# qurAI-amsterdam/SuperResolution_aniso_MRI

Measured on AMD Instinct MI355X. Metric: training slices/sec (ae_combined, 160x160, latent=128), higher is better.
Workload: dtype f32; 1 GPU; ACDC synthetic 12x(3x1x160x160) triplets, ae_combined latent=128 depth=32 scales=2, MSE synthesis loss (BASELINE configs[1]); global_batch_triplets=12, parallelism=dp1, init=reference Initializer, seed 892372, random weights, launch=captured HIP graph replay

## Files before the change

include/aesr_hip.h:

```cpp
#ifndef AESR_HIP_H
#define AESR_HIP_H

#include <stddef.h>
#include <stdint.h>

#ifdef __cplusplus
extern "C" {
#endif

#define AESR_ABI_VERSION 1
#define AESR_ERR_ARG 1
#define AESR_ERR_HIP 2
#define AESR_ERR_UNSUPPORTED 3

int aesr_version(void);
const char* aesr_last_error_string(void);


size_t aesr_conv2d_packed_floats(int Cout, int Cin, int KS, int transpose);
int aesr_conv2d_pack(const float* w, float* packed, int Cout, int Cin, int KS, int transpose, void* stream);
typedef struct aesr_pack_job {
    const float* w;
    float* packed;
    int Cout, Cin, KS, transpose;
} aesr_pack_job;
int aesr_conv2d_pack_many(const aesr_pack_job* jobs_host, int njobs, void* stream);

#define AESR_PREP_PACK 0
#define AESR_PREP_WINO_PACK 1
#define AESR_PREP_STEM_FOLD 2
#define AESR_PREP_COUT1_FLIP 3
typedef struct aesr_prep_job {
    const float* w;
    const float* aux0;
    const float* aux1;
    float* out;
    int kind, Cout, Cin, KS, transpose;
} aesr_prep_job;
int aesr_weight_prep_many(const aesr_prep_job* jobs_host, int njobs, void* stream);

int aesr_conv2d_fwd(const float* in, const float* packed, const float* bias, float* out, int N, int H, int W, int Cin,
                    int Cout, int KS, int pad, int act, float slope, void* stream);

size_t aesr_conv2d_workspace_floats(int N, int H, int W, int Cin, int Cout, int KS, int pad);
size_t aesr_conv2d_dgrad_workspace_floats(int N, int H, int W, int Cin, int Cout, int KS, int pad);
int aesr_conv2d_fwd_ws(const float* in, const float* packed, const float* bias, float* out, float* workspace, int N, int H, int W,
                       int Cin, int Cout, int KS, int pad, int act, float slope, void* stream);
int aesr_conv2d_dgrad_ws(const float* dy, const float* packed_t, const float* x_saved, float* dx, float* workspace, int N, int H,
                         int W, int Cin, int Cout, int KS, int pad, int mask_act, float slope, void* stream);

int aesr_conv2d_dgrad(const float* dy, const float* packed_t, const float* x_saved, float* dx, int N, int H, int W,
                      int Cin, int Cout, int KS, int pad, int mask_act, float slope, void* stream);

size_t aesr_conv2d_wgrad_workspace_floats(int N, int H, int W, int Cin, int Cout, int KS, int pad);
int aesr_conv2d_wgrad(const float* x, const float* dy, float* dw, float* db, float* workspace, int N, int H, int W,
                      int Cin, int Cout, int KS, int pad, void* stream);

int aesr_conv2d_smallcin_fwd(const float* in, const float* w, const float* bias, const float* y_saved, float* out, int N,
                             int H, int W, int Cin, int Cout, int KS, int pad, int act, int mask_act, float slope,
                             int transpose, int bcast, const float* ca_host, const float* cb_host, void* stream);
int aesr_conv2d_smallcin_dgrad(const float* dy, const float* w, float* dx, int N, int H, int W, int Cin, int Cout, int KS,
                               int pad, int bcast, const float* ca_host, void* stream);
size_t aesr_small_wgrad_workspace_floats(int nout);
int aesr_conv2d_smallcin_wgrad(const float* in, const float* dout, float* dw, float* db, float* workspace, int N, int H,
                               int W, int Cin, int Cout, int pad, void* stream);
int aesr_conv2d_cout1_fwd(const float* x, const float* w, const float* bias, float* out, int N, int H, int W, int Cin, int act,
                          float slope, void* stream);
size_t aesr_conv2d_cout1_workspace_floats(int Cin);
int aesr_conv2d_cout1_wgrad(const float* x, const float* dy, float* dw, float* db, float* workspace, int N, int H, int W,
                            int Cin, void* stream);
int aesr_conv2d_cout1_dgrad(const float* dy, const float* w, const float* y_saved, float* dx, float* workspace, int N, int H,
                            int W, int Cin, int mask_act, float slope, void* stream);
int aesr_conv2d_cout1_dgrad_pre(const float* dy, const float* w_flipped, const float* y_saved, float* dx, int N, int H, int W, int Cin,
                                int mask_act, float slope, void* stream);

size_t aesr_stemconv_folded_floats(int C1);
int aesr_stemconv_fold(const float* w_stem, const float* b_stem, const float* w1, float* folded, int Cs, int C1, void* stream);
int aesr_stemconv_fwd(const float* x, const float* folded, const float* b1, float* out, int N, int H, int W, int C1,
                      int stem_pad, int act, float slope, void* stream);
size_t aesr_stemconv_workspace_floats(int C1);
int aesr_stemconv_wgrad(const float* x, const float* g, const float* w_stem, const float* b_stem, const float* w1,
                        float* dw_stem, float* db_stem, float* dw1, float* db1, float* workspace, int N, int H, int W, int Cs,
                        int C1, int stem_pad, void* stream);

int aesr_space_to_depth2(const float* x, float* out, int N, int H, int W, int C, void* stream);
int aesr_depth_to_space2(const float* g, float* dx, int N, int H, int W, int C, void* stream);

#define AESR_RS_POOL 1
#define AESR_RS_NEAREST 2
#define AESR_RS_BILINEAR 3
int aesr_resample2_fwd(const float* x, float* out, int N, int H, int W, int C, int mode, void* stream);
int aesr_resample2_bwd(const float* gout, const float* x_saved, float* dx, int N, int H, int W, int C, int mode, int mask_act,
                       float slope, void* stream);

#define AESR_BN_NONE 0
#define AESR_BN_POOL 1
#define AESR_BN_UP 2
#define AESR_BN_NWG 512

int aesr_bn_stats(const float* y, float* partial, double* sums, int HW, int C, int G, const int* nstart_host,
                  void* stream);
int aesr_bn_finalize(const double* sums, const double* counts_host, const float* gamma, const float* beta,
                     float* running_mean, float* running_var, int64_t* num_batches_tracked, float* mean, float* invstd,
                     float* scale, float* shift, int C, int G, float momentum, float eps, int train, int update_running,
                     void* stream);
int aesr_bn_stats_finalize(const float* y, float* partial, const double* counts_host, const float* gamma, const float* beta,
                           float* running_mean, float* running_var, int64_t* num_batches_tracked, float* mean, float* invstd,
                           float* scale, float* shift, int HW, int C, int G, const int* nstart_host, float momentum, float eps,
                           int update_running, void* stream);
int aesr_bn_apply(const float* y, const float* scale, const float* shift, float* out, int N, int H, int W, int C, int mode,
                  int G, const int* nstart_host, void* stream);
int aesr_bn_fused_supported(int C, int G);
int aesr_bn_finalize_apply(const double* sums, const double* counts_host, const float* gamma, const float* beta, float* running_mean,
                           float* running_var, int64_t* num_batches_tracked, float* mean, float* invstd, float* scale, float* shift,
                           const float* y, float* out, int N, int H, int W, int C, int mode, int G, const int* nstart_host, float momentum,
                           float eps, int update_running, void* stream);
int aesr_bn_bwd_reduce(const float* gout, const float* y, const float* mean, const float* invstd, float* partial,
                       double* sums, int N, int H, int W, int C, int mode, int G, const int* nstart_host, void* stream);
int aesr_bn_bwd_apply(const float* gout, const float* y, const float* mean, const float* invstd, const float* scale,
                      const double* sums, const double* counts_host, float* coef, float* dgamma, float* dbeta,
                      float* dpre, int N, int H, int W, int C, int mode, int act, float slope, int G,
                      const int* nstart_host, void* stream);
int aesr_bn_bwd(const float* gout, const float* y, const float* mean, const float* invstd, const float* scale, float* partial,
                const double* counts_host, float* coef, float* dgamma, float* dbeta, float* dpre, int N, int H, int W, int C,
                int mode, int act, float slope, int G, const int* nstart_host, void* stream);

int aesr_scale_expand_fwd(const float* x, float* out4, size_t n, const float* ca_host, const float* cb_host, void* stream);
int aesr_scale_expand_bwd(const float* d4, float* dx, size_t n, const float* ca_host, void* stream);
int aesr_maxpool2_fwd(const float* x, float* out, int N, int H, int W, int C, void* stream);
int aesr_maxpool2_bwd(const float* gout, const float* x, const float* gadd, float* dx, int N, int H, int W, int C,
                      int relu_mask, void* stream);
#define AESR_LPIPS_NCH 64
int aesr_lpips_tap_fwd(const float* f, const float* lin_w, float* partial, int B, int HW, int C, void* stream);
int aesr_lpips_tap_bwd(const float* f, const float* lin_w, const float* gd, float* gf0, int B, int HW, int C, void* stream);
int aesr_lpips_finalize(const float* const* partials_host, const int* hw_host, int ntaps, float* d, int B, void* stream);

int aesr_lerp_fwd(const float* z, const float* a_from, const float* a_to, float* zmix, int B, size_t per, void* stream);
int aesr_lerp_bwd(const float* dzmix, const float* a_from, const float* a_to, float* dz, int B, size_t per, void* stream);
int aesr_lerp_cat_fwd(const float* z, const float* a_from, const float* a_to, float* zcat, int B, size_t per, void* stream);
int aesr_lerp_multi(const float* z, float* out, int Z, size_t per_slice, const float* alphas_host, int n, int act, float slope,
                    void* stream);
int aesr_lerp_cat_bwd(const float* g, const float* a_from, const float* a_to, float* dz, int B, size_t per, void* stream);
int aesr_interleave_clamp(const float* orig, const float* synth, float* out, int Z, int n, size_t per_slice, float lo, float hi, void* stream);

#define AESR_MSE_NPART 512
int aesr_mse_fwd(const float* a, const float* b, double* partial, float* loss, size_t n, void* stream);
int aesr_mse_bwd(const float* a, const float* b, const float* gloss, float* da, size_t n, void* stream);
#define AESR_MSE3_NPART 256
#define AESR_MSE3_WS (3 * AESR_MSE3_NPART + 1)
int aesr_mse3_fwd(const float* a1, const float* b1, size_t n1, const float* a2, const float* b2, size_t n2, const float* a3,
                  const float* b3, size_t n3, const float* lam, double* workspace, float* out4, void* stream);
int aesr_mse3_bwd(const float* a1, const float* b1, size_t n1, const float* a2, const float* b2, size_t n2, const float* lam,
                  const float* gloss, float* d1, float* d2, void* stream);
int aesr_l1_fwd(const float* a, const float* b, double* partial, float* loss, size_t n, void* stream);
int aesr_l1_bwd(const float* a, const float* b, const float* gloss, float* da, size_t n, void* stream);
int aesr_lap_blur5(const float* in, const float* add, float* out, int P, int H, int W, float gain, int adjoint, void* stream);
int aesr_lap_down2(const float* in, float* out, int P, int H, int W, void* stream);
int aesr_lap_zero_insert2(const float* in, float* out, int P, int h, int w, int H, int W, void* stream);
int aesr_row_mean_fwd(const float* x, float* out, int N, size_t M, void* stream);
int aesr_row_mean_bwd(const float* g, float* dx, int N, size_t M, void* stream);
int aesr_act_bwd(const float* dout, const float* y, float* dpre, size_t n, int act, float slope, void* stream);

void aesr_adam_state_init(float* state_host8, double steps_done, double beta1, double beta2);
int aesr_adam_step(float* p, float* g, float* exp_avg, float* exp_avg_sq, float* state, size_t n, float lr,
                   double beta1, double beta2, float eps, float weight_decay, int zero_grad, void* stream);

typedef struct aesr_triplet_desc {
    long long vol_off;
    int H, W, z_from, z_to, z_between, oy, ox, k;
    float gain, cutoff;
} aesr_triplet_desc;
int aesr_triplet_assemble(const float* volumes, const aesr_triplet_desc* desc_host, int B, int width, float* image,
                          float* between, void* stream);

size_t aesr_ssim_workspace_doubles(int Z, int H, int W);
int aesr_ssim_mse(const float* a, const float* b, double* workspace, double* ssim, double* mse, int Z, int H, int W, int win,
                  double data_range, double k1, double k2, void* stream);

int aesr_long_axis_views(const float* ref, const float* rec, float* ref_view, float* rec_view, unsigned char* black, int Z, int H, int W,
                         int axis, void* stream);

int aesr_bn_fused1_supported(int N, int H, int W, int C, int mode, int G, int backward);
size_t aesr_bn_fused1_workspace_floats(int C, int G);
size_t aesr_bn_fused1_barrier_words(void);
unsigned int aesr_bn_fused1_timeouts(void);
int aesr_bn_fused1_fwd(const float* y, float* out, float* workspace, unsigned int* barrier_state, const double* counts_host, const float* gamma,
                       const float* beta, float* running_mean, float* running_var, int64_t* num_batches_tracked, float* mean, float* invstd,
                       float* scale, float* shift, int N, int H, int W, int C, int mode, int G, const int* nstart_host, float momentum, float eps,
                       int update_running, void* stream);
int aesr_bn_fused1_bwd(const float* gout, const float* y, const float* mean, const float* invstd, const float* scale, float* workspace,
                       unsigned int* barrier_state, const double* counts_host, float* coef, float* dgamma, float* dbeta, float* dpre, int N, int H,
                       int W, int C, int mode, int act, float slope, int G, const int* nstart_host, void* stream);

#define AESR_P2P_HANDLE_BYTES 64
#define AESR_P2P_SLOTS 32
#define AESR_P2P_REC_BYTES (512 * 8 + 128)
int aesr_p2p_alloc(size_t bytes, void** region);
int aesr_p2p_free(void* region);
int aesr_p2p_get_handle(void* region, char* handle64);
int aesr_p2p_open(const char* handle64, void** peer_region);
int aesr_p2p_close(void* peer_region);
size_t aesr_p2p_region_bytes(int world);
int aesr_p2p_tick(unsigned int* gen_dev, void* stream);
int aesr_bn_fused1_fwd_p2p(const float* y, float* out, float* workspace, unsigned int* barrier_state, const double* counts_host, const float* gamma,
                           const float* beta, float* running_mean, float* running_var, int64_t* num_batches_tracked, float* mean, float* invstd,
                           float* scale, float* shift, int N, int H, int W, int C, int mode, int G, const int* nstart_host, float momentum, float eps,
                           int update_running, void* const* peers_host, int world, int rank, int slot, const unsigned int* gen_dev, void* stream);
int aesr_bn_fused1_bwd_p2p(const float* gout, const float* y, const float* mean, const float* invstd, const float* scale, float* workspace,
                           unsigned int* barrier_state, const double* counts_host, float* coef, float* dgamma, float* dbeta, float* dpre, int N, int H,
                           int W, int C, int mode, int act, float slope, int G, const int* nstart_host, void* const* peers_host, int world, int rank,
                           int slot, const unsigned int* gen_dev, void* stream);

size_t aesr_vif_workspace_bytes(int Z, int H, int W);
int aesr_vif_mscale(const float* ref, const float* dist, void* workspace, double* vif, int Z, int H, int W, const double* weights_host,
                    const int* radii_host, double sigma_nsq, void* stream);

int aesr_conv2d_wino_supported(int Cin, int Cout, int KS, int pad, int transpose);
int aesr_conv2d_wino_kernel(int N, int H, int W, int Cin, int Cout, int KS, int pad, int transpose);
unsigned int aesr_conv2d_wino_ring_timeouts(void);
size_t aesr_conv2d_wino_packed_floats(int Cout, int Cin, int transpose);
int aesr_conv2d_wino_pack_many(const aesr_pack_job* jobs_host, int njobs, void* stream);
int aesr_conv2d_wino_fwd(const float* in, const float* upacked, const float* bias, float* out, int N, int H, int W, int Cin,
                         int Cout, int act, float slope, void* stream);
int aesr_conv2d_wino_dgrad(const float* dy, const float* upacked_t, const float* x_saved, float* dx, int N, int H, int W, int Cin,
                           int Cout, int mask_act, float slope, void* stream);
int aesr_conv2d_wino_fwd_bn_supported(int N, int H, int W, int Cin, int Cout);
int aesr_conv2d_wino_fwd_bn(const float* in, const float* upacked, const float* bias, const float* bn_scale, const float* bn_shift, float* out, int N,
                            int H, int W, int Cin, int Cout, int act, float slope, int pool, void* stream);
size_t aesr_conv2d_wino_workspace_floats(int N, int H, int W, int Cin, int Cout, int transpose);
int aesr_conv2d_wino_fwd_ws(const float* in, const float* upacked, const float* bias, float* out, float* workspace, size_t workspace_floats,
                            int N, int H, int W, int Cin, int Cout, int act, float slope, void* stream);
int aesr_conv2d_wino_dgrad_ws(const float* dy, const float* upacked_t, const float* x_saved, float* dx, float* workspace, size_t workspace_floats,
                              int N, int H, int W, int Cin, int Cout, int mask_act, float slope, void* stream);

int aesr_conv2d_wino_fwd_up2(const float* in_half, const float* upacked, const float* bias, float* out, int N, int H, int W, int Cin,
                             int Cout, int act, float slope, void* stream);
int aesr_conv2d_wino_dgrad_sum2(const float* dy, const float* upacked_t, float* dx_half, int N, int H, int W, int Cin, int Cout,
                                void* stream);
int aesr_conv2d_wgrad_up2_supported(int Cin, int Cout);
int aesr_conv2d_wgrad_up2(const float* x_half, const float* dy, float* dw, float* db, float* workspace, int N, int H, int W, int Cin,
                          int Cout, void* stream);

typedef struct aesr_wgrad_reduce_job {
    const float* workspace;
    float* dw;
    float* db;
    int N, H, W, Cin, Cout, KS, pad;
} aesr_wgrad_reduce_job;
int aesr_conv2d_wgrad_partial(const float* x, const float* dy, float* workspace, int N, int H, int W, int Cin, int Cout, int KS,
                              int pad, int x_up2, void* stream);
int aesr_conv2d_wgrad_reduce_many(const aesr_wgrad_reduce_job* jobs_host, int njobs, void* stream);

#define AESR_COMM_ID_BYTES 128
#define AESR_COMM_F32 0
#define AESR_COMM_F64 1
#define AESR_COMM_SUM 0
#define AESR_COMM_MAX 1
int aesr_comm_rccl_version(int* version_out);
int aesr_comm_unique_id(void* id_host128);
int aesr_comm_init(const void* id_host128, int nranks, int rank, void** comm_out);
int aesr_comm_destroy(void* comm);
int aesr_comm_abort(void* comm);
int aesr_comm_allreduce(void* comm, void* buf, size_t count, int dtype, int op, void* stream);
int aesr_comm_allreduce_many(void* comm, void* const* bufs_host, const size_t* counts_host, int nbufs, int dtype, int op,
                             void* stream);
int aesr_comm_broadcast(void* comm, void* buf, size_t count, int dtype, int root, void* stream);

#ifdef __cplusplus
}
#endif
#endif
```

superresolution_aniso_mri_amd/_hip.py:

```python
import ctypes
import os
from ctypes import c_char_p, c_double, c_float, c_int, c_int64, c_size_t, c_void_p

import torch

_HERE = os.path.dirname(os.path.abspath(__file__))
LIB_PATH = os.path.join(_HERE, "libaesr_hip.so")
if os.environ.get("AESR_LIB"):
    import sys as _sys
    LIB_PATH = os.path.abspath(os.environ["AESR_LIB"])
    _sys.stderr.write("[aesr] AESR_LIB: loading the VARIANT library %s (not the shipped libaesr_hip.so)\n" % LIB_PATH)

P = c_void_p
IP = ctypes.POINTER(c_int)
FP = ctypes.POINTER(c_float)
DP = ctypes.POINTER(c_double)

class TripletDesc(ctypes.Structure):
    _fields_ = [("vol_off", ctypes.c_longlong), ("H", c_int), ("W", c_int), ("z_from", c_int), ("z_to", c_int), ("z_between", c_int),
                ("oy", c_int), ("ox", c_int), ("k", c_int), ("gain", c_float), ("cutoff", c_float)]


class WgradReduceJob(ctypes.Structure):
    _fields_ = [("workspace", c_void_p), ("dw", c_void_p), ("db", c_void_p), ("N", c_int), ("H", c_int), ("W", c_int), ("Cin", c_int),
                ("Cout", c_int), ("KS", c_int), ("pad", c_int)]


class PrepJob(ctypes.Structure):
    _fields_ = [("w", c_void_p), ("aux0", c_void_p), ("aux1", c_void_p), ("out", c_void_p), ("kind", c_int), ("Cout", c_int), ("Cin", c_int),
                ("KS", c_int), ("transpose", c_int)]


PREP_PACK, PREP_WINO_PACK, PREP_STEM_FOLD, PREP_COUT1_FLIP = 0, 1, 2, 3


class PackJob(ctypes.Structure):
    _fields_ = [("w", c_void_p), ("packed", c_void_p), ("Cout", c_int), ("Cin", c_int), ("KS", c_int), ("transpose", c_int)]


SIGNATURES = {
    "aesr_version": (c_int, []),
    "aesr_last_error_string": (c_char_p, []),
    "aesr_conv2d_packed_floats": (c_size_t, [c_int, c_int, c_int, c_int]),
    "aesr_conv2d_pack": (c_int, [P, P, c_int, c_int, c_int, c_int, P]),
    "aesr_conv2d_pack_many": (c_int, [ctypes.POINTER(PackJob), c_int, P]),
    "aesr_weight_prep_many": (c_int, [ctypes.POINTER(PrepJob), c_int, P]),
    "aesr_conv2d_cout1_dgrad_pre": (c_int, [P, P, P, P] + [c_int] * 5 + [c_float, P]),
    "aesr_conv2d_fwd": (c_int, [P, P, P, P] + [c_int] * 8 + [c_float, P]),
    "aesr_conv2d_workspace_floats": (c_size_t, [c_int] * 7),
    "aesr_conv2d_dgrad_workspace_floats": (c_size_t, [c_int] * 7),
    "aesr_conv2d_fwd_ws": (c_int, [P, P, P, P, P] + [c_int] * 8 + [c_float, P]),
    "aesr_conv2d_dgrad_ws": (c_int, [P, P, P, P, P] + [c_int] * 8 + [c_float, P]),
    "aesr_conv2d_dgrad": (c_int, [P, P, P, P] + [c_int] * 8 + [c_float, P]),
    "aesr_conv2d_wgrad_workspace_floats": (c_size_t, [c_int] * 7),
    "aesr_conv2d_wgrad": (c_int, [P, P, P, P, P] + [c_int] * 7 + [P]),
    "aesr_conv2d_smallcin_fwd": (c_int, [P, P, P, P, P] + [c_int] * 9 + [c_float, c_int, c_int, FP, FP, P]),
    "aesr_conv2d_smallcin_dgrad": (c_int, [P, P, P] + [c_int] * 8 + [FP, P]),
    "aesr_small_wgrad_workspace_floats": (c_size_t, [c_int]),
    "aesr_conv2d_smallcin_wgrad": (c_int, [P, P, P, P, P] + [c_int] * 6 + [P]),
    "aesr_conv2d_cout1_fwd": (c_int, [P, P, P, P] + [c_int] * 5 + [c_float, P]),
    "aesr_conv2d_cout1_workspace_floats": (c_size_t, [c_int]),
    "aesr_conv2d_cout1_wgrad": (c_int, [P, P, P, P, P] + [c_int] * 4 + [P]),
    "aesr_conv2d_cout1_dgrad": (c_int, [P, P, P, P, P] + [c_int] * 5 + [c_float, P]),
    "aesr_stemconv_folded_floats": (c_size_t, [c_int]),
    "aesr_stemconv_fold": (c_int, [P, P, P, P, c_int, c_int, P]),
    "aesr_stemconv_fwd": (c_int, [P, P, P, P] + [c_int] * 6 + [c_float, P]),
    "aesr_stemconv_workspace_floats": (c_size_t, [c_int]),
    "aesr_stemconv_wgrad": (c_int, [P] * 10 + [c_int] * 6 + [P]),
    "aesr_space_to_depth2": (c_int, [P, P] + [c_int] * 4 + [P]),
    "aesr_depth_to_space2": (c_int, [P, P] + [c_int] * 4 + [P]),
    "aesr_resample2_fwd": (c_int, [P, P] + [c_int] * 5 + [P]),
    "aesr_resample2_bwd": (c_int, [P, P, P] + [c_int] * 6 + [c_float, P]),
    "aesr_bn_stats": (c_int, [P, P, P, c_int, c_int, c_int, IP, P]),
    "aesr_bn_finalize": (c_int, [P, DP] + [P] * 9 + [c_int, c_int, c_float, c_float, c_int, c_int, P]),
    "aesr_bn_stats_finalize": (c_int, [P, P, DP] + [P] * 9 + [c_int, c_int, c_int, IP, c_float, c_float, c_int, P]),
    "aesr_bn_bwd": (c_int, [P] * 6 + [DP] + [P] * 4 + [c_int] * 6 + [c_float, c_int, IP, P]),
    "aesr_bn_fused_supported": (c_int, [c_int, c_int]),
    "aesr_bn_finalize_apply": (c_int, [P] * 13 + [c_int] * 6 + [P, c_float, c_float, c_int, P]),
    "aesr_bn_fused1_supported": (c_int, [c_int] * 7),
    "aesr_bn_fused1_workspace_floats": (c_size_t, [c_int, c_int]),
    "aesr_bn_fused1_barrier_words": (c_size_t, []),
    "aesr_bn_fused1_timeouts": (ctypes.c_uint, []),
    "aesr_bn_fused1_fwd": (c_int, [P, P, P, P, DP] + [P] * 9 + [c_int] * 6 + [IP, c_float, c_float, c_int, P]),
    "aesr_bn_fused1_bwd": (c_int, [P] * 7 + [DP] + [P] * 4 + [c_int] * 6 + [c_float, c_int, IP, P]),
    "aesr_p2p_alloc": (c_int, [c_size_t, ctypes.POINTER(c_void_p)]),
    "aesr_p2p_free": (c_int, [P]),
    "aesr_p2p_get_handle": (c_int, [P, c_char_p]),
    "aesr_p2p_open": (c_int, [c_char_p, ctypes.POINTER(c_void_p)]),
    "aesr_p2p_close": (c_int, [P]),
    "aesr_p2p_region_bytes": (c_size_t, [c_int]),
    "aesr_p2p_tick": (c_int, [P, P]),
    "aesr_bn_fused1_fwd_p2p": (c_int, [P, P, P, P, DP] + [P] * 9 + [c_int] * 6 + [IP, c_float, c_float, c_int, ctypes.POINTER(c_void_p), c_int, c_int, c_int, P, P]),
    "aesr_bn_fused1_bwd_p2p": (c_int, [P] * 7 + [DP] + [P] * 4 + [c_int] * 6 + [c_float, c_int, IP, ctypes.POINTER(c_void_p), c_int, c_int, c_int, P, P]),
    "aesr_bn_apply": (c_int, [P, P, P, P] + [c_int] * 6 + [IP, P]),
    "aesr_bn_bwd_reduce": (c_int, [P] * 6 + [c_int] * 6 + [IP, P]),
    "aesr_bn_bwd_apply": (c_int, [P] * 6 + [DP] + [P] * 4 + [c_int] * 6 + [c_float, c_int, IP, P]),
    "aesr_scale_expand_fwd": (c_int, [P, P, c_size_t, FP, FP, P]),
    "aesr_scale_expand_bwd": (c_int, [P, P, c_size_t, FP, P]),
    "aesr_maxpool2_fwd": (c_int, [P, P] + [c_int] * 4 + [P]),
    "aesr_maxpool2_bwd": (c_int, [P, P, P, P] + [c_int] * 5 + [P]),
    "aesr_lpips_tap_fwd": (c_int, [P, P, P, c_int, c_int, c_int, P]),
    "aesr_lpips_tap_bwd": (c_int, [P, P, P, P, c_int, c_int, c_int, P]),
    "aesr_lpips_finalize": (c_int, [ctypes.POINTER(c_void_p), IP, c_int, P, c_int, P]),
    "aesr_lerp_fwd": (c_int, [P, P, P, P, c_int, c_size_t, P]),
    "aesr_lerp_bwd": (c_int, [P, P, P, P, c_int, c_size_t, P]),
    "aesr_lerp_cat_fwd": (c_int, [P, P, P, P, c_int, c_size_t, P]),
    "aesr_lerp_multi": (c_int, [P, P, c_int, c_size_t, FP, c_int, c_int, c_float, P]),
    "aesr_lerp_cat_bwd": (c_int, [P, P, P, P, c_int, c_size_t, P]),
    "aesr_interleave_clamp": (c_int, [P, P, P, c_int, c_int, c_size_t, c_float, c_float, P]),
    "aesr_mse_fwd": (c_int, [P, P, P, P, c_size_t, P]),
    "aesr_mse_bwd": (c_int, [P, P, P, P, c_size_t, P]),
    "aesr_mse3_fwd": (c_int, [P, P, c_size_t, P, P, c_size_t, P, P, c_size_t, P, P, P, P]),
    "aesr_mse3_bwd": (c_int, [P, P, c_size_t, P, P, c_size_t, P, P, P, P, P]),
    "aesr_row_mean_fwd": (c_int, [P, P, c_int, c_size_t, P]),
    "aesr_row_mean_bwd": (c_int, [P, P, c_int, c_size_t, P]),
    "aesr_l1_fwd": (c_int, [P, P, P, P, c_size_t, P]),
    "aesr_l1_bwd": (c_int, [P, P, P, P, c_size_t, P]),
    "aesr_lap_blur5": (c_int, [P, P, P, c_int, c_int, c_int, c_float, c_int, P]),
    "aesr_lap_down2": (c_int, [P, P, c_int, c_int, c_int, P]),
    "aesr_lap_zero_insert2": (c_int, [P, P, c_int, c_int, c_int, c_int, c_int, P]),
    "aesr_act_bwd": (c_int, [P, P, P, c_size_t, c_int, c_float, P]),
    "aesr_triplet_assemble": (c_int, [P, ctypes.POINTER(TripletDesc), c_int, c_int, P, P, P]),
    "aesr_ssim_workspace_doubles": (c_size_t, [c_int, c_int, c_int]),
    "aesr_ssim_mse": (c_int, [P, P, P, P, P, c_int, c_int, c_int, c_int, c_double, c_double, c_double, P]),
    "aesr_long_axis_views": (c_int, [P, P, P, P, P, c_int, c_int, c_int, c_int, P]),
    "aesr_vif_workspace_bytes": (c_size_t, [c_int, c_int, c_int]),
    "aesr_vif_mscale": (c_int, [P, P, P, P, c_int, c_int, c_int, DP, IP, c_double, P]),
    "aesr_adam_state_init": (None, [FP, c_double, c_double, c_double]),
    "aesr_adam_step": (c_int, [P, P, P, P, P, c_size_t, c_float, c_double, c_double, c_float, c_float, c_int, P]),
    "aesr_conv2d_wino_supported": (c_int, [c_int] * 5),
    "aesr_conv2d_wino_kernel": (c_int, [c_int] * 8),
    "aesr_conv2d_wino_ring_timeouts": (ctypes.c_uint, []),
    "aesr_conv2d_wino_packed_floats": (c_size_t, [c_int, c_int, c_int]),
    "aesr_conv2d_wino_pack_many": (c_int, [ctypes.POINTER(PackJob), c_int, P]),
    "aesr_conv2d_wino_fwd": (c_int, [P, P, P, P] + [c_int] * 6 + [c_float, P]),
    "aesr_conv2d_wino_dgrad": (c_int, [P, P, P, P] + [c_int] * 6 + [c_float, P]),
    "aesr_conv2d_wino_workspace_floats": (c_size_t, [c_int] * 6),
    "aesr_conv2d_wino_fwd_bn_supported": (c_int, [c_int] * 5),
    "aesr_conv2d_wino_fwd_bn": (c_int, [P, P, P, P, P, P] + [c_int] * 6 + [c_float, c_int, P]),
    "aesr_conv2d_wino_fwd_ws": (c_int, [P, P, P, P, P, c_size_t] + [c_int] * 6 + [c_float, P]),
    "aesr_conv2d_wino_dgrad_ws": (c_int, [P, P, P, P, P, c_size_t] + [c_int] * 6 + [c_float, P]),
    "aesr_conv2d_wino_fwd_up2": (c_int, [P, P, P, P] + [c_int] * 6 + [c_float, P]),
    "aesr_conv2d_wino_dgrad_sum2": (c_int, [P, P, P] + [c_int] * 5 + [P]),
    "aesr_conv2d_wgrad_up2_supported": (c_int, [c_int, c_int]),
    "aesr_conv2d_wgrad_up2": (c_int, [P, P, P, P, P] + [c_int] * 5 + [P]),
    "aesr_conv2d_wgrad_partial": (c_int, [P, P, P] + [c_int] * 8 + [P]),
    "aesr_conv2d_wgrad_reduce_many": (c_int, [ctypes.POINTER(WgradReduceJob), c_int, P]),
    "aesr_comm_rccl_version": (c_int, [IP]),
    "aesr_comm_unique_id": (c_int, [c_char_p]),
    "aesr_comm_init": (c_int, [c_char_p, c_int, c_int, ctypes.POINTER(c_void_p)]),
    "aesr_comm_destroy": (c_int, [P]),
    "aesr_comm_abort": (c_int, [P]),
    "aesr_comm_allreduce": (c_int, [P, P, c_size_t, c_int, c_int, P]),
    "aesr_comm_allreduce_many": (c_int, [P, ctypes.POINTER(c_void_p), ctypes.POINTER(c_size_t), c_int, c_int, c_int, P]),
    "aesr_comm_broadcast": (c_int, [P, P, c_size_t, c_int, c_int, P]),
}
SIGNATURES_PREPROC = {
    "aesr_inplane_out_size": (c_int, [c_int, c_double]),
    "aesr_inplane_workspace_bytes": (c_size_t, [c_int, c_int]),
    "aesr_inplane_resample": (c_int, [P, P, P] + [c_int] * 5 + [DP, c_int, DP, c_int, IP, DP, IP, DP, c_int, P]),
}
P2P_HANDLE_BYTES, P2P_SLOTS = 64, 32
COMM_ID_BYTES = 128
COMM_F32, COMM_F64, COMM_SUM, COMM_MAX = 0, 1, 0, 1

ACT_NONE, ACT_LRELU, ACT_RELU, ACT_SIGMOID = 0, 1, 2, 3
BN_NONE, BN_POOL, BN_UP = 0, 1, 2
RS_POOL, RS_NEAREST, RS_BILINEAR = 1, 2, 3
BN_NWG = 512
REDUCE_MAX_JOBS = 16
MSE_NPART = 512
MSE3_WS = 3 * 256 + 1
LPIPS_NCH = 64


def _load():
    if not os.path.exists(LIB_PATH):
        raise RuntimeError(
            "libaesr_hip.so not found at %s -- build it with `python __graft_entry__.py` (or `make -C "
            "superresolution_aniso_mri_amd/csrc`). The HIP extension is mandatory: there is no CPU/eager fallback." % LIB_PATH)
    lib = ctypes.CDLL(LIB_PATH)
    for name, (res, args) in list(SIGNATURES.items()) + list(SIGNATURES_PREPROC.items()):
        fn = getattr(lib, name, None)
        if fn is None:
            raise RuntimeError("libaesr_hip.so does not export %s (stale build?)" % name)
        fn.restype, fn.argtypes = res, args
    return lib


lib = _load()


def last_error():
    return lib.aesr_last_error_string().decode("utf-8", "replace")


def check(rc, what):
    if rc != 0:
        raise RuntimeError("%s failed (code %d): %s" % (what, rc, last_error()))


def check_device_watchdogs(where):
    nb = int(lib.aesr_bn_fused1_timeouts())
    if nb:
        raise RuntimeError("%s: the one-launch BatchNorm kernel's grid barrier gave up %d time(s) in this process -- its workgroups were not all "
                           "resident (the device is shared with another grid-barrier kernel: set AESR_BN_FUSED=0); results since are not "
                           "trustworthy; nothing was written" % (where, nb))
    n = int(lib.aesr_conv2d_wino_ring_timeouts())
    if n:
        raise RuntimeError("%s: the ring convolution kernel's arrival-counter watchdog fired %d time(s) in this process -- activations / "
                           "gradients computed since are not trustworthy (csrc/conv_wino_ring.hip: wait_full); nothing was written" % (where, n))


def ptr(t):
    if t is None:
        return None
    return c_void_p(t.data_ptr())


_raw_stream = getattr(torch._C, "_cuda_getCurrentRawStream", None)
_cur_device = getattr(torch._C, "_cuda_getDevice", None)
# ... 29 lines not shown
```

superresolution_aniso_mri_amd/csrc/aesr_api.hip:

```cpp
#include <stdarg.h>
#include <stdio.h>
#include <stdlib.h>
#include <string.h>

#include <map>
#include <mutex>
#include <tuple>

#include "../../include/aesr_hip.h"
#include "aesr_kernels.h"

static thread_local char g_err[512] = "";
void aesr_set_error(const char* fmt, ...) {
    va_list ap;
    va_start(ap, fmt);
    vsnprintf(g_err, sizeof(g_err), fmt, ap);
    va_end(ap);
}

static void cout_padding(int Cout, int* CoutP, int* NB) {
    if (Cout <= 16) { *CoutP = 16; *NB = 1; }
    else if (Cout <= 32) { *CoutP = 32; *NB = 2; }
    else { *CoutP = round_up(Cout, 64); *NB = 4; }
}
// ... 442 lines not shown
    const int kin = transpose ? Cout : Cin, nout = transpose ? Cin : Cout;
    const WinoPlan p = plan_wino(N, H, W, kin, nout);
    WinoArgs a = {};
    a.N = N; a.H = H; a.W = W; a.Cin = kin; a.Cout = nout;
    a.CinP = p.CinP; a.CoutP = p.CoutP;
    a.plan_cost = p.cost;
    if (aesr_wino_res_ok(a)) return 0;
    return aesr_wino_ring_workspace_floats(a);
}

unsigned int aesr_conv2d_wino_ring_timeouts(void) {
    (void)hipDeviceSynchronize();
    return aesr_wino_ring_timeouts();
}

size_t aesr_conv2d_wino_packed_floats(int Cout, int Cin, int transpose) {
    const int kin = transpose ? Cout : Cin, nout = transpose ? Cin : Cout;
    return (size_t)16 * round_up(kin, 16) * round_up(nout, 32);
}

int aesr_conv2d_wino_pack_many(const aesr_pack_job* jobs_host, int njobs, void* stream) {
    AESR_CHECK_ARG(jobs_host && njobs > 0, "aesr_conv2d_wino_pack_many: no jobs");
    for (int j0 = 0; j0 < njobs; j0 += PACK_MAX_JOBS) {
        PackTable t;
        memset(&t, 0, sizeof(t));
        t.njobs = njobs - j0 < PACK_MAX_JOBS ? njobs - j0 : PACK_MAX_JOBS;
        int nb = 0;
        for (int k = 0; k < t.njobs; ++k) {
            const aesr_pack_job& jb = jobs_host[j0 + k];
            AESR_CHECK_ARG(jb.w && jb.packed && jb.Cout > 0 && jb.Cin > 0 && jb.KS == 3, "aesr_conv2d_wino_pack_many: bad job %d", j0 + k);
            const int kin = jb.transpose ? jb.Cout : jb.Cin, nout = jb.transpose ? jb.Cin : jb.Cout;
            PackJob& o = t.job[k];
            o.w = jb.w; o.p = jb.packed; o.Cout = jb.Cout; o.Cin = jb.Cin; o.KS = 3; o.KinP = round_up(kin, 16); o.NoutP = round_up(nout, 32);
            o.TN = 32; o.transpose = jb.transpose; o.block0 = nb;
            const size_t pairs = (size_t)o.KinP * o.NoutP;
            int blocks = (int)((pairs + 255) / 256);
            if (blocks > 256) blocks = 256;
            nb += blocks;
        }
        t.nblocks = nb;
        if (int e = aesr_launch_wino_pack_many(t, (hipStream_t)stream)) return e;
    }
    return AESR_OK;
}

static int run_wino(const float* in, const float* upk, const float* bias, const float* ysave, float* out, int N, int H, int W,
                    int Cin, int Cout, int act, int mask_act, float slope, hipStream_t st, int in_up2 = 0, int out_sum2 = 0,
                    float* ws = nullptr, size_t ws_floats = 0) {
    AESR_CHECK_DIMS("aesr_conv2d_wino", N, H, W, Cin, Cout);
    const WinoPlan p = plan_wino(N, H, W, Cin, Cout);
    WinoArgs a = {};
    a.in = in; a.upk = upk; a.bias = bias; a.ysave = ysave; a.out = out;
    a.N = N; a.H = H; a.W = W; a.Cin = Cin; a.CinP = p.CinP; a.Cout = Cout; a.CoutP = p.CoutP;
    a.TI = p.TI; a.THt = p.THt; a.TWt = p.TWt; a.regs_y = a.regs_x = a.nitems = 0;
    a.plan_cost = p.cost;
    a.act = act; a.mask_act = mask_act; a.slope = slope; a.dbgbuf = nullptr; a.flags = 0; a.in_up2 = in_up2; a.out_sum2 = out_sum2;
    a.ws = ws_floats ? ws : nullptr; a.ws_floats = ws ? ws_floats : 0;
    a.ksplit = 1;
    return aesr_launch_conv_wino(a, st);
}

int aesr_conv2d_wino_fwd(const float* in, const float* upacked, const float* bias, float* out, int N, int H, int W, int Cin,
                         int Cout, int act, float slope, void* stream) {
    AESR_CHECK_ARG(in && upacked && out && N > 0 && H > 0 && W > 0, "aesr_conv2d_wino_fwd: null pointer or empty shape");
    AESR_CHECK_ARG(aesr_conv2d_wino_supported(Cin, Cout, 3, 1, 0), "aesr_conv2d_wino_fwd: needs Cin %% 16 == 0 and Cout %% 32 == 0 (got %d -> %d)", Cin, Cout);
    return run_wino(in, upacked, bias, nullptr, out, N, H, W, Cin, Cout, act, ACT_NONE, slope, (hipStream_t)stream);
}

int aesr_conv2d_wino_dgrad(const float* dy, const float* upacked_t, const float* x_saved, float* dx, int N, int H, int W, int Cin,
                           int Cout, int mask_act, float slope, void* stream) {
    AESR_CHECK_ARG(dy && upacked_t && dx && N > 0 && H > 0 && W > 0, "aesr_conv2d_wino_dgrad: null pointer or empty shape");
    AESR_CHECK_ARG(aesr_conv2d_wino_supported(Cin, Cout, 3, 1, 1), "aesr_conv2d_wino_dgrad: needs Cout %% 16 == 0 and Cin %% 32 == 0 (got %d -> %d)", Cin, Cout);
    return run_wino(dy, upacked_t, nullptr, x_saved, dx, N, H, W, Cout, Cin, ACT_NONE, mask_act, slope, (hipStream_t)stream);
}

int aesr_conv2d_wino_fwd_ws(const float* in, const float* upacked, const float* bias, float* out, float* workspace, size_t workspace_floats,
                            int N, int H, int W, int Cin, int Cout, int act, float slope, void* stream) {
    AESR_CHECK_ARG(in && upacked && out && N > 0 && H > 0 && W > 0, "aesr_conv2d_wino_fwd_ws: null pointer or empty shape");
    AESR_CHECK_ARG(aesr_conv2d_wino_supported(Cin, Cout, 3, 1, 0), "aesr_conv2d_wino_fwd_ws: needs Cin %% 16 == 0 and Cout %% 32 == 0 (got %d -> %d)", Cin, Cout);
    return run_wino(in, upacked, bias, nullptr, out, N, H, W, Cin, Cout, act, ACT_NONE, slope, (hipStream_t)stream, 0, 0, workspace, workspace_floats);
}

int aesr_conv2d_wino_dgrad_ws(const float* dy, const float* upacked_t, const float* x_saved, float* dx, float* workspace, size_t workspace_floats,
                              int N, int H, int W, int Cin, int Cout, int mask_act, float slope, void* stream) {
    AESR_CHECK_ARG(dy && upacked_t && dx && N > 0 && H > 0 && W > 0, "aesr_conv2d_wino_dgrad_ws: null pointer or empty shape");
    AESR_CHECK_ARG(aesr_conv2d_wino_supported(Cin, Cout, 3, 1, 1), "aesr_conv2d_wino_dgrad_ws: needs Cout %% 16 == 0 and Cin %% 32 == 0 (got %d -> %d)", Cin, Cout);
    return run_wino(dy, upacked_t, nullptr, x_saved, dx, N, H, W, Cout, Cin, ACT_NONE, mask_act, slope, (hipStream_t)stream, 0, 0, workspace, workspace_floats);
}

int aesr_conv2d_wino_fwd_bn_supported(int N, int H, int W, int Cin, int Cout) {
    if (!aesr_conv2d_wino_supported(Cin, Cout, 3, 1, 0) || !conv_dims_ok(N, H, W, Cin, Cout)) return 0;
    const WinoPlan p = plan_wino(N, H, W, Cin, Cout);
    WinoArgs a = {};
    a.N = N; a.H = H; a.W = W; a.Cin = Cin; a.Cout = Cout;
    a.CinP = p.CinP; a.CoutP = p.CoutP;
    a.plan_cost = p.cost;
    if (aesr_wino_res_ok(a)) return 1;
    return aesr_wino_ring_takes(a) ? 1 : 0;
}

int aesr_conv2d_wino_fwd_bn(const float* in, const float* upacked, const float* bias, const float* bn_scale, const float* bn_shift, float* out, int N,
                            int H, int W, int Cin, int Cout, int act, float slope, int pool, void* stream) {
    AESR_CHECK_ARG(in && upacked && bn_scale && bn_shift && out && N > 0 && H > 0 && W > 0, "aesr_conv2d_wino_fwd_bn: null pointer or empty shape");
    AESR_CHECK_ARG(!pool || (H >= 2 && W >= 2), "aesr_conv2d_wino_fwd_bn: pooling needs H, W >= 2");
    AESR_CHECK_ARG(aesr_conv2d_wino_fwd_bn_supported(N, H, W, Cin, Cout), "aesr_conv2d_wino_fwd_bn: %d -> %d at %d x %d x %d is not a resident-filter or ring-kernel layer "
                   "(aesr_conv2d_wino_fwd_bn_supported)", Cin, Cout, N, H, W);
    const WinoPlan p = plan_wino(N, H, W, Cin, Cout);
    WinoArgs a = {};
    a.in = in; a.upk = upacked; a.bias = bias; a.ysave = nullptr; a.out = out;
    a.N = N; a.H = H; a.W = W; a.Cin = Cin; a.CinP = p.CinP; a.Cout = Cout; a.CoutP = p.CoutP;
    a.TI = p.TI; a.THt = p.THt; a.TWt = p.TWt;
    a.plan_cost = p.cost;
    a.act = act; a.mask_act = ACT_NONE; a.slope = slope; a.ksplit = 1;
    a.post_scale = bn_scale; a.post_shift = bn_shift; a.post_pool = pool ? 1 : 0;
    return aesr_launch_conv_wino(a, (hipStream_t)stream);
}

int aesr_conv2d_wino_fwd_up2(const float* in_half, const float* upacked, const float* bias, float* out, int N, int H, int W, int Cin,
                             int Cout, int act, float slope, void* stream) {
    AESR_CHECK_ARG(in_half && upacked && out && N > 0 && H > 0 && W > 0 && !((H | W) & 1), "aesr_conv2d_wino_fwd_up2: null pointer, empty or odd shape");
    AESR_CHECK_ARG(aesr_conv2d_wino_supported(Cin, Cout, 3, 1, 0), "aesr_conv2d_wino_fwd_up2: needs Cin %% 16 == 0 and Cout %% 32 == 0 (got %d -> %d)", Cin, Cout);
    return run_wino(in_half, upacked, bias, nullptr, out, N, H, W, Cin, Cout, act, ACT_NONE, slope, (hipStream_t)stream, 1, 0);
}

int aesr_conv2d_wino_dgrad_sum2(const float* dy, const float* upacked_t, float* dx_half, int N, int H, int W, int Cin, int Cout,
                                void* stream) {
    AESR_CHECK_ARG(dy && upacked_t && dx_half && N > 0 && H > 0 && W > 0 && !((H | W) & 1), "aesr_conv2d_wino_dgrad_sum2: null pointer, empty or odd shape");
    AESR_CHECK_ARG(aesr_conv2d_wino_supported(Cin, Cout, 3, 1, 1), "aesr_conv2d_wino_dgrad_sum2: needs Cout %% 16 == 0 and Cin %% 32 == 0 (got %d -> %d)", Cin, Cout);
    return run_wino(dy, upacked_t, nullptr, nullptr, dx_half, N, H, W, Cout, Cin, ACT_NONE, ACT_NONE, 0.f, (hipStream_t)stream, 0, 1);
}

size_t aesr_conv2d_wgrad_workspace_floats(int N, int H, int W, int Cin, int Cout, int KS, int pad) {
    if (!conv_dims_ok(N, H, W, Cin, Cout) || (KS != 1 && KS != 3) || pad < 0 || pad >= KS) return 0;
    const int Ho = H + 2 * pad - KS + 1, Wo = W + 2 * pad - KS + 1;
    if (Ho <= 0 || Wo <= 0) return 0;
    return plan_wgrad(N, Ho, Wo, Cin, Cout, KS, pad).slab_floats;
}

static int wgrad_impl(const float* x, const float* dy, float* dw, float* db, float* workspace, int N, int H, int W, int Cin,
                      int Cout, int KS, int pad, void* stream, int x_up2);

int aesr_conv2d_wgrad(const float* x, const float* dy, float* dw, float* db, float* workspace, int N, int H, int W, int Cin,
                      int Cout, int KS, int pad, void* stream) {
    return wgrad_impl(x, dy, dw, db, workspace, N, H, W, Cin, Cout, KS, pad, stream, 0);
}

int aesr_conv2d_wgrad_partial(const float* x, const float* dy, float* workspace, int N, int H, int W, int Cin, int Cout, int KS,
                              int pad, int x_up2, void* stream) {
    AESR_CHECK_ARG(!x_up2 || (wgrad_wino_ok(Cin, Cout, KS, pad) && !((H | W) & 1)), "aesr_conv2d_wgrad_partial: the folded upsampling needs "
                   "the Winograd weight-gradient kernel (3x3, padding 1, Cin, Cout multiples of 32) and an even size");
    return wgrad_impl(x, dy, nullptr, nullptr, workspace, N, H, W, Cin, Cout, KS, pad, stream, x_up2);
}

int aesr_conv2d_wgrad_reduce_many(const aesr_wgrad_reduce_job* jobs_host, int njobs, void* stream) {
    AESR_CHECK_ARG(jobs_host && njobs > 0, "aesr_conv2d_wgrad_reduce_many: no jobs");
    for (int j0 = 0; j0 < njobs; j0 += REDUCE_MAX_JOBS) {
        ReduceTable t;
        memset(&t, 0, sizeof(t));
        t.njobs = njobs - j0 < REDUCE_MAX_JOBS ? njobs - j0 : REDUCE_MAX_JOBS;
        int nb = 0;
        for (int k = 0; k < t.njobs; ++k) {
            const aesr_wgrad_reduce_job& jb = jobs_host[j0 + k];
            AESR_CHECK_ARG(jb.workspace && jb.dw && jb.N > 0 && (jb.KS == 1 || jb.KS == 3), "aesr_conv2d_wgrad_reduce_many: bad job %d", j0 + k);
            AESR_CHECK_ARG(conv_dims_ok(jb.N, jb.H, jb.W, jb.Cin, jb.Cout) && jb.pad >= 0 && jb.pad < jb.KS && jb.H + 2 * jb.pad >= jb.KS && jb.W + 2 * jb.pad >= jb.KS,
                           "aesr_conv2d_wgrad_reduce_many: job %d: bad shape", j0 + k);
            const int Ho = jb.H + 2 * jb.pad - jb.KS + 1, Wo = jb.W + 2 * jb.pad - jb.KS + 1;
            const WgradPlan p = plan_wgrad(jb.N, Ho, Wo, jb.Cin, jb.Cout, jb.KS, jb.pad);
            ReduceJob& o = t.job[k];
            o.slab = jb.workspace; o.dw = jb.dw; o.db = jb.db; o.nslab = p.nslab; o.KS2 = jb.KS * jb.KS; o.Cin = jb.Cin; o.CinP = p.CinP;
            o.Cout = jb.Cout; o.CoutP = p.CoutP; o.block0 = nb;
            nb += ceil_div(o.KS2 * jb.Cin * jb.Cout + (jb.db ? jb.Cout : 0), 64);
        }
        t.nblocks = nb;
        if (int e = aesr_launch_wgrad_reduce_many(t, (hipStream_t)stream)) return e;
    }
    return AESR_OK;
}

int aesr_conv2d_wgrad_up2_supported(int Cin, int Cout) { return wgrad_wino_ok(Cin, Cout, 3, 1) ? 1 : 0; }

int aesr_conv2d_wgrad_up2(const float* x_half, const float* dy, float* dw, float* db, float* workspace, int N, int H, int W, int Cin,
                          int Cout, void* stream) {
    AESR_CHECK_ARG(wgrad_wino_ok(Cin, Cout, 3, 1) && !((H | W) & 1), "aesr_conv2d_wgrad_up2: needs the Winograd weight-gradient kernel "
                   "(Cin, Cout multiples of 32; got %d -> %d) and an even size", Cin, Cout);
    return wgrad_impl(x_half, dy, dw, db, workspace, N, H, W, Cin, Cout, 3, 1, stream, 1);
}

static int wgrad_impl(const float* x, const float* dy, float* dw, float* db, float* workspace, int N, int H, int W, int Cin,
                      int Cout, int KS, int pad, void* stream, int x_up2) {
    AESR_CHECK_ARG(x && dy && workspace && N > 0, "aesr_conv2d_wgrad: null pointer or empty shape");
    AESR_CHECK_ARG(Cin % 4 == 0 && Cout % 4 == 0, "aesr_conv2d_wgrad: Cin=%d, Cout=%d must be multiples of 4", Cin, Cout);
    AESR_CHECK_ARG((KS == 1 || KS == 3) && pad >= 0 && pad < KS, "aesr_conv2d_wgrad: unsupported KS=%d pad=%d", KS, pad);
    AESR_CHECK_DIMS("aesr_conv2d_wgrad", N, H, W, Cin, Cout);
    const int Ho = H + 2 * pad - KS + 1, Wo = W + 2 * pad - KS + 1;
    AESR_CHECK_ARG(Ho > 0 && Wo > 0, "aesr_conv2d_wgrad: the %d x %d input is smaller than the %d x %d filter", H, W, KS, KS);
    const WgradPlan p = plan_wgrad(N, Ho, Wo, Cin, Cout, KS, pad);
    WgradArgs a;
    a.x = x; a.dy = dy; a.slab = workspace;
    a.N = N; a.H = H; a.W = W; a.Cin = Cin; a.CinP = p.CinP; a.Cout = Cout; a.CoutP = p.CoutP; a.Ho = Ho; a.Wo = Wo; a.pad = pad;
    a.TH = p.TH; a.TW = p.TW; a.tiles_y = ceil_div(Ho, p.TH); a.tiles_x = ceil_div(Wo, p.TW);
    a.ntiles = N * a.tiles_y * a.tiles_x; a.S = p.S;
    a.PWS = p.PWS; a.TWS = p.TWS; a.PSX = p.PSX; a.PSD = p.PSD; a.dbgbuf = nullptr; a.x_up2 = x_up2;
    if (p.variant == 2) {
        if (int e = aesr_launch_conv_wgrad_wino(a, (hipStream_t)stream)) return e;
    } else if (int e = aesr_launch_conv_wgrad(a, KS, p.variant, (hipStream_t)stream)) {
        return e;
    }
    if (!dw) return AESR_OK;
    return aesr_launch_wgrad_reduce(workspace, dw, db, p.nslab, KS, Cin, p.CinP, Cout, p.CoutP, (hipStream_t)stream);
}

int aesr_conv2d_smallcin_fwd(const float* in, const float* w, const float* bias, const float* y_saved, float* out, int N,
                             int H, int W, int Cin, int Cout, int KS, int pad, int act, int mask_act, float slope,
                             int transpose, int bcast, const float* ca_host, const float* cb_host, void* stream) {
    AESR_CHECK_ARG(in && w && out && N > 0 && Cin >= 1 && Cin <= 4 && Cout > 0, "aesr_conv2d_smallcin_fwd: need 1 <= Cin <= 4");
    AESR_CHECK_ARG(!bcast || (ca_host && cb_host), "aesr_conv2d_smallcin_fwd: bcast needs ca/cb");
    SmallArgs a;
    memset(&a, 0, sizeof(a));
    a.in = in; a.w = w; a.bias = bias; a.ysave = y_saved; a.out = out;
    a.N = N; a.H = H; a.W = W; a.Cin = Cin; a.Cout = Cout; a.KS = KS; a.pad = pad;
    a.Ho = H + 2 * pad - KS + 1; a.Wo = W + 2 * pad - KS + 1;
    a.act = act; a.mask_act = mask_act; a.slope = slope; a.transpose = transpose; a.bcast = bcast;
    for (int i = 0; i < Cin && bcast; ++i) { a.ca[i] = ca_host[i]; a.cb[i] = cb_host[i]; }
    return aesr_launch_smallcin_fwd(a, (hipStream_t)stream);
}

int aesr_conv2d_smallcin_dgrad(const float* dy, const float* w, float* dx, int N, int H, int W, int Cin, int Cout, int KS,
                               int pad, int bcast, const float* ca_host, void* stream) {
    AESR_CHECK_ARG(dy && w && dx && N > 0 && Cin >= 1 && Cin <= 4 && Cout > 0, "aesr_conv2d_smallcin_dgrad: need 1 <= Cin <= 4");
    AESR_CHECK_ARG(!bcast || ca_host, "aesr_conv2d_smallcin_dgrad: bcast needs ca");
    SmallDgradArgs a;
    memset(&a, 0, sizeof(a));
    a.dy = dy; a.w = w; a.dx = dx; a.N = N; a.H = H; a.W = W; a.Cin = Cin; a.Cout = Cout; a.KS = KS; a.pad = pad; a.bcast = bcast;
    a.Ho = H + 2 * pad - KS + 1; a.Wo = W + 2 * pad - KS + 1;
    for (int i = 0; i < Cin && bcast; ++i) a.ca[i] = ca_host[i];
    return aesr_launch_smallcin_dgrad(a, (hipStream_t)stream);
}

#define SMALL_WGRAD_NWG 512
size_t aesr_small_wgrad_workspace_floats(int nout) { return (size_t)SMALL_WGRAD_NWG * nout; }

int aesr_conv2d_smallcin_wgrad(const float* in, const float* dout, float* dw, float* db, float* workspace, int N, int H,
                               int W, int Cin, int Cout, int pad, void* stream) {
    AESR_CHECK_ARG(in && dout && dw && db && workspace && Cin >= 1 && Cin <= 4, "aesr_conv2d_smallcin_wgrad: need 1 <= Cin <= 4");
    AESR_CHECK_ARG(Cout >= 4 && Cout % 4 == 0 && 256 % (Cout / 4) == 0 && Cout <= 256,
                   "aesr_conv2d_smallcin_wgrad: Cout=%d must be a multiple of 4 with Cout/4 dividing 256", Cout);
    SmallWgradArgs a;
    a.in = in; a.dout = dout; a.partial = workspace; a.N = N; a.H = H; a.W = W; a.Cin = Cin; a.Cout = Cout; a.pad = pad;
    a.Ho = H + 2 * pad; a.Wo = W + 2 * pad;
    if (int e = aesr_launch_smallcin_wgrad(a, SMALL_WGRAD_NWG, (hipStream_t)stream)) return e;
    return aesr_launch_sum_partials(workspace, SMALL_WGRAD_NWG, Cout * (Cin + 1), dw, Cout * Cin, db, (hipStream_t)stream);
}

int aesr_conv2d_cout1_fwd(const float* x, const float* w, const float* bias, float* out, int N, int H, int W, int Cin, int act,
                          float slope, void* stream) {
    AESR_CHECK_ARG(x && w && out && N > 0 && H > 0 && W > 0, "aesr_conv2d_cout1_fwd: null pointer or empty shape");
    AESR_CHECK_ARG(Cin > 0 && Cin % 4 == 0 && Cin <= 256, "aesr_conv2d_cout1_fwd: Cin=%d must be a multiple of 4 (<= 256)", Cin);
    if (((Cin / 4) & (Cin / 4 - 1)) == 0)
        return aesr_launch_thin_collapse(x, w, bias, out, N, H, W, Cin, act, slope, (hipStream_t)stream);
    Cout1FwdArgs a;
    a.x = x; a.w = w; a.bias = bias; a.out = out; a.N = N; a.H = H; a.W = W; a.Cin = Cin; a.act = act; a.slope = slope;
    a.TH = H < 16 ? H : 16; a.TW = W < 16 ? W : 16;
    while (((size_t)(a.TH + 2) * (a.TW + 2) * (Cin + 4) + 9 * Cin) * 4 > 64 * 1024 && a.TH > 1) a.TH /= 2;
    a.tiles_y = ceil_div(H, a.TH); a.tiles_x = ceil_div(W, a.TW);
    return aesr_launch_cout1_fwd(a, (hipStream_t)stream);
}

#define THIN_NWG 512
static bool thin_channels_ok(int C) { return C >= 4 && C <= 256 && C % 4 == 0 && ((C / 4) & (C / 4 - 1)) == 0; }

size_t aesr_conv2d_cout1_workspace_floats(int Cin) {
    const size_t legacy = (size_t)SMALL_WGRAD_NWG * (Cin * 9 + 1);
    const size_t thin = (size_t)(THIN_NWG + 1) * 10 * Cin;
    return legacy > thin ? legacy : thin;
}

int aesr_conv2d_cout1_wgrad(const float* x, const float* dy, float* dw, float* db, float* workspace, int N, int H, int W,
                            int Cin, void* stream) {
    AESR_CHECK_ARG(x && dy && dw && db && workspace, "aesr_conv2d_cout1_wgrad: null pointer");
    AESR_CHECK_ARG(N > 0 && H > 0 && W > 0, "aesr_conv2d_cout1_wgrad: empty shape");
    if (thin_channels_ok(Cin)) {
        ThinArgs a;
        memset(&a, 0, sizeof(a));
        a.s = dy; a.t = x; a.partial = workspace;
        a.N = N; a.Hs = H; a.Ws = W; a.Ho = H; a.Wo = W; a.C = Cin; a.ps = 0; a.with_be = 0;
        float* R = workspace + (size_t)THIN_NWG * 10 * Cin;
        if (int e = aesr_launch_thin_reduce(a, THIN_NWG, (hipStream_t)stream)) return e;
        if (int e = aesr_launch_sum_partials(workspace, THIN_NWG, 10 * Cin, R, 10 * Cin, nullptr, (hipStream_t)stream)) return e;
        return aesr_launch_thin_cout1_finish(R, dw, db, Cin, (hipStream_t)stream);
    }
    AESR_CHECK_ARG(Cin >= 4 && Cin <= 128 && 256 % Cin == 0, "aesr_conv2d_cout1_wgrad: Cin=%d must divide 256 (and be >= 4)", Cin);
    Cout1WgradArgs a;
    a.x = x; a.dy = dy; a.partial = workspace; a.N = N; a.H = H; a.W = W; a.Cin = Cin;
    a.TH = H < 16 ? H : 16; a.TW = W < 16 ? W : 16;
    while ((size_t)(a.TH + 2) * (a.TW + 2) * (Cin + 1) * 4 > 60 * 1024 && a.TH > 1) a.TH /= 2;
    a.tiles_y = ceil_div(H, a.TH); a.tiles_x = ceil_div(W, a.TW); a.ntiles = N * a.tiles_y * a.tiles_x;
    int nwg = a.ntiles < SMALL_WGRAD_NWG ? a.ntiles : SMALL_WGRAD_NWG;
    if (int e = aesr_launch_cout1_wgrad(a, nwg, (hipStream_t)stream)) return e;
    return aesr_launch_sum_partials(workspace, nwg, Cin * 9 + 1, dw, Cin * 9, db, (hipStream_t)stream);
}

int aesr_conv2d_cout1_dgrad(const float* dy, const float* w, const float* y_saved, float* dx, float* workspace, int N, int H,
                            int W, int Cin, int mask_act, float slope, void* stream) {
    AESR_CHECK_ARG(dy && w && dx && workspace && N > 0 && H > 0 && W > 0, "aesr_conv2d_cout1_dgrad: null pointer or empty shape");
    AESR_CHECK_ARG(thin_channels_ok(Cin), "aesr_conv2d_cout1_dgrad: Cin=%d must be 4 times a power of two (4..256)", Cin);
    if (int e = aesr_launch_thin_cout1_flip(w, workspace, Cin, (hipStream_t)stream)) return e;
    ThinArgs a;
    memset(&a, 0, sizeof(a));
    a.s = dy; a.w = workspace; a.ysave = y_saved; a.out = dx;
    a.N = N; a.Hs = H; a.Ws = W; a.Ho = H; a.Wo = W; a.C = Cin; a.ps = 0;
    a.act = ACT_NONE; a.mask_act = y_saved ? mask_act : ACT_NONE; a.slope = slope;
    return aesr_launch_thin_expand(a, (hipStream_t)stream);
}

int aesr_conv2d_cout1_dgrad_pre(const float* dy, const float* w_flipped, const float* y_saved, float* dx, int N, int H, int W, int Cin,
                                int mask_act, float slope, void* stream) {
    AESR_CHECK_ARG(dy && w_flipped && dx && N > 0 && H > 0 && W > 0, "aesr_conv2d_cout1_dgrad_pre: null pointer or empty shape");
    AESR_CHECK_ARG(thin_channels_ok(Cin), "aesr_conv2d_cout1_dgrad_pre: Cin=%d must be 4 times a power of two (4..256)", Cin);
    ThinArgs a;
    memset(&a, 0, sizeof(a));
    a.s = dy; a.w = w_flipped; a.ysave = y_saved; a.out = dx;
    a.N = N; a.Hs = H; a.Ws = W; a.Ho = H; a.Wo = W; a.C = Cin; a.ps = 0;
    a.act = ACT_NONE; a.mask_act = y_saved ? mask_act : ACT_NONE; a.slope = slope;
    return aesr_launch_thin_expand(a, (hipStream_t)stream);
}

size_t aesr_stemconv_folded_floats(int C1) { return (size_t)2 * 9 * C1; }

int aesr_stemconv_fold(const float* w_stem, const float* b_stem, const float* w1, float* folded, int Cs, int C1, void* stream) {
    AESR_CHECK_ARG(w_stem && w1 && folded && Cs > 0 && C1 > 0, "aesr_stemconv_fold: bad arguments");
    return aesr_launch_thin_stem_fold(w_stem, b_stem, w1, folded, Cs, C1, (hipStream_t)stream);
}

int aesr_stemconv_fwd(const float* x, const float* folded, const float* b1, float* out, int N, int H, int W, int C1,
                      int stem_pad, int act, float slope, void* stream) {
    AESR_CHECK_ARG(x && folded && out && N > 0 && H > 0 && W > 0 && stem_pad >= 0, "aesr_stemconv_fwd: bad arguments");
    AESR_CHECK_ARG(thin_channels_ok(C1), "aesr_stemconv_fwd: C1=%d must be 4 times a power of two (4..256)", C1);
    ThinArgs a;
    memset(&a, 0, sizeof(a));
    a.s = x; a.w = folded; a.be = folded + (size_t)9 * C1; a.b = b1; a.out = out;
    a.N = N; a.Hs = H; a.Ws = W; a.Ho = H + 2 * stem_pad; a.Wo = W + 2 * stem_pad; a.C = C1; a.ps = stem_pad;
    a.act = act; a.mask_act = ACT_NONE; a.slope = slope;
    return aesr_launch_thin_expand(a, (hipStream_t)stream);
}

size_t aesr_stemconv_workspace_floats(int C1) { return (size_t)(THIN_NWG + 1) * 19 * C1; }

int aesr_stemconv_wgrad(const float* x, const float* g, const float* w_stem, const float* b_stem, const float* w1,
                        float* dw_stem, float* db_stem, float* dw1, float* db1, float* workspace, int N, int H, int W, int Cs,
                        int C1, int stem_pad, void* stream) {
    AESR_CHECK_ARG(x && g && w_stem && w1 && dw_stem && dw1 && workspace, "aesr_stemconv_wgrad: null pointer");
    AESR_CHECK_ARG(N > 0 && H > 0 && W > 0 && Cs > 0 && stem_pad >= 0, "aesr_stemconv_wgrad: bad shape");
    AESR_CHECK_ARG(thin_channels_ok(C1), "aesr_stemconv_wgrad: C1=%d must be 4 times a power of two (4..256)", C1);
    AESR_CHECK_ARG(!db_stem || b_stem, "aesr_stemconv_wgrad: db_stem needs b_stem");
    ThinArgs a;
    memset(&a, 0, sizeof(a));
    a.s = x; a.t = g; a.partial = workspace;
    a.N = N; a.Hs = H; a.Ws = W; a.Ho = H + 2 * stem_pad; a.Wo = W + 2 * stem_pad; a.C = C1; a.ps = stem_pad; a.with_be = 1;
    float* R = workspace + (size_t)THIN_NWG * 19 * C1;
    if (int e = aesr_launch_thin_reduce(a, THIN_NWG, (hipStream_t)stream)) return e;
    if (int e = aesr_launch_sum_partials(workspace, THIN_NWG, 19 * C1, R, 19 * C1, nullptr, (hipStream_t)stream)) return e;
    return aesr_launch_thin_stem_finish(R, w_stem, b_stem, w1, dw_stem, db_stem, dw1, db1, Cs, C1, (hipStream_t)stream);
}

int aesr_resample2_fwd(const float* x, float* out, int N, int H, int W, int C, int mode, void* stream) {
    AESR_CHECK_ARG(x && out && N > 0 && H > 0 && W > 0 && C > 0 && C % 4 == 0, "aesr_resample2_fwd: bad arguments (C %% 4 == 0)");
    AESR_CHECK_ARG(mode >= AESR_RS_POOL && mode <= AESR_RS_BILINEAR, "aesr_resample2_fwd: unknown mode %d", mode);
    AESR_CHECK_ARG(mode != AESR_RS_POOL || (H >= 2 && W >= 2), "aesr_resample2_fwd: pooling needs H, W >= 2");
    return aesr_launch_resample2(x, nullptr, nullptr, out, N, H, W, C, mode, 0, ACT_NONE, 0.f, (hipStream_t)stream);
}

int aesr_resample2_bwd(const float* gout, const float* x_saved, float* dx, int N, int H, int W, int C, int mode, int mask_act,
                       float slope, void* stream) {
    AESR_CHECK_ARG(gout && dx && N > 0 && H > 0 && W > 0 && C > 0 && C % 4 == 0, "aesr_resample2_bwd: bad arguments (C %% 4 == 0)");
    AESR_CHECK_ARG(mode >= AESR_RS_POOL && mode <= AESR_RS_BILINEAR, "aesr_resample2_bwd: unknown mode %d", mode);
    AESR_CHECK_ARG(mode != AESR_RS_POOL || (H >= 2 && W >= 2), "aesr_resample2_bwd: pooling needs H, W >= 2");
    return aesr_launch_resample2(nullptr, gout, x_saved, dx, N, H, W, C, mode, 1, x_saved ? mask_act : ACT_NONE, slope,
                                 (hipStream_t)stream);
}

int aesr_bn_stats(const float* y, float* partial, double* sums, int HW, int C, int G, const int* nstart_host, void* stream) {
    BnGroups gr;
    AESR_CHECK_ARG(y && partial && sums && fill_groups(&gr, G, nstart_host), "aesr_bn_stats: bad arguments");
    if (int e = aesr_launch_bn_stats(y, partial, HW, C, gr, AESR_BN_NWG, (hipStream_t)stream)) return e;
    return aesr_launch_bn_reduce(partial, sums, AESR_BN_NWG, C, G, (hipStream_t)stream);
}

int aesr_bn_finalize(const double* sums, const double* counts_host, const float* gamma, const float* beta, float* running_mean,
                     float* running_var, int64_t* num_batches_tracked, float* mean, float* invstd, float* scale, float* shift,
                     int C, int G, float momentum, float eps, int train, int update_running, void* stream) {
    AESR_CHECK_ARG(gamma && beta && mean && invstd && scale && shift && G >= 1 && G <= 4, "aesr_bn_finalize: bad arguments");
    AESR_CHECK_ARG(!train || (sums && counts_host), "aesr_bn_finalize: train mode needs sums and counts");
    AESR_CHECK_ARG(train || (running_mean && running_var), "aesr_bn_finalize: eval mode needs running stats");
    return aesr_launch_bn_finalize(sums, counts_host, gamma, beta, running_mean, running_var, (long long*)num_batches_tracked, mean,
                                   invstd, scale, shift, C, G, momentum, eps, train, update_running && running_mean && running_var,
                                   (hipStream_t)stream);
}

int aesr_bn_stats_finalize(const float* y, float* partial, const double* counts_host, const float* gamma, const float* beta,
                           float* running_mean, float* running_var, int64_t* num_batches_tracked, float* mean, float* invstd,
                           float* scale, float* shift, int HW, int C, int G, const int* nstart_host, float momentum, float eps,
                           int update_running, void* stream) {
    BnGroups gr;
    AESR_CHECK_ARG(y && partial && counts_host && fill_groups(&gr, G, nstart_host), "aesr_bn_stats_finalize: bad arguments");
    AESR_CHECK_ARG(gamma && beta && mean && invstd && scale && shift, "aesr_bn_stats_finalize: null pointer");
    if (int e = aesr_launch_bn_stats(y, partial, HW, C, gr, AESR_BN_NWG, (hipStream_t)stream)) return e;
    return aesr_launch_bn_reduce_finalize(partial, AESR_BN_NWG, counts_host, gamma, beta, running_mean, running_var,
                                          (long long*)num_batches_tracked, mean, invstd, scale, shift, C, G, momentum, eps,
                                          update_running && running_mean && running_var, (hipStream_t)stream);
}

static void bn_out_dims(int H, int W, int mode, int* Ho, int* Wo) {
    if (mode == AESR_BN_POOL) { *Ho = H / 2; *Wo = W / 2; }
    else if (mode == AESR_BN_UP) { *Ho = 2 * H; *Wo = 2 * W; }
    else { *Ho = H; *Wo = W; }
}

int aesr_bn_apply(const float* y, const float* scale, const float* shift, float* out, int N, int H, int W, int C, int mode,
                  int G, const int* nstart_host, void* stream) {
    BnApplyArgs a;
    AESR_CHECK_ARG(y && scale && shift && out && fill_groups(&a.gr, G, nstart_host), "aesr_bn_apply: bad arguments");
    a.y = y; a.scale = scale; a.shift = shift; a.out = out; a.N = N; a.H = H; a.W = W; a.C = C; a.mode = mode;
    bn_out_dims(H, W, mode, &a.Ho, &a.Wo);
    AESR_CHECK_ARG(a.Ho > 0 && a.Wo > 0, "aesr_bn_apply: empty output");
    return aesr_launch_bn_apply(a, (hipStream_t)stream);
}

int aesr_bn_fused_supported(int C, int G) { return aesr_bn_fused_ok(C, G) ? 1 : 0; }

int aesr_bn_fused1_supported(int N, int H, int W, int C, int mode, int G, int backward) {
    if (mode != AESR_BN_NONE && mode != AESR_BN_POOL) return 0;
    return aesr_bn_fused1_ok(N, H, W, C, mode == AESR_BN_POOL, G, backward) ? 1 : 0;
}

size_t aesr_bn_fused1_workspace_floats(int C, int G) { return (size_t)256 * G * 2 * C; }
size_t aesr_bn_fused1_barrier_words(void) { return 16 * 32; }
unsigned int aesr_bn_fused1_timeouts(void) { return aesr_bn_fused_timeouts_impl(); }

int aesr_bn_fused1_fwd(const float* y, float* out, float* workspace, unsigned int* barrier_state, const double* counts_host, const float* gamma,
                       const float* beta, float* running_mean, float* running_var, int64_t* num_batches_tracked, float* mean, float* invstd,
                       float* scale, float* shift, int N, int H, int W, int C, int mode, int G, const int* nstart_host, float momentum, float eps,
                       int update_running, void* stream) {
    BnGroups gr;
    AESR_CHECK_ARG(y && out && workspace && barrier_state && counts_host && gamma && beta && mean && invstd && scale && shift &&
                       fill_groups(&gr, G, nstart_host) && gr.nstart[G] == N, "aesr_bn_fused1_fwd: bad arguments");
    AESR_CHECK_ARG(mode == AESR_BN_NONE || mode == AESR_BN_POOL, "aesr_bn_fused1_fwd: mode %d (the un-folded Upsample takes the three-launch path)", mode);
    return aesr_bn_fused_run(y, nullptr, out, workspace, barrier_state, gamma, beta, running_mean, running_var, (long long*)num_batches_tracked, mean,
                             invstd, scale, shift, nullptr, nullptr, nullptr, N, H, W, C, mode == AESR_BN_POOL, G, gr.nstart, counts_host, momentum, eps,
                             update_running && running_mean && running_var, ACT_NONE, 0.f, 0, nullptr, (hipStream_t)stream);
}

int aesr_bn_fused1_bwd(const float* gout, const float* y, const float* mean, const float* invstd, const float* scale, float* workspace,
                       unsigned int* barrier_state, const double* counts_host, float* coef, float* dgamma, float* dbeta, float* dpre, int N, int H,
                       int W, int C, int mode, int act, float slope, int G, const int* nstart_host, void* stream) {
    BnGroups gr;
    AESR_CHECK_ARG(gout && y && mean && invstd && scale && workspace && barrier_state && counts_host && coef && dgamma && dbeta && dpre &&
                       fill_groups(&gr, G, nstart_host) && gr.nstart[G] == N, "aesr_bn_fused1_bwd: bad arguments");
    AESR_CHECK_ARG(mode == AESR_BN_NONE || mode == AESR_BN_POOL, "aesr_bn_fused1_bwd: mode %d (the un-folded Upsample takes the three-launch path)", mode);
    return aesr_bn_fused_run(y, gout, dpre, workspace, barrier_state, nullptr, nullptr, nullptr, nullptr, nullptr, (float*)mean, (float*)invstd,
                             (float*)scale, nullptr, coef, dgamma, dbeta, N, H, W, C, mode == AESR_BN_POOL, G, gr.nstart, counts_host, 0.f, 0.f, 0, act, slope,
                             1, nullptr, (hipStream_t)stream);
}

size_t aesr_p2p_region_bytes(int world) { return world > 0 && world <= 8 ? (size_t)AESR_P2P_SLOTS * 2 * world * AESR_P2P_REC_BYTES : 0; }

int aesr_p2p_tick(unsigned int* gen_dev, void* stream) {
    AESR_CHECK_ARG(gen_dev, "aesr_p2p_tick: null pointer");
    return aesr_launch_p2p_tick(gen_dev, (hipStream_t)stream);
}

static int fill_p2p(BnP2P* p, void* const* peers_host, int world, int rank, int slot, const unsigned int* gen_dev, const char* who) {
    if (!peers_host || !gen_dev || world < 1 || world > 8 || rank < 0 || rank >= world || slot < 0 || slot >= AESR_P2P_SLOTS) {
        aesr_set_error("%s: bad exchange arguments (world %d, rank %d, slot %d of %d)", who, world, rank, slot, AESR_P2P_SLOTS);
        return AESR_ERR_ARG;
    }
    p->world = world; p->rank = rank; p->slot = slot; p->gen = gen_dev;
    for (int r = 0; r < 8; ++r) p->peers[r] = r < world ? peers_host[r] : nullptr;
    for (int r = 0; r < world; ++r)
        if (!p->peers[r]) {
            aesr_set_error("%s: the region of rank %d is not mapped", who, r);
            return AESR_ERR_ARG;
        }
    return AESR_OK;
}

int aesr_bn_fused1_fwd_p2p(const float* y, float* out, float* workspace, unsigned int* barrier_state, const double* counts_host, const float* gamma,
                           const float* beta, float* running_mean, float* running_var, int64_t* num_batches_tracked, float* mean, float* invstd,
                           float* scale, float* shift, int N, int H, int W, int C, int mode, int G, const int* nstart_host, float momentum, float eps,
                           int update_running, void* const* peers_host, int world, int rank, int slot, const unsigned int* gen_dev, void* stream) {
    BnGroups gr;
    BnP2P p2p;
    AESR_CHECK_ARG(y && out && workspace && barrier_state && counts_host && gamma && beta && mean && invstd && scale && shift &&
                       fill_groups(&gr, G, nstart_host) && gr.nstart[G] == N, "aesr_bn_fused1_fwd_p2p: bad arguments");
    AESR_CHECK_ARG(mode == AESR_BN_NONE || mode == AESR_BN_POOL, "aesr_bn_fused1_fwd_p2p: mode %d", mode);
    if (int e = fill_p2p(&p2p, peers_host, world, rank, slot, gen_dev, "aesr_bn_fused1_fwd_p2p")) return e;
    return aesr_bn_fused_run(y, nullptr, out, workspace, barrier_state, gamma, beta, running_mean, running_var, (long long*)num_batches_tracked, mean,
                             invstd, scale, shift, nullptr, nullptr, nullptr, N, H, W, C, mode == AESR_BN_POOL, G, gr.nstart, counts_host, momentum, eps,
                             update_running && running_mean && running_var, ACT_NONE, 0.f, 0, &p2p, (hipStream_t)stream);
}

int aesr_bn_fused1_bwd_p2p(const float* gout, const float* y, const float* mean, const float* invstd, const float* scale, float* workspace,
                           unsigned int* barrier_state, const double* counts_host, float* coef, float* dgamma, float* dbeta, float* dpre, int N, int H,
                           int W, int C, int mode, int act, float slope, int G, const int* nstart_host, void* const* peers_host, int world, int rank,
                           int slot, const unsigned int* gen_dev, void* stream) {
    BnGroups gr;
    BnP2P p2p;
    AESR_CHECK_ARG(gout && y && mean && invstd && scale && workspace && barrier_state && counts_host && coef && dgamma && dbeta && dpre &&
                       fill_groups(&gr, G, nstart_host) && gr.nstart[G] == N, "aesr_bn_fused1_bwd_p2p: bad arguments");
    AESR_CHECK_ARG(mode == AESR_BN_NONE || mode == AESR_BN_POOL, "aesr_bn_fused1_bwd_p2p: mode %d", mode);
    if (int e = fill_p2p(&p2p, peers_host, world, rank, slot, gen_dev, "aesr_bn_fused1_bwd_p2p")) return e;
    return aesr_bn_fused_run(y, gout, dpre, workspace, barrier_state, nullptr, nullptr, nullptr, nullptr, nullptr, (float*)mean, (float*)invstd,
                             (float*)scale, nullptr, coef, dgamma, dbeta, N, H, W, C, mode == AESR_BN_POOL, G, gr.nstart, counts_host, 0.f, 0.f, 0, act, slope,
                             1, &p2p, (hipStream_t)stream);
}

int aesr_bn_finalize_apply(const double* sums, const double* counts_host, const float* gamma, const float* beta, float* running_mean,
                           float* running_var, int64_t* num_batches_tracked, float* mean, float* invstd, float* scale, float* shift,
// ... 281 lines not shown
```

superresolution_aniso_mri_amd/csrc/aesr_kernels.h:

```cpp
#pragma once
#include "aesr_common.h"

struct IgemmArgs {
    const float* in; const float* wpk; const float* bias; const float* ysave; float* out;
    int N, H, W, Cin, CinP, Cout, CoutP, Ho, Wo, pad;
    int TI, TH, TW, tiles_y, tiles_x, nitems, dbg;
    int NT;
    int ksplit;
    float* dbgbuf;
    int act, mask_act;
    float slope;
};
int aesr_launch_conv_igemm(const IgemmArgs& a, int KS, int NB, int MBW, hipStream_t st);
int aesr_launch_conv_ksplit_fixup(const float* partial, const float* bias, const float* ysave, float* out, size_t nelem, int Cout,
                                  int ksplit, int act, int mask_act, float slope, hipStream_t st);
int aesr_launch_pack_weights(const float* w, float* p, int Cout, int Cin, int KS, int KinP, int NoutP, int TN, int transpose, hipStream_t st);

struct WinoArgs {
    const float* in; const float* upk; const float* bias; const float* ysave; float* out;
    int N, H, W, Cin, CinP, Cout, CoutP;
    int TI, THt, TWt;
    int regs_y, regs_x, nitems;
    unsigned m_ncot, m_regs_x, m_regs_y;
    int act, mask_act;
    float slope;
    float* dbgbuf;
    int flags;
    int in_up2;
    int out_sum2;
    int bpi, nblk;
    unsigned m_bpi;
    int nw, rowP, imgP, patch_fl, sw_a, sw_m, sw_b;
    int xcd_map;
    double plan_cost;
    int nfull, tail_k;
    int ksplit, kchunks, split_bytes;
    unsigned m_ksplit;
    float* ws;
    size_t ws_floats;
    const float* post_scale; const float* post_shift;
    int post_pool;
};
int aesr_launch_conv_wino(const WinoArgs& a, hipStream_t st);
bool aesr_wino_res_ok(const WinoArgs& a);
int aesr_launch_conv_wino_res(const WinoArgs& a, hipStream_t st);
int aesr_wino_ring_mode();
bool aesr_wino_ring_takes(const WinoArgs& a);
int aesr_launch_conv_wino_ring(const WinoArgs& a, hipStream_t st);
size_t aesr_wino_ring_workspace_floats(const WinoArgs& a);
unsigned aesr_wino_ring_timeouts();
size_t aesr_wino_lds_bytes(int patch_pixels);

#define PACK_MAX_JOBS 32
struct PackJob { const float* w; float* p; int Cout, Cin, KS, KinP, NoutP, TN, transpose, block0; };
struct PackTable { int njobs, nblocks; PackJob job[PACK_MAX_JOBS]; };
int aesr_launch_pack_many(const PackTable& t, hipStream_t st);
enum { PREP_PACK = 0, PREP_WINO_PACK = 1, PREP_STEM_FOLD = 2, PREP_COUT1_FLIP = 3 };
struct PrepJob { const float* w; const float* aux0; const float* aux1; float* out; int kind, Cout, Cin, KS, KinP, NoutP, TN, transpose, block0; };
struct PrepTable { int njobs, nblocks; PrepJob job[PACK_MAX_JOBS]; };
int aesr_launch_prep_many(const PrepTable& t, hipStream_t st);
int aesr_launch_wino_pack_many(const PackTable& t, hipStream_t st);

struct WgradArgs {
    const float* x; const float* dy; float* slab;
    int N, H, W, Cin, CinP, Cout, CoutP, Ho, Wo, pad;
    int TH, TW, tiles_y, tiles_x, ntiles;
    int S;
    int PWS, TWS, PSX, PSD;
    float* dbgbuf;
    int x_up2;
};
int aesr_launch_conv_wgrad(const WgradArgs& a, int KS, int variant, hipStream_t st);
int aesr_launch_conv_wgrad_wino(const WgradArgs& a, hipStream_t st);
size_t aesr_wgrad_wino_lds_bytes(int TH, int TW);
bool aesr_wgrad_wino_tile_ok(int TH, int TW);
#define REDUCE_MAX_JOBS 16
struct ReduceJob { const float* slab; float* dw; float* db; int nslab, KS2, Cin, CinP, Cout, CoutP, block0; };
struct ReduceTable { int njobs, nblocks; ReduceJob job[REDUCE_MAX_JOBS]; };
int aesr_launch_wgrad_reduce_many(const ReduceTable& t, hipStream_t st);
int aesr_launch_wgrad_reduce(const float* slab, float* dw, float* db, int nslab, int KS, int Cin, int CinP, int Cout, int CoutP, hipStream_t st);

struct SmallArgs {
    const float* in; const float* w; const float* bias; const float* ysave; float* out;
    int N, H, W, Cin, Cout, Ho, Wo, KS, pad;
    int act, mask_act;
    float slope;
    int transpose, bcast;
    float ca[4], cb[4];
};
struct SmallDgradArgs {
    const float* dy; const float* w; float* dx;
    int N, H, W, Cin, Cout, Ho, Wo, KS, pad, bcast;
    float ca[4];
};
struct SmallWgradArgs {
    const float* in; const float* dout; float* partial;
    int N, H, W, Cin, Cout, Ho, Wo, pad;
};
struct Cout1WgradArgs {
    const float* x; const float* dy; float* partial;
    int N, H, W, Cin, TH, TW, tiles_y, tiles_x, ntiles;
};
struct Cout1FwdArgs {
    const float* x; const float* w; const float* bias; float* out;
    int N, H, W, Cin, TH, TW, tiles_y, tiles_x, act;
    float slope;
};
int aesr_launch_cout1_fwd(const Cout1FwdArgs& a, hipStream_t st);
int aesr_launch_smallcin_fwd(const SmallArgs& a, hipStream_t st);
int aesr_launch_smallcin_dgrad(const SmallDgradArgs& a, hipStream_t st);
int aesr_launch_sum_partials(const float* partial, int np, int n, float* out0, int n0, float* out1, hipStream_t st);
int aesr_launch_smallcin_wgrad(const SmallWgradArgs& a, int nwg, hipStream_t st);
int aesr_launch_cout1_wgrad(const Cout1WgradArgs& a, int nwg, hipStream_t st);

struct ThinArgs {
    const float* s;
    const float* w;
    const float* be;
    const float* b;
    const float* ysave;
    float* out;
    const float* t;
    float* partial;
    int N, Hs, Ws, Ho, Wo, C, ps;
    int act, mask_act;
    float slope;
    int with_be;
    int tiles_y, tiles_x, ntiles;
};
int aesr_launch_thin_expand(ThinArgs a, hipStream_t st);
int aesr_launch_thin_reduce(ThinArgs a, int nwg, hipStream_t st);
int aesr_launch_thin_collapse(const float* x, const float* w, const float* bias, float* out, int N, int H, int W, int C, int act,
                              float slope, hipStream_t st);
int aesr_launch_thin_stem_fold(const float* ws, const float* bs, const float* w1, float* folded, int Cs, int C1, hipStream_t st);
int aesr_launch_thin_stem_finish(const float* R, const float* ws, const float* bs, const float* w1, float* dws, float* dbs,
                                 float* dw1, float* db1, int Cs, int C1, hipStream_t st);
int aesr_launch_thin_cout1_flip(const float* w, float* wexp, int Cin, hipStream_t st);
int aesr_launch_thin_cout1_finish(const float* R, float* dw, float* db, int Cin, hipStream_t st);

struct BnGroups { int G; int nstart[5]; };
struct BnApplyArgs {
    const float* y; const float* scale; const float* shift; float* out;
    int N, H, W, C, Ho, Wo, mode;
    BnGroups gr;
};
struct BnBwdArgs {
    const float* gout; const float* y; const float* mean; const float* invstd; const float* scale; const float* coef;
    float* partial; float* dpre;
    int N, H, W, C, Ho, Wo, mode, act;
    float slope;
    BnGroups gr;
    unsigned long long m_hw, m_w;
    int k_hw, k_w;
};
struct BnFusedArgs;
struct BnP2P { int world, rank, slot; const unsigned* gen; void* peers[8]; };
int aesr_launch_p2p_tick(unsigned* gen, hipStream_t st);
bool aesr_bn_fused1_ok(int N, int H, int W, int C, int pool, int G, int backward);
unsigned aesr_bn_fused_timeouts_impl();
int aesr_bn_fused_run(const float* y, const float* gout, float* out, float* rec, unsigned* bar, const float* gamma, const float* beta,
                      float* running_mean, float* running_var, long long* nbt, float* mean, float* invstd, float* scale, float* shift, float* coef,
                      float* dgamma, float* dbeta, int N, int H, int W, int C, int pool, int G, const int* nstart, const double* counts,
                      float momentum, float eps, int update_running, int act, float slope, int backward, const BnP2P* p2p, hipStream_t st);
int aesr_launch_bn_stats(const float* y, float* partial, int HW, int C, const BnGroups& gr, int nwg, hipStream_t st);
int aesr_launch_bn_reduce(const float* partial, double* sums, int nwg, int C, int G, hipStream_t st);
int aesr_launch_bn_finalize(const double* sums, const double* counts, const float* gamma, const float* beta, float* rm, float* rv,
                            long long* nbt, float* mean, float* invstd, float* scale, float* shift, int C, int G, float momentum,
                            float eps, int train, int update_running, hipStream_t st);
int aesr_launch_bn_reduce_finalize(const float* partial, int nwg, const double* counts, const float* gamma, const float* beta,
                                   float* running_mean, float* running_var, long long* nbt, float* mean, float* invstd,
                                   float* scale, float* shift, int C, int G, float momentum, float eps, int update_running,
                                   hipStream_t st);
int aesr_launch_bn_bwd_reduce_finalize(const float* partial, int nwg, const double* counts, float* coef, float* dgamma,
                                       float* dbeta, int C, int G, hipStream_t st);
int aesr_launch_bn_apply(const BnApplyArgs& a, hipStream_t st);
int aesr_launch_bn_bwd_reduce(const BnBwdArgs& a, int nwg, hipStream_t st);
int aesr_launch_bn_bwd_finalize(const double* sums, const double* counts, float* coef, float* dgamma, float* dbeta, int C, int G, hipStream_t st);
int aesr_launch_bn_bwd_apply(const BnBwdArgs& a, hipStream_t st);
bool aesr_bn_fused_ok(int C, int G);
int aesr_launch_bn_finalize_apply(const double* sums, const double* counts, const float* gamma, const float* beta, float* running_mean,
                                  float* running_var, long long* nbt, float* mean, float* invstd, float* scale, float* shift, float momentum,
                                  float eps, int update_running, int G, const BnApplyArgs& a, hipStream_t st);
int aesr_launch_bn_bwd_finalize_apply(const double* sums, const double* counts, float* coef, float* dgamma, float* dbeta, int G,
                                      const BnBwdArgs& a, hipStream_t st);

int aesr_launch_lerp_fwd(const float* z, const float* af, const float* at, float* zmix, int B, size_t per, hipStream_t st);
int aesr_launch_lerp_bwd(const float* dmix, const float* af, const float* at, float* dz, int B, size_t per, hipStream_t st);
int aesr_launch_lerp_cat_fwd(const float* z, const float* af, const float* at, float* zcat, int B, size_t per, hipStream_t st);
int aesr_launch_interleave_clamp(const float* orig, const float* synth, float* out, int Z, int n, size_t per, float lo, float hi, hipStream_t st);
int aesr_launch_lerp_multi(const float* z, float* out, int Z, size_t per, const float* alphas, int n, float nslope, hipStream_t st);
int aesr_launch_lerp_cat_bwd(const float* g, const float* af, const float* at, float* dz, int B, size_t per, hipStream_t st);
int aesr_launch_mse_fwd(const float* a, const float* b, double* partial, int np, float* out, size_t n, hipStream_t st);
int aesr_launch_mse3_fwd(const float* const* a, const float* const* b, const size_t* n, const float* lam, double* ws, float* out, hipStream_t st);
int aesr_launch_mse3_bwd(const float* a1, const float* b1, size_t n1, const float* a2, const float* b2, size_t n2, const float* lam,
                         const float* g, float* d1, float* d2, hipStream_t st);
int aesr_launch_mse_bwd(const float* a, const float* b, const float* g, float* da, size_t n, hipStream_t st);
int aesr_launch_act_bwd(const float* dout, const float* y, float* dpre, size_t n, int act, float slope, hipStream_t st);
int aesr_launch_adam(float* p, float* g, float* m, float* v, float* state, size_t n, float lr, double beta1, double beta2,
                     float eps, float wd, int zero_g, hipStream_t st);


int aesr_launch_maxpool2_fwd(const float* x, float* out, int N, int H, int W, int C, hipStream_t st);
int aesr_launch_maxpool2_bwd(const float* gout, const float* x, const float* gadd, float* dx, int N, int H, int W, int C, int relu, hipStream_t st);
int aesr_launch_lpips_tap_fwd(const float* f, const float* lin, float* partial, int B, int HW, int C, hipStream_t st);
int aesr_launch_lpips_tap_bwd(const float* f, const float* lin, const float* gd, float* gf0, int B, int HW, int C, hipStream_t st);
int aesr_launch_lpips_finalize(const float* const* partials, const int* hw, int ntaps, float* d, int B, hipStream_t st);
int aesr_launch_scale_expand(const float* x, float* out4, int n, const float* ca, const float* cb, int backward, hipStream_t st);
int aesr_launch_resample2(const float* x, const float* gout, const float* xsave, float* dst, int N, int H, int W, int C, int mode,
                          int backward, int mask_act, float slope, hipStream_t st);
size_t aesr_vif_workspace_bytes_impl(int Z, int H, int W);
int aesr_launch_vif_mscale(const float* ref, const float* dist, void* workspace, double* vif, int Z, int H, int W, const double* weights,
                           const int* radii, double sigma_nsq, hipStream_t st);
int aesr_launch_ssim_mse(const float* a, const float* b, double* partial, double* ssim, double* mse, int Z, int H, int W, int win,
                         double data_range, double k1, double k2, hipStream_t st);
int aesr_launch_long_axis_views(const float* ref, const float* rec, float* ref_view, float* rec_view, unsigned char* black, int Z, int H,
                                int W, int axis, hipStream_t st);
#define TRIPLET_MAX 64
struct TripletDesc { long long vol_off; int H, W, z_from, z_to, z_between, oy, ox, k; float gain, cutoff; };
struct TripletTable { TripletDesc d[TRIPLET_MAX]; };
int aesr_launch_triplet_assemble(const float* vol, const TripletTable& t, int B, int W, float* image, float* between, hipStream_t st);
int aesr_launch_s2d(const float* x, float* out, int N, int H, int W, int C, int inverse, hipStream_t st);

int aesr_launch_lap_blur5(const float* in, const float* add, float* out, int P, int H, int W, float gain, int adjoint, hipStream_t st);
int aesr_launch_lap_down2(const float* in, float* out, int P, int H, int W, hipStream_t st);
int aesr_launch_lap_zero_insert2(const float* in, float* out, int P, int h, int w, int H, int W, hipStream_t st);
int aesr_launch_l1_fwd(const float* a, const float* b, double* partial, int np, float* out, size_t n, hipStream_t st);
int aesr_launch_l1_bwd(const float* a, const float* b, const float* g, float* da, size_t n, hipStream_t st);
int aesr_launch_row_mean_fwd(const float* x, float* out, int N, size_t M, hipStream_t st);
int aesr_launch_row_mean_bwd(const float* g, float* dx, int N, size_t M, hipStream_t st);
```

superresolution_aniso_mri_amd/csrc/conv_thin.hip:

```cpp
#include "aesr_kernels.h"
#include "aesr_pack_dev.h"

#define THIN_TH 8
#ifndef THIN_ETH
#define THIN_ETH 16
#endif
#define THIN_XS 68

__host__ __device__ __forceinline__ int thin_tw(int C4) { return 256 / C4 < 64 ? 256 / C4 : 64; }

template <int TH = THIN_TH>
__device__ __forceinline__ void thin_stage(const ThinArgs& a, float (*xs)[THIN_XS], int n, int y0, int x0, int TW) {
    const int PW = TW + 2;
    for (int q = threadIdx.x; q < (TH + 2) * PW; q += 256) {
        const int r = q / PW, c = q - r * PW;
        const int sy = y0 + r - 1 - a.ps, sx = x0 + c - 1 - a.ps;
        float v = 0.f;
        if (sy >= 0 && sy < a.Hs && sx >= 0 && sx < a.Ws) v = a.s[((size_t)n * a.Hs + sy) * a.Ws + sx];
        xs[r][c] = v;
    }
}

__global__ __launch_bounds__(256) void thin_expand_kernel(ThinArgs a) {
    __shared__ float xs[THIN_ETH + 2][THIN_XS];
    const int C4 = a.C >> 2, TW = thin_tw(C4);
    const int tid = threadIdx.x, c4 = tid % C4, pl = tid / C4;
    int tile = blockIdx.x;
    const int tx = tile % a.tiles_x;
    tile /= a.tiles_x;
    const int ty = tile % a.tiles_y;
    const int n = tile / a.tiles_y;
    const int y0 = ty * THIN_ETH, x0 = tx * TW;
    thin_stage<THIN_ETH>(a, xs, n, y0, x0, TW);
    f32x4 w[9];
#pragma unroll
    for (int t = 0; t < 9; ++t) w[t] = *(const f32x4*)(a.w + t * a.C + c4 * 4);
    const f32x4 b0 = a.b ? *(const f32x4*)(a.b + c4 * 4) : (f32x4){0.f, 0.f, 0.f, 0.f};
    f32x4 bfull = b0;
    if (a.be) {
#pragma unroll
        for (int t = 0; t < 9; ++t) bfull += *(const f32x4*)(a.be + t * a.C + c4 * 4);
    }
    __syncthreads();
    const int ox = x0 + pl;
    if (pl >= TW || ox >= a.Wo) return;
    const bool xedge = a.be && (ox == 0 || ox == a.Wo - 1);
    const bool sigm = a.act == ACT_SIGMOID;
    const float nslope = a.act == ACT_LRELU ? a.slope : (a.act == ACT_RELU ? 0.f : 1.f);
    const bool fastact = !sigm && nslope >= 0.f && nslope <= 1.f;
#pragma unroll 4
    for (int r = 0; r < THIN_ETH; ++r) {
        const int oy = y0 + r;
        if (oy >= a.Ho) break;
        f32x4 acc = bfull;
        if (xedge || (a.be && (oy == 0 || oy == a.Ho - 1))) {
            acc = b0;
            for (int t = 0; t < 9; ++t) {
                const int yy = oy + t / 3 - 1, xx = ox + t % 3 - 1;
                if (yy >= 0 && yy < a.Ho && xx >= 0 && xx < a.Wo) acc += *(const f32x4*)(a.be + t * a.C + c4 * 4);
            }
        }
#pragma unroll
        for (int t = 0; t < 9; ++t) {
            const float v = xs[r + t / 3][pl + t % 3];
#pragma unroll
            for (int e = 0; e < 4; ++e) acc[e] = fmaf(w[t][e], v, acc[e]);
        }
        const size_t o = (((size_t)n * a.Ho + oy) * a.Wo + ox) * a.C + c4 * 4;
        if (fastact) {
#pragma unroll
            for (int e = 0; e < 4; ++e) acc[e] = fmaxf(acc[e], acc[e] * nslope);
        } else {
#pragma unroll
            for (int e = 0; e < 4; ++e) acc[e] = act_apply(acc[e], a.act, a.slope);
        }
        if (a.ysave) {
            const f32x4 ys = *(const f32x4*)(a.ysave + o);
#pragma unroll
            for (int e = 0; e < 4; ++e) acc[e] *= act_grad_from_output(ys[e], a.mask_act, a.slope);
        }
        *(f32x4*)(a.out + o) = acc;
    }
}

template <bool WITH_BE>
__global__ __launch_bounds__(256) void thin_reduce_kernel(ThinArgs a) {
    __shared__ float xs[THIN_TH + 2][THIN_XS];
    extern __shared__ __attribute__((aligned(16))) float red[];
    constexpr int NROW = WITH_BE ? 19 : 10;
    const int C4 = a.C >> 2, TW = thin_tw(C4);
    const int tid = threadIdx.x, c4 = tid % C4, pl = tid / C4;
    const int lane = tid & 63, wave = tid >> 6;
    f32x4 accW[9], accB[9];
    float accs = 0.f;
#pragma unroll
    for (int t = 0; t < 9; ++t) {
        accW[t] = (f32x4){0.f, 0.f, 0.f, 0.f};
        accB[t] = (f32x4){0.f, 0.f, 0.f, 0.f};
    }
    const int tpi = a.tiles_y * a.tiles_x;
    for (int tile = blockIdx.x; tile < a.ntiles; tile += gridDim.x) {
        const int n = tile / tpi;
        const int trem = tile - n * tpi;
        const int ty = trem / a.tiles_x, tx = trem - ty * a.tiles_x;
        const int y0 = ty * THIN_TH, x0 = tx * TW;
        __syncthreads();
        thin_stage(a, xs, n, y0, x0, TW);
        const int ox = x0 + pl;
        const bool xin = pl < TW && ox < a.Wo;
        const int plr = pl < TW ? pl : 0;
        f32x4 g[THIN_TH];
#pragma unroll
        for (int r = 0; r < THIN_TH; ++r) {
            const int oy = y0 + r;
            g[r] = (f32x4){0.f, 0.f, 0.f, 0.f};
            if (xin && oy < a.Ho) g[r] = *(const f32x4*)(a.t + (((size_t)n * a.Ho + oy) * a.Wo + ox) * a.C + c4 * 4);
        }
        float mxf[3];
        mxf[0] = (ox - 1 >= 0) ? 1.f : 0.f;
        mxf[1] = 1.f;
        mxf[2] = (ox + 1 < a.Wo) ? 1.f : 0.f;
        __syncthreads();
#pragma unroll
        for (int r = 0; r < THIN_TH; ++r) {
            const int oy = y0 + r;
#pragma unroll
            for (int t = 0; t < 9; ++t) {
                const float v = xs[r + t / 3][plr + t % 3];
#pragma unroll
                for (int e = 0; e < 4; ++e) accW[t][e] = fmaf(g[r][e], v, accW[t][e]);
            }
            if (WITH_BE) {
#pragma unroll
                for (int dy = 0; dy < 3; ++dy) {
                    const int yy = oy + dy - 1;
                    const float myf = (yy >= 0 && yy < a.Ho) ? 1.f : 0.f;
#pragma unroll
                    for (int dx = 0; dx < 3; ++dx) {
                        const float m = myf * mxf[dx];
#pragma unroll
                        for (int e = 0; e < 4; ++e) accB[dy * 3 + dx][e] = fmaf(g[r][e], m, accB[dy * 3 + dx][e]);
                    }
                }
            }
            if (c4 == 0 && xin && oy < a.Ho) accs += xs[r + 1][plr + 1];
        }
    }
    for (int m = C4; m < 64; m <<= 1) {
#pragma unroll
        for (int t = 0; t < 9; ++t)
#pragma unroll
            for (int e = 0; e < 4; ++e) {
                accW[t][e] += __shfl_xor(accW[t][e], m, 64);
                if (WITH_BE) accB[t][e] += __shfl_xor(accB[t][e], m, 64);
            }
    }
    for (int m = 1; m < 64; m <<= 1) accs += __shfl_xor(accs, m, 64);
    __syncthreads();
    if (lane < C4) {
        float* rw = red + (size_t)wave * NROW * a.C;
#pragma unroll
        for (int t = 0; t < 9; ++t) {
            *(f32x4*)(rw + t * a.C + c4 * 4) = accW[t];
            if (WITH_BE) *(f32x4*)(rw + (9 + t) * a.C + c4 * 4) = accB[t];
        }
        *(f32x4*)(rw + (NROW - 1) * a.C + c4 * 4) = (f32x4){c4 == 0 ? accs : 0.f, 0.f, 0.f, 0.f};
    }
    __syncthreads();
    const int nout = NROW * a.C;
    for (int o = tid; o < nout; o += 256)
        a.partial[(size_t)blockIdx.x * nout + o] =
            (red[o] + red[(size_t)nout + o]) + (red[2 * (size_t)nout + o] + red[3 * (size_t)nout + o]);
}

__global__ __launch_bounds__(256) void thin_collapse_kernel(const float* __restrict__ x, const float* __restrict__ w,
                                                            const float* __restrict__ bias, float* __restrict__ out, int N, int H,
                                                            int W, int C, int TH, int tiles_y, int tiles_x, int act, float slope) {
    __shared__ float S[2][3][4][64];
    const int C4 = C >> 2, TW = thin_tw(C4), TO = TW - 2;
    const int tid = threadIdx.x, c4 = tid % C4, pl = tid / C4;
    int tile = blockIdx.x;
    const int tx = tile % tiles_x;
    tile /= tiles_x;
    const int ty = tile % tiles_y;
    const int n = tile / tiles_y;
    const int y0 = ty * TH, x0 = tx * TO;
    const int xc = x0 - 1 + pl;
    const bool live = pl < TW && xc >= 0 && xc < W;
    f32x4 wq[9];
#pragma unroll
    for (int t = 0; t < 9; ++t)
#pragma unroll
        for (int e = 0; e < 4; ++e) wq[t][e] = w[(c4 * 4 + e) * 9 + t];
    const float b0 = bias ? bias[0] : 0.f;
    const f32x4 zero = {0.f, 0.f, 0.f, 0.f};
    const float* base = x + ((size_t)n * H * W + (live ? xc : 0)) * C + c4 * 4;
    auto load1 = [&](int yy) -> f32x4 {
        const f32x4 v = *(const f32x4*)(base + (size_t)min(max(yy, 0), H - 1) * W * C);
        return (live && yy >= 0 && yy < H) ? v : zero;
    };
    f32x4 r[6];
    r[0] = load1(y0 - 1);
    r[1] = load1(y0);
    int par = 0;
    for (int i = 0; i < TH; i += 4, par ^= 1) {
        const int oy = y0 + i;
        if (oy >= H) break;
#pragma unroll
        for (int k = 0; k < 4; ++k) r[2 + k] = load1(oy + 1 + k);
#pragma unroll
        for (int k = 0; k < 4; ++k) {
            float sk[3];
#pragma unroll
            for (int kx = 0; kx < 3; ++kx) {
                f32x4 acc = zero;
#pragma unroll
                for (int ky = 0; ky < 3; ++ky)
#pragma unroll
                    for (int e = 0; e < 4; ++e) acc[e] = fmaf(wq[ky * 3 + kx][e], r[k + ky][e], acc[e]);
                sk[kx] = (acc[0] + acc[1]) + (acc[2] + acc[3]);
            }
            for (int m = 1; m < C4; m <<= 1) {
                sk[0] += __shfl_xor(sk[0], m, 64);
                sk[1] += __shfl_xor(sk[1], m, 64);
                sk[2] += __shfl_xor(sk[2], m, 64);
            }
            if (c4 == 0 && pl < TW) {
                S[par][0][k][pl] = sk[0];
                S[par][1][k][pl] = sk[1];
                S[par][2][k][pl] = sk[2];
            }
        }
        __syncthreads();
        for (int o = tid; o < 4 * TO; o += 256) {
            const int k = o / TO, j = o - k * TO;
            const int xo = x0 + j, yo = oy + k;
            if (xo < W && yo < H && i + k < TH) {
                const float v = (S[par][0][k][j] + S[par][1][k][j + 1]) + S[par][2][k][j + 2];
                out[((size_t)n * H + yo) * W + xo] = act_apply(v + b0, act, slope);
            }
        }
        r[0] = r[4];
        r[1] = r[5];
    }
}


__global__ __launch_bounds__(256) void thin_stem_fold_kernel(const float* __restrict__ ws, const float* __restrict__ bs,
                                                             const float* __restrict__ w1, float* __restrict__ folded, int Cs,
                                                             int C1) {
    stem_fold_elements(ws, bs, w1, folded, Cs, C1, blockIdx.x * 256 + threadIdx.x, gridDim.x * 256);
}

__global__ __launch_bounds__(256) void thin_stem_finish_kernel(const float* __restrict__ R, const float* __restrict__ ws,
                                                               const float* __restrict__ bs, const float* __restrict__ w1,
                                                               float* __restrict__ dws, float* __restrict__ dbs,
                                                               float* __restrict__ dw1, float* __restrict__ db1, int Cs, int C1) {
    __shared__ double redw[256], redb[256];
    if ((int)blockIdx.x < Cs) {
        const int c = blockIdx.x;
        double sw = 0.0, sb = 0.0;
        for (int o = threadIdx.x; o < C1 * 9; o += 256) {
            const int co = o / 9, t = o - co * 9;
            const double wv = (double)w1[((size_t)co * Cs + c) * 9 + t];
            sw += wv * (double)R[t * C1 + co];
            sb += wv * (double)R[(9 + t) * C1 + co];
        }
        redw[threadIdx.x] = sw;
        redb[threadIdx.x] = sb;
        __syncthreads();
        for (int h = 128; h > 0; h >>= 1) {
            if ((int)threadIdx.x < h) {
                redw[threadIdx.x] += redw[threadIdx.x + h];
                redb[threadIdx.x] += redb[threadIdx.x + h];
            }
            __syncthreads();
        }
        if (threadIdx.x == 0) {
            dws[c] = (float)redw[0];
            if (dbs) dbs[c] = (float)redb[0];
        }
        return;
    }
    const int tid = (blockIdx.x - Cs) * 256 + threadIdx.x, nth = (gridDim.x - Cs) * 256;
    for (int o = tid; o < C1 * Cs * 9; o += nth) {
        const int t = o % 9, c = (o / 9) % Cs, co = o / (9 * Cs);
        float v = R[t * C1 + co] * ws[c];
        if (bs) v = fmaf(R[(9 + t) * C1 + co], bs[c], v);
        dw1[o] = v;
    }
    if (db1)
        for (int co = tid; co < C1; co += nth) db1[co] = R[(9 + 4) * C1 + co];
}

__global__ __launch_bounds__(256) void thin_cout1_flip_kernel(const float* __restrict__ w, float* __restrict__ wexp, int Cin) {
    cout1_flip_elements(w, wexp, Cin, blockIdx.x * 256 + threadIdx.x, gridDim.x * 256);
}

__global__ __launch_bounds__(256) void thin_cout1_finish_kernel(const float* __restrict__ R, float* __restrict__ dw,
                                                                float* __restrict__ db, int Cin) {
    for (int o = blockIdx.x * 256 + threadIdx.x; o < 9 * Cin; o += gridDim.x * 256) {
        const int ci = o / 9, k = o - ci * 9;
        dw[o] = R[(8 - k) * Cin + ci];
    }
    if (db && blockIdx.x == 0 && threadIdx.x == 0) db[0] = R[9 * Cin];
}


static bool thin_shape_ok(const ThinArgs& a) {
    const int C4 = a.C / 4;
    return a.C >= 4 && a.C % 4 == 0 && a.C <= 256 && (C4 & (C4 - 1)) == 0;
}

int aesr_launch_thin_expand(ThinArgs a, hipStream_t st) {
    if (!thin_shape_ok(a)) {
        aesr_set_error("thin conv: C=%d must be 4 times a power of two (4..256)", a.C);
        return AESR_ERR_ARG;
    }
    const int TW = thin_tw(a.C / 4);
    a.tiles_y = ceil_div(a.Ho, THIN_ETH);
    a.tiles_x = ceil_div(a.Wo, TW);
    a.ntiles = a.N * a.tiles_y * a.tiles_x;
    hipLaunchKernelGGL(thin_expand_kernel, dim3(a.ntiles), dim3(256), 0, st, a);
    AESR_LAUNCH_CHECK("thin_expand");
    return AESR_OK;
}

int aesr_launch_thin_reduce(ThinArgs a, int nwg, hipStream_t st) {
    if (!thin_shape_ok(a)) {
        aesr_set_error("thin conv: C=%d must be 4 times a power of two (4..256)", a.C);
        return AESR_ERR_ARG;
    }
    const int TW = thin_tw(a.C / 4);
    a.tiles_y = ceil_div(a.Ho, THIN_TH);
    a.tiles_x = ceil_div(a.Wo, TW);
    a.ntiles = a.N * a.tiles_y * a.tiles_x;
    const int nrow = a.with_be ? 19 : 10;
    const size_t shmem = (size_t)4 * nrow * a.C * sizeof(float);
    if (a.with_be)
        hipLaunchKernelGGL(thin_reduce_kernel<true>, dim3(nwg), dim3(256), shmem, st, a);
    else
        hipLaunchKernelGGL(thin_reduce_kernel<false>, dim3(nwg), dim3(256), shmem, st, a);
    AESR_LAUNCH_CHECK("thin_reduce");
    return AESR_OK;
}

int aesr_launch_thin_collapse(const float* x, const float* w, const float* bias, float* out, int N, int H, int W, int C, int act,
                              float slope, hipStream_t st) {
    const int C4 = C / 4;
    if (C < 4 || C % 4 != 0 || C > 256 || (C4 & (C4 - 1)) != 0) {
        aesr_set_error("thin conv: C=%d must be 4 times a power of two (4..256)", C);
        return AESR_ERR_ARG;
    }
    const int TW = thin_tw(C4), TH = H < 20 ? H : 20;
    const int tiles_y = ceil_div(H, TH), tiles_x = ceil_div(W, TW - 2);
    hipLaunchKernelGGL(thin_collapse_kernel, dim3(N * tiles_y * tiles_x), dim3(256), 0, st, x, w, bias, out, N, H, W, C, TH, tiles_y,
                       tiles_x, act, slope);
    AESR_LAUNCH_CHECK("thin_collapse");
    return AESR_OK;
}

int aesr_launch_thin_stem_fold(const float* ws, const float* bs, const float* w1, float* folded, int Cs, int C1, hipStream_t st) {
    hipLaunchKernelGGL(thin_stem_fold_kernel, dim3(ceil_div(9 * C1, 256)), dim3(256), 0, st, ws, bs, w1, folded, Cs, C1);
    AESR_LAUNCH_CHECK("thin_stem_fold");
    return AESR_OK;
}

int aesr_launch_thin_stem_finish(const float* R, const float* ws, const float* bs, const float* w1, float* dws, float* dbs,
                                 float* dw1, float* db1, int Cs, int C1, hipStream_t st) {
    int grid = ceil_div(C1 * Cs * 9, 256);
    if (grid > 64) grid = 64;
    hipLaunchKernelGGL(thin_stem_finish_kernel, dim3(Cs + grid), dim3(256), 0, st, R, ws, bs, w1, dws, dbs, dw1, db1, Cs, C1);
    AESR_LAUNCH_CHECK("thin_stem_finish");
    return AESR_OK;
}

int aesr_launch_thin_cout1_flip(const float* w, float* wexp, int Cin, hipStream_t st) {
    hipLaunchKernelGGL(thin_cout1_flip_kernel, dim3(ceil_div(9 * Cin, 256)), dim3(256), 0, st, w, wexp, Cin);
    AESR_LAUNCH_CHECK("thin_cout1_flip");
    return AESR_OK;
}

int aesr_launch_thin_cout1_finish(const float* R, float* dw, float* db, int Cin, hipStream_t st) {
    hipLaunchKernelGGL(thin_cout1_finish_kernel, dim3(ceil_div(9 * Cin, 256)), dim3(256), 0, st, R, dw, db, Cin);
    AESR_LAUNCH_CHECK("thin_cout1_finish");
    return AESR_OK;
}
```

superresolution_aniso_mri_amd/csrc/conv_wgrad.hip:

```cpp
#include "aesr_kernels.h"

#define WG_NX(nwco) ((nwco) == 4 ? 4 : 6)
#define WG_ND(nwco) ((nwco) == 4 ? 5 : 6)

template <int KS, int NWCO>
__global__ __launch_bounds__(256) __attribute__((amdgpu_waves_per_eu(3, 3))) void conv_wgrad_f32(WgradArgs a) {
    constexpr int CIBW = (NWCO == 2) ? 1 : 2;
    constexpr int CIT = 32, COT = 16 * NWCO;
    constexpr int XPAIRS = CIT / 8, DPAIRS = COT / 8;
    constexpr int NX = WG_NX(NWCO), ND = WG_ND(NWCO);
    extern __shared__ __attribute__((aligned(16))) float lds[];
    const int tid = threadIdx.x, lane = tid & 63;
    const int wave = __builtin_amdgcn_readfirstlane(tid >> 6);
    const int l15 = lane & 15, g = lane >> 4;
    const int wco = (NWCO == 2) ? (wave >> 1) : wave;
    const int wci = (NWCO == 2) ? (wave & 1) : 0;
    const int nci = a.CinP / CIT, nchunks = nci * (a.CoutP / COT);
    int chunk, split;
    if ((a.S & 7) == 0) {
        const int xcd = blockIdx.x & 7, local = blockIdx.x >> 3;
        chunk = local % nchunks;
        split = (local / nchunks) * 8 + xcd;
    } else {
        chunk = blockIdx.x % nchunks;
// ... 67 lines not shown
        }
    };

    long long st[5] = {0, 0, 0, 0, 0}, t0 = 0, t1;
#define WG_STAMP(i)                                   \
    if (a.dbgbuf) {                                   \
        t1 = __builtin_amdgcn_s_memtime();            \
        st[i] += t1 - t0;                             \
        t0 = t1;                                      \
    }
    int tile = split;
    if (tile < a.ntiles) issue_loads(tile);
    if (a.dbgbuf) t0 = __builtin_amdgcn_s_memtime();
    while (tile < a.ntiles) {
#pragma unroll
        for (int k = 0; k < NX; ++k)
            if (xlds[k] >= 0) {
                float* d = ldsX + xlds[k];
                d[0] = RX[k][0];
                d[PSX] = RX[k][1];
                d[2 * PSX] = RX[k][2];
                d[3 * PSX] = RX[k][3];
            }
#pragma unroll
        for (int k = 0; k < ND; ++k)
            if (dlds[k] >= 0) {
                float* d = ldsD + dlds[k];
                d[0] = RD[k][0];
                d[PSD] = RD[k][1];
                d[2 * PSD] = RD[k][2];
                d[3 * PSD] = RD[k][3];
            }
        WG_STAMP(0)
        __syncthreads();
        WG_STAMP(1)
        const int next = tile + a.S;
        if (next < a.ntiles) issue_loads(next);
        __builtin_amdgcn_sched_barrier(0);
        WG_STAMP(2)
        {
            constexpr int NSTEP = KS * CIBW;
            const int gpr = a.TW >> 3, ngrp = a.TH * gpr;
            int r = 0, cg = 0;
            float2 dv = *(const float2*)(ldsD + dbase);
            float2 e01 = *(const float2*)(ldsX + xbase0), e23 = e01;
            if (KS > 1) e23 = *(const float2*)(ldsX + xbase0 + 2);
            for (int gi = 0; gi < ngrp; ++gi) {
                const int c0 = cg * 8;
                int rn = r, cgn = cg + 1;
                if (cgn == gpr) { cgn = 0; rn = r + 1; }
                if (gi + 1 == ngrp) { rn = r; cgn = cg; }
                float2 dvn = dv;
#pragma unroll
                for (int st_ = 0; st_ < NSTEP; ++st_) {
                    const int ky = st_ / CIBW, i = st_ % CIBW;
                    const float* xn;
                    if (st_ + 1 < NSTEP) {
                        const int kyn = (st_ + 1) / CIBW, in_ = (st_ + 1) % CIBW;
                        xn = ldsX + xbase0 + in_ * 16 * PSX + (r + kyn) * PWS + c0;
                    } else {
                        xn = ldsX + xbase0 + rn * PWS + cgn * 8;
                        dvn = *(const float2*)(ldsD + dbase + rn * TWS + cgn * 8);
                    }
                    const float2 n01 = *(const float2*)xn;
                    float2 n23 = n01;
                    if (KS > 1) n23 = *(const float2*)(xn + 2);
                    __builtin_amdgcn_sched_barrier(0);
                    const float e[4] = {e01.x, e01.y, e23.x, e23.y};
#pragma unroll
                    for (int kx = 0; kx < KS; ++kx)
                        acc[ky * KS + kx][i] = __builtin_amdgcn_mfma_f32_16x16x4f32(e[kx], dv.x, acc[ky * KS + kx][i], 0, 0, 0);
#pragma unroll
                    for (int kx = 0; kx < KS; ++kx)
                        acc[ky * KS + kx][i] = __builtin_amdgcn_mfma_f32_16x16x4f32(e[kx + 1], dv.y, acc[ky * KS + kx][i], 0, 0, 0);
                    __builtin_amdgcn_sched_barrier(0);
                    e01 = n01;
                    e23 = n23;
                }
                accb += dv.x + dv.y;
                dv = dvn;
                r = rn;
                cg = cgn;
            }
        }
        WG_STAMP(3)
        __syncthreads();
        WG_STAMP(4)
        tile = next;
    }
#undef WG_STAMP
    if (a.dbgbuf && tid == 0)
        for (int i = 0; i < 5; ++i) a.dbgbuf[blockIdx.x * 5 + i] = (float)st[i];

    const size_t plane = (size_t)a.CinP * a.CoutP;
    float* sl = a.slab + (size_t)split * (KS * KS + 1) * plane;
    const int co = co0 + wco * 16 + l15;
#pragma unroll
    for (int t = 0; t < KS * KS; ++t)
#pragma unroll
        for (int i = 0; i < CIBW; ++i)
#pragma unroll
            for (int e = 0; e < 4; ++e) {
                const int ci = ci0 + (wci * CIBW + i) * 16 + g * 4 + e;
                sl[t * plane + (size_t)ci * a.CoutP + co] = acc[t][i][e];
            }
    accb += __shfl_xor(accb, 16, 64);
    accb += __shfl_xor(accb, 32, 64);
    if (do_bias && g == 0) sl[(KS * KS) * plane + co] = accb;
}

__global__ __launch_bounds__(256) void wgrad_reduce_kernel(const float* __restrict__ slab, float* __restrict__ dw,
                                                           float* __restrict__ db, int nslab, int KS2, int Cin, int CinP,
                                                           int Cout, int CoutP) {
    __shared__ float red[4][64];
    const int o = blockIdx.x * 64 + (threadIdx.x & 63);
    const int sl = threadIdx.x >> 6;
    const int nw = KS2 * Cin * Cout;
    const int total = nw + (db ? Cout : 0);
    float s = 0.f;
    size_t off = 0;
    const bool live = o < total;
    int co = 0, ci = 0, tap = 0;
    if (live) {
        if (o < nw) {
            co = o % Cout;
            const int rest = o / Cout;
            ci = rest % Cin;
            tap = rest / Cin;
            off = ((size_t)tap * CinP + ci) * CoutP + co;
        } else {
            off = (size_t)KS2 * CinP * CoutP + (o - nw);
        }
        const size_t stride = (size_t)(KS2 + 1) * CinP * CoutP;
        float s0 = 0.f, s1 = 0.f, s2 = 0.f, s3 = 0.f;
        int k = sl;
        for (; k + 12 < nslab; k += 16) {
            s0 += slab[(size_t)k * stride + off];
            s1 += slab[(size_t)(k + 4) * stride + off];
            s2 += slab[(size_t)(k + 8) * stride + off];
            s3 += slab[(size_t)(k + 12) * stride + off];
        }
        for (; k < nslab; k += 4) s0 += slab[(size_t)k * stride + off];
        s = (s0 + s1) + (s2 + s3);
    }
    red[sl][threadIdx.x & 63] = s;
    __syncthreads();
    if (sl == 0 && live) {
        s = (red[0][threadIdx.x] + red[1][threadIdx.x]) + (red[2][threadIdx.x] + red[3][threadIdx.x]);
        if (o < nw) dw[((size_t)co * Cin + ci) * KS2 + tap] = s;
        else db[o - nw] = s;
    }
}

__global__ __launch_bounds__(256) void wgrad_reduce_many_kernel(ReduceTable t) {
    __shared__ float red[4][64];
    int j = 0;
    for (int k = 1; k < t.njobs; ++k)
        if ((int)blockIdx.x >= t.job[k].block0) j = k;
    const ReduceJob& jb = t.job[j];
    const int o = ((int)blockIdx.x - jb.block0) * 64 + (threadIdx.x & 63);
    const int sl = threadIdx.x >> 6;
    const int nw = jb.KS2 * jb.Cin * jb.Cout;
    const int total = nw + (jb.db ? jb.Cout : 0);
    float s = 0.f;
    size_t off = 0;
    const bool live = o < total;
    int co = 0, ci = 0, tap = 0;
    if (live) {
        if (o < nw) {
            co = o % jb.Cout;
            const int rest = o / jb.Cout;
            ci = rest % jb.Cin;
            tap = rest / jb.Cin;
            off = ((size_t)tap * jb.CinP + ci) * jb.CoutP + co;
        } else {
            off = (size_t)jb.KS2 * jb.CinP * jb.CoutP + (o - nw);
        }
        const size_t stride = (size_t)(jb.KS2 + 1) * jb.CinP * jb.CoutP;
        float s0 = 0.f, s1 = 0.f, s2 = 0.f, s3 = 0.f;
        int k = sl;
        for (; k + 12 < jb.nslab; k += 16) {
            s0 += jb.slab[(size_t)k * stride + off];
            s1 += jb.slab[(size_t)(k + 4) * stride + off];
            s2 += jb.slab[(size_t)(k + 8) * stride + off];
            s3 += jb.slab[(size_t)(k + 12) * stride + off];
        }
        for (; k < jb.nslab; k += 4) s0 += jb.slab[(size_t)k * stride + off];
        s = (s0 + s1) + (s2 + s3);
    }
    red[sl][threadIdx.x & 63] = s;
    __syncthreads();
    if (sl == 0 && live) {
        s = (red[0][threadIdx.x] + red[1][threadIdx.x]) + (red[2][threadIdx.x] + red[3][threadIdx.x]);
        if (o < nw) jb.dw[((size_t)co * jb.Cin + ci) * jb.KS2 + tap] = s;
        else jb.db[o - nw] = s;
    }
}

int aesr_launch_wgrad_reduce_many(const ReduceTable& t, hipStream_t st) {
    hipLaunchKernelGGL(wgrad_reduce_many_kernel, dim3(t.nblocks), dim3(256), 0, st, t);
    AESR_LAUNCH_CHECK("wgrad_reduce_many");
    return AESR_OK;
}

template <int KS, int NWCO>
static int launch_wgrad(const WgradArgs& a, hipStream_t st) {
    constexpr int COT = 16 * NWCO;
    const size_t shmem = ((size_t)32 * a.PSX + (size_t)COT * a.PSD) * sizeof(float);
    if (shmem > 160 * 1024) {
        aesr_set_error("conv_wgrad: tile needs %zu B of LDS", shmem);
        return AESR_ERR_ARG;
    }
    if ((a.TH + KS - 1) * (a.TW + KS - 1) * 8 > 256 * WG_NX(NWCO) || a.TH * a.TW * (COT / 4) > 256 * WG_ND(NWCO)) {
        aesr_set_error("conv_wgrad: tile %dx%d does not fit the register prefetch slots", a.TH, a.TW);
        return AESR_ERR_ARG;
    }
    static bool attr_set[AESR_MAX_DEVICES] = {};
    int dev_ = 0;
    if (hipGetDevice(&dev_) != hipSuccess || dev_ < 0 || dev_ >= AESR_MAX_DEVICES) dev_ = 0;
    if (!attr_set[dev_]) {
        const hipError_t e_ = hipFuncSetAttribute((const void*)conv_wgrad_f32<KS, NWCO>, hipFuncAttributeMaxDynamicSharedMemorySize, 160 * 1024);
        if (e_ != hipSuccess) {
            aesr_set_error("conv_wgrad_f32: hipFuncSetAttribute(MaxDynamicSharedMemorySize = 160 KB) failed: %s", hipGetErrorString(e_));
            return AESR_ERR_HIP;
        }
        attr_set[dev_] = true;
    }
    dim3 grid(a.S * (a.CinP / 32) * (a.CoutP / COT));
    if (getenv("AESR_WGRAD_DBG")) {
        static float* dbuf = nullptr;
        if (!dbuf) (void)hipMalloc(&dbuf, 4096 * 5 * sizeof(float));
        WgradArgs b = a;
        b.dbgbuf = grid.x <= 4096 ? dbuf : nullptr;
        hipLaunchKernelGGL((conv_wgrad_f32<KS, NWCO>), grid, dim3(256), shmem, st, b);
        (void)hipStreamSynchronize(st);
        static float host[4096 * 5];
        (void)hipMemcpy(host, dbuf, grid.x * 5 * sizeof(float), hipMemcpyDeviceToHost);
        double s5[5] = {0, 0, 0, 0, 0};
        for (unsigned i = 0; i < grid.x; ++i) for (int k = 0; k < 5; ++k) s5[k] += host[i * 5 + k];
        fprintf(stderr, "[wgrad stamps] grid=%u tiles=%d tile=%dx%d per-WG kcycles: lds-write %.1f | barrier1 %.1f | issue-loads %.1f | mfma %.1f | barrier2 %.1f\n",
                grid.x, a.ntiles, a.TH, a.TW, s5[0] / grid.x / 1e3, s5[1] / grid.x / 1e3, s5[2] / grid.x / 1e3, s5[3] / grid.x / 1e3, s5[4] / grid.x / 1e3);
        return AESR_OK;
    }
    hipLaunchKernelGGL((conv_wgrad_f32<KS, NWCO>), grid, dim3(256), shmem, st, a);
    AESR_LAUNCH_CHECK("conv_wgrad_f32");
    return AESR_OK;
}

int aesr_launch_conv_wgrad(const WgradArgs& a, int KS, int variant, hipStream_t st) {
    if ((size_t)a.N * a.H * a.W * a.Cin >= (size_t)0x1C000000 || (size_t)a.N * a.Ho * a.Wo * a.Cout >= (size_t)0x1C000000) {
        aesr_set_error("conv_wgrad: tensors of 469M elements (1.75 GB) or more need 64-bit indexing (not built)");
        return AESR_ERR_UNSUPPORTED;
    }
    if (a.TW % 8 != 0 || (a.PWS & 1) || (a.TWS & 1) || (a.PSX & 1) || (a.PSD & 1)) {
        aesr_set_error("conv_wgrad: TW=%d must be a multiple of 8 and strides even", a.TW);
        return AESR_ERR_ARG;
    }
#define WG_CASE(ks, v, nwco) \
    if (KS == ks && variant == v) return launch_wgrad<ks, nwco>(a, st);
    WG_CASE(3, 0, 2) WG_CASE(3, 1, 4) WG_CASE(1, 0, 2) WG_CASE(1, 1, 4)
#undef WG_CASE
    aesr_set_error("conv_wgrad: no instantiation for KS=%d variant=%d", KS, variant);
    return AESR_ERR_UNSUPPORTED;
}

int aesr_launch_wgrad_reduce(const float* slab, float* dw, float* db, int nslab, int KS, int Cin, int CinP, int Cout,
                             int CoutP, hipStream_t st) {
    const int total = KS * KS * Cin * Cout + (db ? Cout : 0);
    hipLaunchKernelGGL(wgrad_reduce_kernel, dim3(ceil_div(total, 64)), dim3(256), 0, st, slab, dw, db, nslab, KS * KS, Cin,
                       CinP, Cout, CoutP);
    AESR_LAUNCH_CHECK("wgrad_reduce");
    return AESR_OK;
}
```

superresolution_aniso_mri_amd/csrc/conv_wgrad_wino.hip:

```cpp
#include <stdio.h>
#include <stdlib.h>

#include <type_traits>
#include <utility>

#include "aesr_kernels.h"

constexpr int WW_OOB = 0x70000000;
typedef float f32x2 __attribute__((ext_vector_type(2)));
#ifndef WW_ABL
#define WW_ABL 0
#endif

template <int... I, class F>
__device__ __forceinline__ void ww_for(std::integer_sequence<int, I...>, F&& f) {
    (f(std::integral_constant<int, I>{}), ...);
}
template <int N, class F>
__device__ __forceinline__ void ww_rep(F&& f) { ww_for(std::make_integer_sequence<int, N>{}, f); }

__device__ __forceinline__ void ww_dma(__amdgpu_buffer_rsrc_t rs, float* lds_wave_base, int byte_off) {
    __builtin_amdgcn_raw_ptr_buffer_load_lds(rs, (__attribute__((address_space(3))) void*)lds_wave_base, 16, byte_off, 0, 0, 0);
}

// ... 30 lines not shown
    extern __shared__ __attribute__((aligned(16))) float lds[];
    const int tid = threadIdx.x, lane = tid & 63;
    const int wave = __builtin_amdgcn_readfirstlane(tid >> 6);
    const int l15 = lane & 15, g = lane >> 4;
    const int nci = a.CinP / CIT, nchunks = nci * (a.CoutP / COT);
    int chunk, split;
    if ((a.S & 7) == 0) {
        const int xcd = blockIdx.x & 7, local = blockIdx.x >> 3;
        chunk = local % nchunks;
        split = (local / nchunks) * 8 + xcd;
    } else {
        chunk = blockIdx.x % nchunks;
        split = blockIdx.x / nchunks;
    }
    const int ciy = chunk % nci, coz = chunk / nci;
    const int ci0 = ciy * CIT, co0 = coz * COT;
    float* const ldsX0 = lds;
    float* const ldsD0 = lds + 2 * XFL;
    const bool do_bias = ciy == 0;

    const int sh = a.x_up2 ? 1 : 0;
    const int xH = a.H >> sh, xW = a.W >> sh;
    const int ximg = xH * xW * a.Cin * 4, dimg = a.H * a.W * a.Cout * 4;
    const int xrow = xW * a.Cin * 4, drow = a.W * a.Cout * 4;
    const int sgx = wave % SPR, rx0 = wave / SPR, sgd = wave % SPRD, rd0 = wave / SPRD;
    const int pxl = lane >> 3, pos = lane & 7;
    const int quad = pos ^ (((pxl >> 1) & 1) << 2);
    const int pcx = 8 * sgx + pxl, pcd = 8 * sgd + pxl;
    const int lcx = (((pcx - sh) >> sh) * a.Cin + ci0 + 4 * quad) * 4;
    const int lcd = (pcd * a.Cout + co0 + 4 * quad) * 4;
    const int tpi = a.tiles_y * a.tiles_x;
    const int dS_n = a.S / tpi, dS_r = a.S - dS_n * tpi, dS_ty = dS_r / a.tiles_x, dS_tx = dS_r - dS_ty * a.tiles_x;
    auto advance = [&](WwTile t) {
        t.tx += dS_tx;
        if (t.tx >= a.tiles_x) { t.tx -= a.tiles_x; ++t.ty; }
        t.ty += dS_ty;
        if (t.ty >= a.tiles_y) { t.ty -= a.tiles_y; ++t.n; }
        t.n += dS_n;
        return t;
    };
    auto fetch = [&](const WwTile& t, int buf) {
        const bool valid = t.n < a.N;
        const int n = valid ? t.n : 0, y0 = t.ty * TH, x0 = t.tx * TW;
        const __amdgpu_buffer_rsrc_t rs_x = __builtin_amdgcn_make_buffer_rsrc((void*)((const char*)a.x + (size_t)n * ximg), 0, valid ? ximg : 0, 0x00020000);
        const __amdgpu_buffer_rsrc_t rs_d = __builtin_amdgcn_make_buffer_rsrc((void*)((const char*)a.dy + (size_t)n * dimg), 0, valid ? dimg : 0, 0x00020000);
        const unsigned gxx = (unsigned)(x0 - 1 + pcx), gxd = (unsigned)(x0 + pcd);
        const int offx = (pcx < TW + 2 && gxx < (unsigned)a.W) ? lcx + ((x0 >> sh) - 1 + sh) * a.Cin * 4 : WW_OOB;
        const int offd = gxd < (unsigned)a.W ? lcd + x0 * a.Cout * 4 : WW_OOB;
        const int r0 = y0 - 1 + rx0;
        int ux = (r0 >> sh) * xrow;
        const int step_odd = sh == 0 ? RXS * xrow : RXS == 2 ? xrow : (r0 & 1) * xrow;
        const int step_even = sh == 0 ? RXS * xrow : RXS == 2 ? xrow : xrow - step_odd;
        float* const xdst = ldsX0 + buf * XFL + (rx0 * PWL + 8 * sgx) * 32;
        int uxk[NXS];
        ww_rep<NXS>([&](auto Kc) {
            constexpr int k = decltype(Kc)::value;
            if constexpr (k > 0) ux += (k & 1) ? step_odd : step_even;
            uxk[k] = ux;
        });
        if (pcx < TW + 2) {
            ww_rep<NXS>([&](auto Kc) {
                constexpr int k = decltype(Kc)::value;
                ww_dma(rs_x, xdst + k * RXS * PWL * 32, offx + uxk[k]);
            });
        }
        int ud = (y0 + rd0) * drow;
        float* const ddst = ldsD0 + buf * DFL + (rd0 * TWL + 8 * sgd) * 32;
        ww_rep<NDS>([&](auto Kc) {
            constexpr int k = decltype(Kc)::value;
            if constexpr (k > 0) ud += RDS * drow;
            ww_dma(rs_d, ddst + k * RDS * TWL * 32, offd + ud);
        });
    };

    f32x4 acc[16][2][2];
#pragma unroll
    for (int x = 0; x < 16; ++x)
#pragma unroll
        for (int i = 0; i < 2; ++i)
#pragma unroll
            for (int o = 0; o < 2; ++o) acc[x][i][o] = (f32x4){0.f, 0.f, 0.f, 0.f};
    float accb[2] = {0.f, 0.f};

    const int sw = (g & 1) << 2;
    const int chA = (((l15 >> 2) ^ sw) << 2) + (l15 & 3);
    const int chB = (((l15 >> 2) ^ sw ^ 4) << 2) + (l15 & 3);
    const unsigned lds0 = (unsigned)(unsigned long long)lds;
    unsigned lx[2][4], ld[2][2];
#pragma unroll
    for (int i = 0; i < 2; ++i) {
#pragma unroll
        for (int c = 0; c < 4; ++c) lx[i][c] = lds0 + (unsigned)(((2 * g + c) * 32 + ((c < 2 ? chA : chB) ^ (i ? 16 : 0))) * 4);
#pragma unroll
        for (int e = 0; e < 2; ++e) ld[i][e] = lds0 + (unsigned)((2 * XFL + (2 * g + e) * 32 + (chA ^ (i ? 16 : 0))) * 4);
    }

    f32x2 Vp[2][2][2][4], Mp[2][2][8];
    f32x2 P[2][4][2];
    auto op_read = [&](int xu, int du, int nb) {
        ww_rep<8>([&](auto Kc) {
            constexpr int i = decltype(Kc)::value >> 2, c = decltype(Kc)::value & 3;
            const unsigned ad = lx[i][c] + (unsigned)(xu * 4);
            f32x2 &p0_ = P[i][c][0], &p1_ = P[i][c][1];
            asm volatile("ds_read2st64_b32 %0, %2 offset0:%3 offset1:%4\n\tds_read2st64_b32 %1, %2 offset0:%5 offset1:%6"
                         : "=&v"(p0_), "=&v"(p1_) : "v"(ad), "n"(0), "n"(PWL / 2), "n"(PWL), "n"(3 * PWL / 2) : "memory");
        });
        ww_rep<4>([&](auto Kc) {
            constexpr int o = decltype(Kc)::value >> 1, e = decltype(Kc)::value & 1;
            const unsigned ad = ld[o][e] + (unsigned)(du * 4);
            f32x2& y_ = Mp[nb][o][e];
            asm volatile("ds_read2st64_b32 %0, %1 offset0:0 offset1:%2" : "=&v"(y_) : "v"(ad), "n"(TWL / 2) : "memory");
        });
    };
    auto op_transform = [&](int nb) {
        asm volatile("s_waitcnt lgkmcnt(0)" ::: "memory");
        ww_rep<2>([&](auto Ic) {
            constexpr int i = decltype(Ic)::value;
            f32x2 T[2][4];
            ww_rep<4>([&](auto Cc) {
                constexpr int c = decltype(Cc)::value;
                WW_PK(T[0][c], P[i][c][0], P[i][c][1], WW_M_T01);
                WW_PK(T[1][c], P[i][c][0], P[i][c][1], WW_M_T23);
            });
            ww_rep<2>([&](auto Sc) {
                constexpr int s_ = decltype(Sc)::value;
                WW_PK(Vp[nb][i][s_][0], T[s_][0], T[s_][2], WW_M_SUB);
                WW_PK(Vp[nb][i][s_][1], T[s_][1], T[s_][2], WW_M_ADD);
                WW_PK(Vp[nb][i][s_][2], T[s_][2], T[s_][1], WW_M_SUB);
                WW_PK(Vp[nb][i][s_][3], T[s_][1], T[s_][3], WW_M_SUB);
            });
        });
        ww_rep<2>([&](auto Oc) {
            constexpr int o = decltype(Oc)::value;
            WW_PK(Mp[nb][o][2], Mp[nb][o][0], Mp[nb][o][0], WW_M_SELF);
            WW_PK(Mp[nb][o][3], Mp[nb][o][1], Mp[nb][o][1], WW_M_SELF);
            WW_PK(Mp[nb][o][4], Mp[nb][o][0], Mp[nb][o][1], WW_M_LL);
            WW_PK(Mp[nb][o][7], Mp[nb][o][0], Mp[nb][o][1], WW_M_HH);
            WW_PK(Mp[nb][o][5], Mp[nb][o][2], Mp[nb][o][3], WW_M_LL);
            WW_PK(Mp[nb][o][6], Mp[nb][o][2], Mp[nb][o][3], WW_M_HH);
            accb[o] += Mp[nb][o][5][0];
        });
    };
    auto mfmas = [&](auto Q0c, auto Nc, int cb) {
        ww_rep<decltype(Nc)::value>([&](auto Dc) {
            constexpr int q = decltype(Q0c)::value + decltype(Dc)::value, x = q >> 2, i = (q >> 1) & 1, o = q & 1;
            constexpr int r = x >> 2, k = x & 3;
            constexpr int mi = k == 0 ? (r == 0 || r == 3 ? 0 : 2) : k == 3 ? (r == 0 || r == 3 ? 1 : 3) : 4 + r;
            constexpr int mh = k == 0 || k == 3 ? (r >= 2 ? 1 : 0) : k - 1;
            f32x4& acc_ = acc[x][i][o];
            const float va_ = Vp[cb][i][r >> 1][k][r & 1], vb_ = Mp[cb][o][mi][mh];
            asm volatile("v_mfma_f32_16x16x4_f32 %0, %1, %2, %0" : "+a"(acc_) : "v"(va_), "v"(vb_));
        });
    };
    auto step_xu = [&](int j, int buf) { const int ks = wave + 4 * j, tyl = ks / KPR, kx = ks - tyl * KPR; return buf * XFL + ((2 * tyl) * PWL + 8 * kx) * 32; };
    auto step_du = [&](int j, int buf) { const int ks = wave + 4 * j, tyl = ks / KPR, kx = ks - tyl * KPR; return buf * DFL + ((2 * tyl) * TWL + 8 * kx) * 32; };
    using C0 = std::integral_constant<int, 0>;
    using C16 = std::integral_constant<int, 16>;
    using C32 = std::integral_constant<int, 32>;

    long long tph[3] = {0, 0, 0}, tq = 0;
#define WW_STAMP(k)                                                   \
    if constexpr (STAMP) {                                            \
        const long long t_ = (long long)__builtin_amdgcn_s_memtime(); \
        tph[k] += t_ - tq;                                            \
        tq = t_;                                                      \
    }
    if constexpr (STAMP) tq = (long long)__builtin_amdgcn_s_memtime();

    WwTile t0, t1, t2;
    {
        t0.n = split / tpi;
        const int rem = split - t0.n * tpi;
        t0.ty = rem / a.tiles_x;
        t0.tx = rem - t0.ty * a.tiles_x;
        if (split >= a.ntiles) t0.n = a.N;
    }
    t1 = advance(t0);
    t2 = advance(t1);
    fetch(t0, 0);
    fetch(t1, 1);
    asm volatile("s_waitcnt vmcnt(0)" ::: "memory");
    __syncthreads();
    int buf = 0;
    op_read(step_xu(0, 0), step_du(0, 0), 0);
    op_transform(0);
    WW_STAMP(2)
    if (t0.n < a.N) do {
        __builtin_amdgcn_sched_barrier(0);
#if WW_ABL != 3 && WW_ABL != 4
        op_read(step_xu(1, buf), step_du(1, buf), 1);
#endif
        mfmas(C0{}, C16{}, 0);
#if WW_ABL != 2 && WW_ABL != 4
        op_transform(1);
#endif
        mfmas(C16{}, std::integral_constant<int, 48>{}, 0);
        __builtin_amdgcn_sched_barrier(0);
        WW_STAMP(0)
        asm volatile("s_waitcnt vmcnt(0) lgkmcnt(0)" ::: "memory");
        __syncthreads();
        WW_STAMP(1)
        __builtin_amdgcn_sched_barrier(0);
#if WW_ABL != 3 && WW_ABL != 4
        op_read(step_xu(0, buf ^ 1), step_du(0, buf ^ 1), 0);
#endif
        mfmas(C0{}, C16{}, 1);
        __builtin_amdgcn_sched_barrier(0);
#if WW_ABL != 1 && WW_ABL != 4
        fetch(t2, buf);
#endif
        __builtin_amdgcn_sched_barrier(0);
        mfmas(C16{}, C16{}, 1);
#if WW_ABL != 2 && WW_ABL != 4
        op_transform(0);
#endif
        mfmas(C32{}, C32{}, 1);
        __builtin_amdgcn_sched_barrier(0);
        t0 = t1;
        t1 = t2;
        t2 = advance(t2);
        buf ^= 1;
    } while (t0.n < a.N);
    WW_STAMP(0)
    asm volatile("s_waitcnt vmcnt(0) lgkmcnt(0)" ::: "memory");
    __syncthreads();
    if (STAMP && lane == 0)
        for (int k = 0; k < 3; ++k) a.dbgbuf[(blockIdx.x * 4 + wave) * 3 + k] = (float)tph[k];

    f32x4 dg[9][2][2];
#pragma unroll
    for (int i = 0; i < 2; ++i)
#pragma unroll
        for (int o = 0; o < 2; ++o) {
            f32x4 R[3][4];
#pragma unroll
            for (int j = 0; j < 4; ++j) {
                const f32x4 u0_ = acc[0 + j][i][o], u1 = acc[4 + j][i][o], u2 = acc[8 + j][i][o], u3 = -acc[12 + j][i][o];
                const f32x4 s = j == 3 ? (f32x4){-1.f, -1.f, -1.f, -1.f} : (f32x4){1.f, 1.f, 1.f, 1.f};
                R[0][j] = s * (u0_ + 0.5f * (u1 + u2));
                R[1][j] = s * (0.5f * (u1 - u2));
                R[2][j] = s * (0.5f * (u1 + u2) + u3);
            }
#pragma unroll
            for (int r = 0; r < 3; ++r) {
                dg[r * 3 + 0][i][o] = R[r][0] + 0.5f * (R[r][1] + R[r][2]);
                dg[r * 3 + 1][i][o] = 0.5f * (R[r][1] - R[r][2]);
                dg[r * 3 + 2][i][o] = 0.5f * (R[r][1] + R[r][2]) + R[r][3];
            }
        }
#pragma unroll
    for (int o = 0; o < 2; ++o) {
        accb[o] += __shfl_xor(accb[o], 16, 64);
        accb[o] += __shfl_xor(accb[o], 32, 64);
    }
    f32x4* ex = (f32x4*)lds;
    float* exb = lds + 4 * 36 * 64 * 4;
#pragma unroll
    for (int t = 0; t < 9; ++t)
#pragma unroll
        for (int i = 0; i < 2; ++i)
#pragma unroll
            for (int o = 0; o < 2; ++o) ex[(wave * 36 + (t * 4 + i * 2 + o)) * 64 + lane] = dg[t][i][o];
    if (g == 0) {
        exb[wave * 32 + l15] = accb[0];
        exb[wave * 32 + 16 + l15] = accb[1];
    }
    __syncthreads();
    const size_t plane = (size_t)a.CinP * a.CoutP;
    float* sl = a.slab + (size_t)split * 10 * plane;
#pragma unroll
    for (int q = 0; q < 9; ++q) {
        const int blk = wave * 9 + q;
        const int t = blk >> 2, i = (blk >> 1) & 1, o = blk & 1;
        f32x4 v = ex[(0 * 36 + blk) * 64 + lane];
#pragma unroll
        for (int w = 1; w < 4; ++w) v += ex[(w * 36 + blk) * 64 + lane];
        const int co = co0 + o * 16 + l15;
#pragma unroll
        for (int e = 0; e < 4; ++e) {
            const int ci = ci0 + i * 16 + g * 4 + e;
            sl[t * plane + (size_t)ci * a.CoutP + co] = v[e];
        }
    }
    if (wave == 0 && do_bias && g == 0) {
#pragma unroll
        for (int o = 0; o < 2; ++o) {
            float bsum = exb[0 * 32 + o * 16 + l15];
#pragma unroll
            for (int w = 1; w < 4; ++w) bsum += exb[w * 32 + o * 16 + l15];
            sl[9 * plane + co0 + o * 16 + l15] = bsum;
        }
    }
}

size_t aesr_wgrad_wino_lds_bytes(int TH, int TW) {
    const size_t xfl = (size_t)(TH + 2) * (TW == 8 ? 16 : 32) * 32, dfl = (size_t)TH * TW * 32;
    const size_t bufs = 2 * (xfl + dfl) * sizeof(float);
    const size_t exch = ((size_t)4 * 36 * 64 * 4 + 4 * 32) * sizeof(float);
    return bufs > exch ? bufs : exch;
}

bool aesr_wgrad_wino_tile_ok(int TH, int TW) { return (TH == 16 && TW == 8) || (TH == 8 && TW == 16); }

template <int TH, int TW>
static int launch_wgrad_wino(const WgradArgs& a, hipStream_t st) {
    const size_t shmem = aesr_wgrad_wino_lds_bytes(TH, TW);
    static bool attr_set[AESR_MAX_DEVICES] = {};
    int dev_ = 0;
    if (hipGetDevice(&dev_) != hipSuccess || dev_ < 0 || dev_ >= AESR_MAX_DEVICES) dev_ = 0;
    if (!attr_set[dev_]) {
        const hipError_t e_ = hipFuncSetAttribute((const void*)conv_wgrad_wino_f32<TH, TW, false>, hipFuncAttributeMaxDynamicSharedMemorySize, 160 * 1024);
        if (e_ == hipSuccess) (void)hipFuncSetAttribute((const void*)conv_wgrad_wino_f32<TH, TW, true>, hipFuncAttributeMaxDynamicSharedMemorySize, 160 * 1024);
        if (e_ != hipSuccess) {
            aesr_set_error("conv_wgrad_wino_f32: hipFuncSetAttribute(MaxDynamicSharedMemorySize = 160 KB) failed: %s", hipGetErrorString(e_));
            return AESR_ERR_HIP;
        }
        attr_set[dev_] = true;
    }
    dim3 grid(a.S * (a.CinP / 32) * (a.CoutP / 32));
    if (getenv("AESR_WGRAD_WINO_DBG") && grid.x <= 4096) {
        static float* dbuf = nullptr;
        if (!dbuf) (void)hipMalloc(&dbuf, 4096 * 4 * 3 * sizeof(float));
        WgradArgs b = a;
        b.dbgbuf = dbuf;
        hipLaunchKernelGGL((conv_wgrad_wino_f32<TH, TW, true>), grid, dim3(256), shmem, st, b);
        (void)hipStreamSynchronize(st);
        static float host[4096 * 4 * 3];
        (void)hipMemcpy(host, dbuf, (size_t)grid.x * 4 * 3 * sizeof(float), hipMemcpyDeviceToHost);
        double s3[3] = {0, 0, 0};
        for (unsigned i = 0; i < grid.x * 4; ++i) for (int k = 0; k < 3; ++k) s3[k] += host[i * 3 + k];
        const double visits = (double)((a.ntiles + a.S - 1) / a.S);
        const int nks = (TH >> 1) * (TW >> 3);
        fprintf(stderr, "[wgrad-wino stamps] grid=%u tile %dx%d S=%d (%.0f visits, %d k-steps = %d MFMA cycles per wave and visit) per visit, cycles: "
                "k-step loop %.0f | barrier %.0f || fill %.0f\n", grid.x, TH, TW, a.S, visits, nks, nks / 4 * 64 * 32,
                s3[0] / grid.x / 4 / visits, s3[1] / grid.x / 4 / visits, s3[2] / grid.x / 4);
        return AESR_OK;
    }
    hipLaunchKernelGGL((conv_wgrad_wino_f32<TH, TW, false>), grid, dim3(256), shmem, st, a);
    AESR_LAUNCH_CHECK("conv_wgrad_wino_f32");
    return AESR_OK;
}

int aesr_launch_conv_wgrad_wino(const WgradArgs& a, hipStream_t st) {
    if ((size_t)a.H * a.W * a.Cin * 4 >= (size_t)0x10000000 || (size_t)a.H * a.W * a.Cout * 4 >= (size_t)0x10000000) {
        aesr_set_error("conv_wgrad_wino: images of 256 MB or more need 64-bit lane offsets (not built)");
        return AESR_ERR_UNSUPPORTED;
    }
    if (a.x_up2 && ((a.H | a.W) & 1)) {
        aesr_set_error("conv_wgrad_wino: the folded Upsample(x2) needs even convolution sizes (got %dx%d)", a.H, a.W);
        return AESR_ERR_ARG;
    }
    if (!aesr_wgrad_wino_tile_ok(a.TH, a.TW) || a.pad != 1 || a.Ho != a.H || a.Wo != a.W) {
        aesr_set_error("conv_wgrad_wino: tile %dx%d is not 16x8 or 8x16 (or not 3x3 / padding 1)", a.TH, a.TW);
        return AESR_ERR_ARG;
    }
    if (a.CinP % 32 != 0 || a.CoutP % 32 != 0 || a.Cin != a.CinP || a.Cout != a.CoutP || a.S < 1 || a.S > a.ntiles ||
        a.tiles_y != ceil_div(a.H, a.TH) || a.tiles_x != ceil_div(a.W, a.TW) || a.ntiles != a.N * a.tiles_y * a.tiles_x) {
        aesr_set_error("conv_wgrad_wino: channel counts must be multiples of 32 and the tile grid consistent (S=%d, %d tiles)", a.S, a.ntiles);
        return AESR_ERR_ARG;
    }
    if (a.TH == 16) return launch_wgrad_wino<16, 8>(a, st);
    return launch_wgrad_wino<8, 16>(a, st);
}
```

superresolution_aniso_mri_amd/engine.py:

```python
import os
from ctypes import c_float

import torch
import torch.nn as nn

from . import _hip
from ._hip import lib, ptr, stream, check

LRELU_SLOPE = 0.01


class KernelProfiler:

    def __init__(self):
        self.records = []

    def begin(self, kind, flops, nbytes=0.0):
        e0 = torch.cuda.Event(enable_timing=True)
        e1 = torch.cuda.Event(enable_timing=True)
        e0.record(torch.cuda.current_stream())
        self.records.append((kind, flops, nbytes, e0, e1))

    def end(self):
        self.records[-1][4].record(torch.cuda.current_stream())
# ... 416 lines not shown
                                            _hip.int_array(nstart), stream()), "aesr_bn_apply")
                _pe()
                if save:
                    saved.append((cur, st))
                cur, H, W = out, Ho, Wo
        return cur, saved, steps

    def max_elems_per_image(self, H, W, C, first=0, last=None):
        return self.trace_shapes(H, W, C, first, last)[0]

    def trace_shapes(self, H, W, C, first=0, last=None):
        best = H * W * C
        for s in self.steps[first:last]:
            if s.kind == "conv":
                if s.s2d:
                    H, W = H // 2, W // 2
                elif s.in_up2:
                    H, W = 2 * H, 2 * W
                    H, W = s.out_hw(H, W)
                else:
                    H, W = s.out_hw(H, W)
                C = s.cout
            elif s.kind == "stemconv":
                H, W = s.out_hw(H, W)
                C = s.cout
            else:
                H, W = s.out_hw(H, W)
            best = max(best, H * W * C)
        return best, (H, W, C)

    def _bn_barrier(self, dev):
        t = self.__dict__.get("_bn_bar")
        if t is None or t.device != torch.device(dev):
            if torch.cuda.is_current_stream_capturing():
                raise RuntimeError("one-launch BatchNorm: run the pass eagerly once before capturing it into a HIP graph")
            t = self._bn_bar = torch.zeros((int(lib.aesr_bn_fused1_barrier_words()),), device=dev, dtype=torch.int32)
        return t

    sync_p2p = None

    def _p2p_fits(self, N, H, W, C, run_mode, G, backward):
        p = self.sync_p2p
        if p is None or not bn_fused_enabled():
            return False
        nmax = max(N, int(round(N * p.nscale)))
        if float(nmax) * H * W * C * 4.0 > float(os.environ.get("AESR_P2P_MAX_MB", "12")) * 1e6:
            return False
        return bool(lib.aesr_bn_fused1_supported(nmax, H, W, C, run_mode, G, backward))

    sync_bn = None
    count_scale = 1.0

    def _bn_forward_stats(self, bn, y, N, H, W, C, nstart, train, out=None, run_mode=0):
        G = len(nstart) - 1
        dev = y.device
        st = {k: torch.empty((G, C), device=dev, dtype=torch.float32) for k in ("mean", "invstd", "scale", "shift")}
        use_batch = train or bn.running_mean is None
        momentum = 0.1 if bn.momentum is None else float(bn.momentum)
        update = bool(train and bn.track_running_stats and bn.running_mean is not None)
        if update:
            self._bn_updates = getattr(self, "_bn_updates", 0) + 1
        if not use_batch:
            ver = lambda t: (-1, 0) if t is None else (t._version, t.data_ptr())
            key = (self.weights_epoch, getattr(self, "_bn_updates", 0), ver(bn.weight), ver(bn.bias), ver(bn.running_mean), ver(bn.running_var),
                   G, str(dev))
            cache = self.__dict__.setdefault("_eval_bn", {})
            hit = cache.get(id(bn))
            if hit is not None and hit[0] == key and not torch.cuda.is_current_stream_capturing():
                return dict(hit[1])
        sums = counts = None
        if use_batch:
            partial = torch.empty((G * _hip.BN_NWG * 2 * C,), device=dev, dtype=torch.float32)
            counts = [float((nstart[g + 1] - nstart[g]) * H * W) * self.count_scale for g in range(G)]
            st["counts"] = counts
            if (self.sync_bn is None and out is not None and bn_fused_enabled() and bn_fused_pays(N, H, W, C)
                    and lib.aesr_bn_fused1_supported(N, H, W, C, run_mode, G, 0)):
                ws = torch.empty((lib.aesr_bn_fused1_workspace_floats(C, G),), device=dev, dtype=torch.float32)
                check(lib.aesr_bn_fused1_fwd(ptr(y), ptr(out), ptr(ws), ptr(self._bn_barrier(dev)), _hip.double_array(counts), ptr(bn.weight),
                                             ptr(bn.bias), ptr(bn.running_mean), ptr(bn.running_var), ptr(bn.num_batches_tracked),
                                             ptr(st["mean"]), ptr(st["invstd"]), ptr(st["scale"]), ptr(st["shift"]), N, H, W, C, run_mode, G,
                                             _hip.int_array(nstart), momentum, float(bn.eps), int(update), stream()), "aesr_bn_fused1_fwd")
                st["applied"] = True
                return st
            if self.sync_bn is not None and out is not None and self._p2p_fits(N, H, W, C, run_mode, G, 0):
                p = self.sync_p2p
                ws = torch.empty((lib.aesr_bn_fused1_workspace_floats(C, G),), device=dev, dtype=torch.float32)
                check(lib.aesr_bn_fused1_fwd_p2p(ptr(y), ptr(out), ptr(ws), ptr(self._bn_barrier(dev)), _hip.double_array(counts), ptr(bn.weight),
                                                 ptr(bn.bias), ptr(bn.running_mean), ptr(bn.running_var), ptr(bn.num_batches_tracked),
                                                 ptr(st["mean"]), ptr(st["invstd"]), ptr(st["scale"]), ptr(st["shift"]), N, H, W, C, run_mode, G,
                                                 _hip.int_array(nstart), momentum, float(bn.eps), int(update), p.peers, p.world, p.rank,
                                                 p.next_slot(), ptr(p.gen), stream()), "aesr_bn_fused1_fwd_p2p")
                st["applied"] = True
                return st
            if self.sync_bn is None:
                check(lib.aesr_bn_stats_finalize(ptr(y), ptr(partial), _hip.double_array(counts), ptr(bn.weight), ptr(bn.bias),
                                                 ptr(bn.running_mean), ptr(bn.running_var), ptr(bn.num_batches_tracked),
                                                 ptr(st["mean"]), ptr(st["invstd"]), ptr(st["scale"]), ptr(st["shift"]), H * W, C,
                                                 G, _hip.int_array(nstart), momentum, float(bn.eps), int(update), stream()),
                      "aesr_bn_stats_finalize")
                return st
            sums = torch.empty((G, 2, C), device=dev, dtype=torch.float64)
            check(lib.aesr_bn_stats(ptr(y), ptr(partial), ptr(sums), H * W, C, G, _hip.int_array(nstart), stream()),
                  "aesr_bn_stats")
            self.sync_bn(sums)
            if out is not None and lib.aesr_bn_fused_supported(C, G):
                st["counts"] = counts
                check(lib.aesr_bn_finalize_apply(ptr(sums), _hip.double_array(counts), ptr(bn.weight), ptr(bn.bias), ptr(bn.running_mean),
                                                 ptr(bn.running_var), ptr(bn.num_batches_tracked), ptr(st["mean"]), ptr(st["invstd"]),
                                                 ptr(st["scale"]), ptr(st["shift"]), ptr(y), ptr(out), N, H, W, C, run_mode, G,
                                                 _hip.int_array(nstart), momentum, float(bn.eps), int(update), stream()),
                      "aesr_bn_finalize_apply")
                st["applied"] = True
                return st
        st["counts"] = counts
        check(lib.aesr_bn_finalize(ptr(sums), _hip.double_array(counts) if counts else None, ptr(bn.weight), ptr(bn.bias), ptr(bn.running_mean),
                                   ptr(bn.running_var), ptr(bn.num_batches_tracked), ptr(st["mean"]), ptr(st["invstd"]),
                                   ptr(st["scale"]), ptr(st["shift"]), C, G, momentum, float(bn.eps), int(use_batch),
                                   int(update), stream()), "aesr_bn_finalize")
        if not use_batch and not torch.cuda.is_current_stream_capturing():
            self.__dict__.setdefault("_eval_bn", {})[id(bn)] = (key, dict(st))
        return st

    @staticmethod
    def _grad_dst(p, grads):
        if p.grad is not None and getattr(p, "_aesr_grad_fresh", False) and p.grad.is_contiguous():
            p._aesr_grad_fresh = False
            grads[p] = None
            return p.grad
        t = torch.empty_like(p)
        grads[p] = t
        return t

    def backward(self, gout, saved, nstart, ngrad, need_input_grad, steps=None):
        steps = self.steps if steps is None else steps
        grads = {}
        G = 0
        while G < len(nstart) - 1 and nstart[G + 1] <= ngrad:
            G += 1
        if G == 0 or nstart[G] != ngrad:
            raise RuntimeError("the images that need gradients must be whole leading statistic groups")
        ns = list(nstart[:G + 1])
        g = gout[:ngrad]
        if not g.is_contiguous():
            g = g.contiguous()
        reduce_jobs = []
        g = self._backward_steps(steps, saved, g, ngrad, need_input_grad, grads, G, ns, reduce_jobs)
        if _DEFERRED is not None:
            _DEFERRED.extend(j for j in reduce_jobs if j[4])
            flush_wgrad_reductions([j for j in reduce_jobs if not j[4]])
        else:
            flush_wgrad_reductions(reduce_jobs)
        return g, grads

    def _backward_steps(self, steps, saved, g, ngrad, need_input_grad, grads, G, ns, reduce_jobs):
        for k in range(len(steps) - 1, -1, -1):
            s = steps[k]
            if s.kind == "stemconv":
                if need_input_grad:
                    raise RuntimeError("the stem-folded pass has no input gradient (run the pass with fused=False)")
                xin = saved[k][0]
                _, H, W, _ = xin.shape
                dws, dbs = self._grad_dst(s.stem.weight, grads), self._grad_dst(s.stem.bias, grads)
                dw1 = self._grad_dst(s.mod.weight, grads)
                db1 = self._grad_dst(s.mod.bias, grads) if s.mod.bias is not None else None
                ws = _empty((lib.aesr_stemconv_workspace_floats(s.cout),), g)
                _pb("thin_reduce", 0.0, 4.0 * (ngrad * H * W + g.numel()))
                check(lib.aesr_stemconv_wgrad(ptr(xin), ptr(g), ptr(s.stem.weight), ptr(s.stem.bias), ptr(s.mod.weight),
                                              ptr(dws), ptr(dbs), ptr(dw1), ptr(db1), ptr(ws), ngrad, H, W, s.cs, s.cout,
                                              s.stem_pad, stream()), "aesr_stemconv_wgrad")
                _pe()
                g = None
                break
            if s.kind == "conv":
                xin, yout = saved[k][0], saved[k][1]
                N, H, W, _ = xin.shape
                N = ngrad
                if s.in_up2:
                    H, W = 2 * H, 2 * W
                Ho, Wo = (H, W) if s.s2d else s.out_hw(H, W)
                if k == len(steps) - 1 and s.act != _hip.ACT_NONE:
                    dpre = torch.empty_like(g)
                    check(lib.aesr_act_bwd(ptr(g), ptr(yout), ptr(dpre), g.numel(), s.act, s.slope, stream()), "aesr_act_bwd")
                    g = dpre
                dw_final = self._grad_dst(s.mod.weight, grads)
                dw = torch.empty((s.cout, s.cin, 1, 1), device=g.device) if s.s2d else dw_final
                db = self._grad_dst(s.mod.bias, grads) if s.mod.bias is not None else None
                if s.cin % 4 == 0 and s.cout % 4 == 0:
                    nws = lib.aesr_conv2d_wgrad_workspace_floats(N, H, W, s.cin, s.cout, s.ks, s.pad)
                    ws = _empty((nws,), g)
                    if s.s2d:
                        _pb(("wgrad", s.cin, s.cout, s.ks, s.pad), 2.0 * N * Ho * Wo * s.cout * s.ks * s.ks * s.cin)
                        check(lib.aesr_conv2d_wgrad(ptr(xin), ptr(g), ptr(dw), ptr(db), ptr(ws), N, H, W, s.cin, s.cout, s.ks,
                                                    s.pad, stream()), "aesr_conv2d_wgrad")
                        _pe()
                    else:
                        _pb(("wgrad", s.cin, s.cout, s.ks, s.pad), 2.0 * N * Ho * Wo * s.cout * s.ks * s.ks * s.cin)
                        check(lib.aesr_conv2d_wgrad_partial(ptr(xin), ptr(g), ptr(ws), N, H, W, s.cin, s.cout, s.ks, s.pad,
                                                            int(s.in_up2), stream()), "aesr_conv2d_wgrad_partial")
                        _pe()
                        direct = grads[s.mod.weight] is None and (db is None or grads[s.mod.bias] is None)
                        reduce_jobs.append((_hip.WgradReduceJob(ws.data_ptr(), dw.data_ptr(), db.data_ptr() if db is not None else None,
                                                                N, H, W, s.cin, s.cout, s.ks, s.pad), ws, dw, db, direct))
                elif s.cin <= 4 and s.ks == 1 and db is not None:
                    ws = _empty((lib.aesr_small_wgrad_workspace_floats(s.cout * (s.cin + 1)),), g)
                    check(lib.aesr_conv2d_smallcin_wgrad(ptr(xin), ptr(g), ptr(dw), ptr(db), ptr(ws), N, H, W, s.cin, s.cout,
                                                         s.pad, stream()), "aesr_conv2d_smallcin_wgrad")
                elif s.cout == 1 and s.ks == 3 and s.pad == 1 and db is not None:
                    ws = _empty((lib.aesr_conv2d_cout1_workspace_floats(s.cin),), g)
                    _pb("thin_reduce", 0.0, 4.0 * (N * H * W * s.cin + g.numel()))
                    check(lib.aesr_conv2d_cout1_wgrad(ptr(xin), ptr(g), ptr(dw), ptr(db), ptr(ws), N, H, W, s.cin, stream()),
                          "aesr_conv2d_cout1_wgrad")
                    _pe()
                else:
                    raise NotImplementedError("no wgrad kernel for conv %d->%d k%d" % (s.cin, s.cout, s.ks))
                if s.s2d:
                    dw_final.copy_(dw.reshape(s.cout, 2, 2, s.cin_full).permute(0, 3, 1, 2))
                if k == 0 and not need_input_grad:
                    g = None
                    break
                mask, mask_act, mslope = None, _hip.ACT_NONE, 0.0
                if k > 0 and steps[k - 1].kind in ("conv", "stemconv"):
                    mask, mask_act, mslope = saved[k - 1][1], steps[k - 1].act, steps[k - 1].slope
                    if mask_act == _hip.ACT_NONE:
                        mask = None
                dx = _empty((N, H // 2, W // 2, s.cin) if s.in_up2 else (N, H, W, s.cin), g)
                if s.in_up2:
                    _pb(("wino", N, H, W, s.cin, s.cout, 1), 2.0 * N * H * W * s.cin * 9 * s.cout)
                    check(lib.aesr_conv2d_wino_dgrad_sum2(ptr(g), ptr(s.packed_wt), ptr(dx), N, H, W, s.cin, s.cout, stream()),
                          "aesr_conv2d_wino_dgrad_sum2")
                    _pe()
                elif s.cin <= 4 and mask is None:
                    check(lib.aesr_conv2d_smallcin_dgrad(ptr(g), ptr(s.mod.weight), ptr(dx), N, H, W, s.cin, s.cout, s.ks,
                                                         s.pad, 0, None, stream()), "aesr_conv2d_smallcin_dgrad")
                elif s.wino_dgrad:
                    _pb(("wino", N, H, W, s.cin, s.cout, 1), 2.0 * N * H * W * s.cin * 9 * s.cout)
                    ws, nws = wino_workspace(g, N, H, W, s.cin, s.cout, 1)
                    check(lib.aesr_conv2d_wino_dgrad_ws(ptr(g), ptr(s.packed_wt), ptr(mask), ptr(dx), ptr(ws), nws, N, H, W, s.cin, s.cout,
                                                        mask_act, mslope, stream()), "aesr_conv2d_wino_dgrad_ws")
                    _pe()
                elif s.cout % 4 == 0:
                    _pb("conv_igemm_f32", 2.0 * N * H * W * s.cin * s.ks * s.ks * s.cout)
                    nws = lib.aesr_conv2d_dgrad_workspace_floats(N, H, W, s.cin, s.cout, s.ks, s.pad)
                    ws = _empty((nws,), g) if nws else None
                    check(lib.aesr_conv2d_dgrad_ws(ptr(g), ptr(s.packed_t), ptr(mask), ptr(dx), ptr(ws), N, H, W, s.cin, s.cout,
                                                   s.ks, s.pad, mask_act, mslope, stream()), "aesr_conv2d_dgrad_ws")
                    _pe()
                elif s.cout == 1 and s.ks == 3 and s.pad == 1 and _thin_channels(s.cin):
                    w = s.mod.weight
                    if s.flipped is not None and s.packed_epoch == (self.weights_epoch, w._version, w.data_ptr()):
                        _pb("thin_expand", 0.0, 4.0 * (g.numel() + dx.numel() * (2 if mask is not None else 1)))
                        check(lib.aesr_conv2d_cout1_dgrad_pre(ptr(g), ptr(s.flipped), ptr(mask), ptr(dx), N, H, W, s.cin, mask_act, mslope,
                                                              stream()), "aesr_conv2d_cout1_dgrad_pre")
                        _pe()
                    else:
                        wsf = _empty((9 * s.cin,), g)
                        check(lib.aesr_conv2d_cout1_dgrad(ptr(g), ptr(w), ptr(mask), ptr(dx), ptr(wsf), N, H, W, s.cin,
                                                          mask_act, mslope, stream()), "aesr_conv2d_cout1_dgrad")
                elif s.cout <= 4:
                    check(lib.aesr_conv2d_smallcin_fwd(ptr(g), ptr(s.mod.weight), None, ptr(mask), ptr(dx), N, Ho, Wo, s.cout,
                                                       s.cin, s.ks, s.ks - 1 - s.pad, _hip.ACT_NONE, mask_act, mslope, 1, 0,
                                                       None, None, stream()), "aesr_conv2d_smallcin_fwd(dgrad)")
                else:
                    raise NotImplementedError("no dgrad kernel for conv %d->%d" % (s.cin, s.cout))
                if s.s2d:
                    if mask is not None:
                        raise NotImplementedError("activation mask in front of a stride-2 convolution")
                    fh, fw = saved[k][2]
                    dfull = _empty((N, fh, fw, s.cin_full), g)
                    check(lib.aesr_depth_to_space2(ptr(dx), ptr(dfull), N, fh, fw, s.cin_full, stream()), "aesr_depth_to_space2")
                    dx = dfull
                g = dx
            elif s.kind == "resample":
                xin = saved[k][0]
                _, H, W, C = xin.shape
                prev = steps[k - 1]
                mask_act, mslope = (prev.act, prev.slope) if prev.kind in ("conv", "stemconv") else (_hip.ACT_NONE, 0.0)
                dx = _empty((ngrad, H, W, C), g)
                check(lib.aesr_resample2_bwd(ptr(g), ptr(xin) if mask_act != _hip.ACT_NONE else None, ptr(dx), ngrad, H, W, C,
                                             s.mode, mask_act, mslope, stream()), "aesr_resample2_bwd")
                g = dx
            else:
                y, st = saved[k]
                prev = steps[k - 1]
                _, H, W, C = y.shape
                N = ngrad
                dev = y.device
                partial = torch.empty((G * _hip.BN_NWG * 2 * C,), device=dev, dtype=torch.float32)
                nsa = _hip.int_array(ns)
                coef = torch.empty((G, 2, C), device=dev, dtype=torch.float32)
                dgamma, dbeta = self._grad_dst(s.mod.weight, grads), self._grad_dst(s.mod.bias, grads)
                dpre = _empty((N, H, W, C), y)
                _pb("bn_bwd", 0.0, 4.0 * (g.numel() + 2.0 * N * H * W * C))
                if (self.sync_bn is None and bn_fused_enabled() and bn_fused_pays(N, H, W, C)
                        and lib.aesr_bn_fused1_supported(N, H, W, C, s.run_mode, G, 1)):
                    ws = torch.empty((lib.aesr_bn_fused1_workspace_floats(C, G),), device=dev, dtype=torch.float32)
                    check(lib.aesr_bn_fused1_bwd(ptr(g), ptr(y), ptr(st["mean"]), ptr(st["invstd"]), ptr(st["scale"]), ptr(ws),
                                                 ptr(self._bn_barrier(dev)), _hip.double_array(st["counts"][:G]), ptr(coef), ptr(dgamma), ptr(dbeta),
                                                 ptr(dpre), N, H, W, C, s.run_mode, prev.act, prev.slope, G, nsa, stream()), "aesr_bn_fused1_bwd")
                elif self.sync_bn is not None and self._p2p_fits(N, H, W, C, s.run_mode, G, 1):
                    p = self.sync_p2p
                    ws = torch.empty((lib.aesr_bn_fused1_workspace_floats(C, G),), device=dev, dtype=torch.float32)
                    check(lib.aesr_bn_fused1_bwd_p2p(ptr(g), ptr(y), ptr(st["mean"]), ptr(st["invstd"]), ptr(st["scale"]), ptr(ws),
                                                     ptr(self._bn_barrier(dev)), _hip.double_array(st["counts"][:G]), ptr(coef), ptr(dgamma),
                                                     ptr(dbeta), ptr(dpre), N, H, W, C, s.run_mode, prev.act, prev.slope, G, nsa, p.peers, p.world,
                                                     p.rank, p.next_slot(), ptr(p.gen), stream()), "aesr_bn_fused1_bwd_p2p")
                elif self.sync_bn is None:
                    check(lib.aesr_bn_bwd(ptr(g), ptr(y), ptr(st["mean"]), ptr(st["invstd"]), ptr(st["scale"]), ptr(partial),
                                          _hip.double_array(st["counts"][:G]), ptr(coef), ptr(dgamma), ptr(dbeta), ptr(dpre), N, H, W,
                                          C, s.run_mode, prev.act, prev.slope, G, nsa, stream()), "aesr_bn_bwd")
                else:
                    sums = torch.empty((G, 2, C), device=dev, dtype=torch.float64)
                    check(lib.aesr_bn_bwd_reduce(ptr(g), ptr(y), ptr(st["mean"]), ptr(st["invstd"]), ptr(partial), ptr(sums), N,
                                                 H, W, C, s.run_mode, G, nsa, stream()), "aesr_bn_bwd_reduce")
                    self.sync_bn(sums)
                    check(lib.aesr_bn_bwd_apply(ptr(g), ptr(y), ptr(st["mean"]), ptr(st["invstd"]), ptr(st["scale"]), ptr(sums),
                                                _hip.double_array(st["counts"][:G]), ptr(coef), ptr(dgamma), ptr(dbeta), ptr(dpre),
                                                N, H, W, C, s.run_mode, prev.act, prev.slope, G, nsa, stream()), "aesr_bn_bwd_apply")
                _pe()
                g = dpre
        return g


def prepare_weights(pairs):
    jobs, commits = [], []
    for runner, steps in pairs:
        j, c = runner._prep_jobs(steps)
        jobs += j
        commits += c
    if jobs:
        arr = (_hip.PrepJob * len(jobs))(*jobs)
        _pb("prep_many", 0.0, 0.0)
        check(lib.aesr_weight_prep_many(arr, len(jobs), stream()), "aesr_weight_prep_many")
        _pe()
    for c in commits:
        c()


_DEFERRED = None

def flush_wgrad_reductions(jobs):
    for k in range(0, len(jobs), _hip.REDUCE_MAX_JOBS):
        part = jobs[k:k + _hip.REDUCE_MAX_JOBS]
        arr = (_hip.WgradReduceJob * len(part))(*[j[0] for j in part])
        _pb("wgrad_reduce_many", 0.0, 4.0 * sum(j[1].numel() + j[2].numel() for j in part))
        check(lib.aesr_conv2d_wgrad_reduce_many(arr, len(part), stream()), "aesr_conv2d_wgrad_reduce_many")
        _pe()


class deferred_wgrad_reductions(object):

    def __enter__(self):
        global _DEFERRED
        self.outer = _DEFERRED
        if os.environ.get("AESR_DEFER_REDUCE", "1") != "0":
            _DEFERRED = []
        return self

    def __exit__(self, *exc):
        global _DEFERRED
        jobs, _DEFERRED = (_DEFERRED or []), self.outer
        if exc[0] is None:
            if self.outer is not None:
                self.outer.extend(jobs)
            else:
                flush_wgrad_reductions(jobs)
# ... 73 lines not shown
```

Baseline: 15870 slices/s.

## Fuse Cout=1 conv dgrad into wgrad pass and defer thin reductions to batched reduce

For the final Cout=1 3x3 conv, one kernel now computes the input gradient (with the activation mask applied) alongside the wgrad partials. This replaces separate dgrad and wgrad passes that each reread the same tiles. The wgrad partial reductions for this conv and for the stem conv are moved into the shared batched reduce_many launch as new job kinds, which removes separate sum and finish launches. The wino wgrad kernel also predicates its second-row MFMAs and reads on partial tiles, so half-empty edge tiles skip the extra work. The cost is more complex reduce tables, a done-word handshake for the stem finish, and more register pressure in the fused kernel.

```diff
diff --git a/include/aesr_hip.h b/include/aesr_hip.h
--- a/include/aesr_hip.h
+++ b/include/aesr_hip.h
@@ -74,6 +74,11 @@
 int aesr_conv2d_cout1_dgrad_pre(const float* dy, const float* w_flipped, const float* y_saved, float* dx, int N, int H, int W, int Cin,
                                 int mask_act, float slope, void* stream);
 
+int aesr_conv2d_cout1_bwd(const float* x, const float* dy, const float* w_flipped, float* dx, float* dw, float* db, float* workspace, int N,
+                          int H, int W, int Cin, int mask_act, float slope, void* stream);
+int aesr_conv2d_cout1_bwd_partial(const float* x, const float* dy, const float* w_flipped, float* dx, float* workspace, int N, int H, int W,
+                                  int Cin, int mask_act, float slope, void* stream);
+
 size_t aesr_stemconv_folded_floats(int C1);
 int aesr_stemconv_fold(const float* w_stem, const float* b_stem, const float* w1, float* folded, int Cs, int C1, void* stream);
 int aesr_stemconv_fwd(const float* x, const float* folded, const float* b1, float* out, int N, int H, int W, int C1,
@@ -82,6 +87,7 @@
 int aesr_stemconv_wgrad(const float* x, const float* g, const float* w_stem, const float* b_stem, const float* w1,
                         float* dw_stem, float* db_stem, float* dw1, float* db1, float* workspace, int N, int H, int W, int Cs,
                         int C1, int stem_pad, void* stream);
+int aesr_stemconv_wgrad_partial(const float* x, const float* g, float* workspace, int N, int H, int W, int C1, int stem_pad, void* stream);
 
 int aesr_space_to_depth2(const float* x, float* out, int N, int H, int W, int C, void* stream);
 int aesr_depth_to_space2(const float* g, float* dx, int N, int H, int W, int C, void* stream);
@@ -241,11 +247,20 @@
 int aesr_conv2d_wgrad_up2(const float* x_half, const float* dy, float* dw, float* db, float* workspace, int N, int H, int W, int Cin,
                           int Cout, void* stream);
 
+#define AESR_REDUCE_SLABS 0
+#define AESR_REDUCE_COUT1 1
+#define AESR_REDUCE_STEM 2
 typedef struct aesr_wgrad_reduce_job {
     const float* workspace;
     float* dw;
     float* db;
     int N, H, W, Cin, Cout, KS, pad;
+    int kind;
+    const float* w_stem;
+    const float* b_stem;
+    const float* w1;
+    float* dw_stem;
+    float* db_stem;
 } aesr_wgrad_reduce_job;
 int aesr_conv2d_wgrad_partial(const float* x, const float* dy, float* workspace, int N, int H, int W, int Cin, int Cout, int KS,
                               int pad, int x_up2, void* stream);
diff --git a/superresolution_aniso_mri_amd/_hip.py b/superresolution_aniso_mri_amd/_hip.py
--- a/superresolution_aniso_mri_amd/_hip.py
+++ b/superresolution_aniso_mri_amd/_hip.py
@@ -23,7 +23,11 @@
 
 class WgradReduceJob(ctypes.Structure):
     _fields_ = [("workspace", c_void_p), ("dw", c_void_p), ("db", c_void_p), ("N", c_int), ("H", c_int), ("W", c_int), ("Cin", c_int),
-                ("Cout", c_int), ("KS", c_int), ("pad", c_int)]
+                ("Cout", c_int), ("KS", c_int), ("pad", c_int), ("kind", c_int), ("w_stem", c_void_p), ("b_stem", c_void_p), ("w1", c_void_p),
+                ("dw_stem", c_void_p), ("db_stem", c_void_p)]
+
+
+REDUCE_SLABS, REDUCE_COUT1, REDUCE_STEM = 0, 1, 2
 
 
 class PrepJob(ctypes.Structure):
@@ -67,6 +71,9 @@
     "aesr_stemconv_fwd": (c_int, [P, P, P, P] + [c_int] * 6 + [c_float, P]),
     "aesr_stemconv_workspace_floats": (c_size_t, [c_int]),
     "aesr_stemconv_wgrad": (c_int, [P] * 10 + [c_int] * 6 + [P]),
+    "aesr_stemconv_wgrad_partial": (c_int, [P, P, P] + [c_int] * 5 + [P]),
+    "aesr_conv2d_cout1_bwd": (c_int, [P] * 7 + [c_int] * 5 + [c_float, P]),
+    "aesr_conv2d_cout1_bwd_partial": (c_int, [P] * 5 + [c_int] * 5 + [c_float, P]),
     "aesr_space_to_depth2": (c_int, [P, P] + [c_int] * 4 + [P]),
     "aesr_depth_to_space2": (c_int, [P, P] + [c_int] * 4 + [P]),
     "aesr_resample2_fwd": (c_int, [P, P] + [c_int] * 5 + [P]),
diff --git a/superresolution_aniso_mri_amd/csrc/aesr_api.hip b/superresolution_aniso_mri_amd/csrc/aesr_api.hip
--- a/superresolution_aniso_mri_amd/csrc/aesr_api.hip
+++ b/superresolution_aniso_mri_amd/csrc/aesr_api.hip
@@ -618,25 +618,48 @@
     return wgrad_impl(x, dy, nullptr, nullptr, workspace, N, H, W, Cin, Cout, KS, pad, stream, x_up2);
 }
 
+#define THIN_NWG 512
+static unsigned* stem_done_word(float* workspace, int C1) { return (unsigned*)(workspace + (size_t)THIN_NWG * 19 * C1 + (size_t)18 * C1); }
+static bool thin_channels_ok(int C) { return C >= 4 && C <= 256 && C % 4 == 0 && ((C / 4) & (C / 4 - 1)) == 0; }
+
 int aesr_conv2d_wgrad_reduce_many(const aesr_wgrad_reduce_job* jobs_host, int njobs, void* stream) {
     AESR_CHECK_ARG(jobs_host && njobs > 0, "aesr_conv2d_wgrad_reduce_many: no jobs");
     for (int j0 = 0; j0 < njobs; j0 += REDUCE_MAX_JOBS) {
         ReduceTable t;
         memset(&t, 0, sizeof(t));
         t.njobs = njobs - j0 < REDUCE_MAX_JOBS ? njobs - j0 : REDUCE_MAX_JOBS;
-        int nb = 0;
-        for (int k = 0; k < t.njobs; ++k) {
-            const aesr_wgrad_reduce_job& jb = jobs_host[j0 + k];
-            AESR_CHECK_ARG(jb.workspace && jb.dw && jb.N > 0 && (jb.KS == 1 || jb.KS == 3), "aesr_conv2d_wgrad_reduce_many: bad job %d", j0 + k);
-            AESR_CHECK_ARG(conv_dims_ok(jb.N, jb.H, jb.W, jb.Cin, jb.Cout) && jb.pad >= 0 && jb.pad < jb.KS && jb.H + 2 * jb.pad >= jb.KS && jb.W + 2 * jb.pad >= jb.KS,
-                           "aesr_conv2d_wgrad_reduce_many: job %d: bad shape", j0 + k);
-            const int Ho = jb.H + 2 * jb.pad - jb.KS + 1, Wo = jb.W + 2 * jb.pad - jb.KS + 1;
-            const WgradPlan p = plan_wgrad(jb.N, Ho, Wo, jb.Cin, jb.Cout, jb.KS, jb.pad);
-            ReduceJob& o = t.job[k];
-            o.slab = jb.workspace; o.dw = jb.dw; o.db = jb.db; o.nslab = p.nslab; o.KS2 = jb.KS * jb.KS; o.Cin = jb.Cin; o.CinP = p.CinP;
-            o.Cout = jb.Cout; o.CoutP = p.CoutP; o.block0 = nb;
-            nb += ceil_div(o.KS2 * jb.Cin * jb.Cout + (jb.db ? jb.Cout : 0), 64);
-        }
+        int nb = 0, k = 0;
+        for (int pass = 0; pass < 2; ++pass)
+            for (int i = 0; i < t.njobs; ++i) {
+                const aesr_wgrad_reduce_job& jb = jobs_host[j0 + i];
+                AESR_CHECK_ARG(jb.kind >= AESR_REDUCE_SLABS && jb.kind <= AESR_REDUCE_STEM, "aesr_conv2d_wgrad_reduce_many: job %d: unknown kind %d", j0 + i, jb.kind);
+                if ((jb.kind == AESR_REDUCE_SLABS) != (pass == 1)) continue;
+                ReduceJob& o = t.job[k++];
+                o.slab = jb.workspace; o.dw = jb.dw; o.db = jb.db; o.block0 = nb; o.kind = jb.kind;
+                if (jb.kind == AESR_REDUCE_COUT1) {
+                    AESR_CHECK_ARG(jb.workspace && jb.dw && thin_channels_ok(jb.Cin), "aesr_conv2d_wgrad_reduce_many: job %d (Cout == 1 tail): null pointer "
+                                   "or Cin=%d not 4 times a power of two (4..256)", j0 + i, jb.Cin);
+                    o.nslab = THIN_NWG; o.Cin = jb.Cin; o.Cout = 1;
+                    o.nblk = ceil_div(10 * jb.Cin, 16);
+                } else if (jb.kind == AESR_REDUCE_STEM) {
+                    AESR_CHECK_ARG(jb.workspace && jb.dw && jb.w_stem && jb.w1 && jb.dw_stem && jb.Cin > 0 && thin_channels_ok(jb.Cout),
+                                   "aesr_conv2d_wgrad_reduce_many: job %d (stem tail): null pointer, Cs=%d or C1=%d not 4 times a power of two (4..256)", j0 + i, jb.Cin, jb.Cout);
+                    AESR_CHECK_ARG(!jb.db_stem || jb.b_stem, "aesr_conv2d_wgrad_reduce_many: job %d: db_stem needs b_stem", j0 + i);
+                    o.nslab = THIN_NWG; o.Cin = jb.Cin; o.Cout = jb.Cout;
+                    o.w_stem = jb.w_stem; o.b_stem = jb.b_stem; o.w1 = jb.w1; o.dws = jb.dw_stem; o.dbs = jb.db_stem;
+                    o.done = stem_done_word(const_cast<float*>(jb.workspace), jb.Cout);
+                    o.nblk = ceil_div(18 * jb.Cout, 16);
+                } else {
+                    AESR_CHECK_ARG(jb.workspace && jb.dw && jb.N > 0 && (jb.KS == 1 || jb.KS == 3), "aesr_conv2d_wgrad_reduce_many: bad job %d", j0 + i);
+                    AESR_CHECK_ARG(conv_dims_ok(jb.N, jb.H, jb.W, jb.Cin, jb.Cout) && jb.pad >= 0 && jb.pad < jb.KS && jb.H + 2 * jb.pad >= jb.KS && jb.W + 2 * jb.pad >= jb.KS,
+                                   "aesr_conv2d_wgrad_reduce_many: job %d: bad shape", j0 + i);
+                    const int Ho = jb.H + 2 * jb.pad - jb.KS + 1, Wo = jb.W + 2 * jb.pad - jb.KS + 1;
+                    const WgradPlan p = plan_wgrad(jb.N, Ho, Wo, jb.Cin, jb.Cout, jb.KS, jb.pad);
+                    o.nslab = p.nslab; o.KS2 = jb.KS * jb.KS; o.Cin = jb.Cin; o.CinP = p.CinP; o.Cout = jb.Cout; o.CoutP = p.CoutP;
+                    o.nblk = ceil_div(o.KS2 * jb.Cin * jb.Cout + (jb.db ? jb.Cout : 0), 64);
+                }
+                nb += o.nblk;
+            }
         t.nblocks = nb;
         if (int e = aesr_launch_wgrad_reduce_many(t, (hipStream_t)stream)) return e;
     }
@@ -732,9 +755,6 @@
     return aesr_launch_cout1_fwd(a, (hipStream_t)stream);
 }
 
-#define THIN_NWG 512
-static bool thin_channels_ok(int C) { return C >= 4 && C <= 256 && C % 4 == 0 && ((C / 4) & (C / 4 - 1)) == 0; }
-
 size_t aesr_conv2d_cout1_workspace_floats(int Cin) {
     const size_t legacy = (size_t)SMALL_WGRAD_NWG * (Cin * 9 + 1);
     const size_t thin = (size_t)(THIN_NWG + 1) * 10 * Cin;
@@ -789,6 +809,32 @@
     a.N = N; a.Hs = H; a.Ws = W; a.Ho = H; a.Wo = W; a.C = Cin; a.ps = 0;
     a.act = ACT_NONE; a.mask_act = y_saved ? mask_act : ACT_NONE; a.slope = slope;
     return aesr_launch_thin_expand(a, (hipStream_t)stream);
+}
+
+static int cout1_bwd_launch(const char* who, const float* x, const float* dy, const float* w_flipped, float* dx, float* workspace, int N, int H,
+                            int W, int Cin, int mask_act, float slope, void* stream) {
+    AESR_CHECK_ARG(x && dy && w_flipped && dx && workspace && N > 0 && H > 0 && W > 0, "%s: null pointer or empty shape", who);
+    AESR_CHECK_ARG(thin_channels_ok(Cin), "%s: Cin=%d must be 4 times a power of two (4..256)", who, Cin);
+    ThinArgs a;
+    memset(&a, 0, sizeof(a));
+    a.s = dy; a.t = x; a.w = w_flipped; a.out = dx; a.partial = workspace;
+    a.N = N; a.Hs = H; a.Ws = W; a.Ho = H; a.Wo = W; a.C = Cin; a.ps = 0; a.with_be = 0;
+    a.act = ACT_NONE; a.mask_act = mask_act; a.slope = slope;
+    return aesr_launch_thin_cout1_bwd(a, THIN_NWG, (hipStream_t)stream);
+}
+
+int aesr_conv2d_cout1_bwd(const float* x, const float* dy, const float* w_flipped, float* dx, float* dw, float* db, float* workspace, int N,
+                          int H, int W, int Cin, int mask_act, float slope, void* stream) {
+    AESR_CHECK_ARG(dw && db, "aesr_conv2d_cout1_bwd: null pointer");
+    if (int e = cout1_bwd_launch("aesr_conv2d_cout1_bwd", x, dy, w_flipped, dx, workspace, N, H, W, Cin, mask_act, slope, stream)) return e;
+    float* R = workspace + (size_t)THIN_NWG * 10 * Cin;
+    if (int e = aesr_launch_sum_partials(workspace, THIN_NWG, 10 * Cin, R, 10 * Cin, nullptr, (hipStream_t)stream)) return e;
+    return aesr_launch_thin_cout1_finish(R, dw, db, Cin, (hipStream_t)stream);
+}
+
+int aesr_conv2d_cout1_bwd_partial(const float* x, const float* dy, const float* w_flipped, float* dx, float* workspace, int N, int H, int W,
+                                  int Cin, int mask_act, float slope, void* stream) {
+    return cout1_bwd_launch("aesr_conv2d_cout1_bwd_partial", x, dy, w_flipped, dx, workspace, N, H, W, Cin, mask_act, slope, stream);
 }
 
 size_t aesr_stemconv_folded_floats(int C1) { return (size_t)2 * 9 * C1; }
@@ -829,6 +875,18 @@
     return aesr_launch_thin_stem_finish(R, w_stem, b_stem, w1, dw_stem, db_stem, dw1, db1, Cs, C1, (hipStream_t)stream);
 }
 
+int aesr_stemconv_wgrad_partial(const float* x, const float* g, float* workspace, int N, int H, int W, int C1, int stem_pad, void* stream) {
+    AESR_CHECK_ARG(x && g && workspace, "aesr_stemconv_wgrad_partial: null pointer");
+    AESR_CHECK_ARG(N > 0 && H > 0 && W > 0 && stem_pad >= 0, "aesr_stemconv_wgrad_partial: bad shape");
+    AESR_CHECK_ARG(thin_channels_ok(C1), "aesr_stemconv_wgrad_partial: C1=%d must be 4 times a power of two (4..256)", C1);
+    ThinArgs a;
+    memset(&a, 0, sizeof(a));
+    a.s = x; a.t = g; a.partial = workspace;
+    a.N = N; a.Hs = H; a.Ws = W; a.Ho = H + 2 * stem_pad; a.Wo = W + 2 * stem_pad; a.C = C1; a.ps = stem_pad; a.with_be = 1;
+    a.done_word = stem_done_word(workspace, C1);
+    return aesr_launch_thin_reduce(a, THIN_NWG, (hipStream_t)stream);
+}
+
 int aesr_resample2_fwd(const float* x, float* out, int N, int H, int W, int C, int mode, void* stream) {
     AESR_CHECK_ARG(x && out && N > 0 && H > 0 && W > 0 && C > 0 && C % 4 == 0, "aesr_resample2_fwd: bad arguments (C %% 4 == 0)");
     AESR_CHECK_ARG(mode >= AESR_RS_POOL && mode <= AESR_RS_BILINEAR, "aesr_resample2_fwd: unknown mode %d", mode);
diff --git a/superresolution_aniso_mri_amd/csrc/aesr_kernels.h b/superresolution_aniso_mri_amd/csrc/aesr_kernels.h
--- a/superresolution_aniso_mri_amd/csrc/aesr_kernels.h
+++ b/superresolution_aniso_mri_amd/csrc/aesr_kernels.h
@@ -75,7 +75,11 @@
 size_t aesr_wgrad_wino_lds_bytes(int TH, int TW);
 bool aesr_wgrad_wino_tile_ok(int TH, int TW);
 #define REDUCE_MAX_JOBS 16
-struct ReduceJob { const float* slab; float* dw; float* db; int nslab, KS2, Cin, CinP, Cout, CoutP, block0; };
+enum { REDUCE_SLABS = 0, REDUCE_COUT1 = 1, REDUCE_STEM = 2 };
+struct ReduceJob {
+    const float* slab; float* dw; float* db; int nslab, KS2, Cin, CinP, Cout, CoutP, block0;
+    int kind, nblk; const float* w_stem; const float* b_stem; const float* w1; float* dws; float* dbs; unsigned* done;
+};
 struct ReduceTable { int njobs, nblocks; ReduceJob job[REDUCE_MAX_JOBS]; };
 int aesr_launch_wgrad_reduce_many(const ReduceTable& t, hipStream_t st);
 int aesr_launch_wgrad_reduce(const float* slab, float* dw, float* db, int nslab, int KS, int Cin, int CinP, int Cout, int CoutP, hipStream_t st);
@@ -127,9 +131,11 @@
     float slope;
     int with_be;
     int tiles_y, tiles_x, ntiles;
+    unsigned* done_word;
 };
 int aesr_launch_thin_expand(ThinArgs a, hipStream_t st);
 int aesr_launch_thin_reduce(ThinArgs a, int nwg, hipStream_t st);
+int aesr_launch_thin_cout1_bwd(ThinArgs a, int nwg, hipStream_t st);
 int aesr_launch_thin_collapse(const float* x, const float* w, const float* bias, float* out, int N, int H, int W, int C, int act,
                               float slope, hipStream_t st);
 int aesr_launch_thin_stem_fold(const float* ws, const float* bs, const float* w1, float* folded, int Cs, int C1, hipStream_t st);
diff --git a/superresolution_aniso_mri_amd/csrc/conv_thin.hip b/superresolution_aniso_mri_amd/csrc/conv_thin.hip
--- a/superresolution_aniso_mri_amd/csrc/conv_thin.hip
+++ b/superresolution_aniso_mri_amd/csrc/conv_thin.hip
@@ -83,8 +83,8 @@
     }
 }
 
-template <bool WITH_BE>
-__global__ __launch_bounds__(256) void thin_reduce_kernel(ThinArgs a) {
+template <bool WITH_BE, bool WITH_DX>
+__device__ __forceinline__ void thin_reduce_body(const ThinArgs& a) {
     __shared__ float xs[THIN_TH + 2][THIN_XS];
     extern __shared__ __attribute__((aligned(16))) float red[];
     constexpr int NROW = WITH_BE ? 19 : 10;
@@ -98,6 +98,13 @@
         accW[t] = (f32x4){0.f, 0.f, 0.f, 0.f};
         accB[t] = (f32x4){0.f, 0.f, 0.f, 0.f};
     }
+    f32x4 wf[WITH_DX ? 9 : 1];
+    if (WITH_DX) {
+#pragma unroll
+        for (int t = 0; t < 9; ++t) wf[t] = *(const f32x4*)(a.w + t * a.C + c4 * 4);
+    }
+    const float nslope = a.act == ACT_LRELU ? a.slope : (a.act == ACT_RELU ? 0.f : 1.f);
+    if (a.done_word && blockIdx.x == 0 && tid == 0) *a.done_word = 0u;
     const int tpi = a.tiles_y * a.tiles_x;
     for (int tile = blockIdx.x; tile < a.ntiles; tile += gridDim.x) {
         const int n = tile / tpi;
@@ -144,6 +151,22 @@
                 }
             }
             if (c4 == 0 && xin && oy < a.Ho) accs += xs[r + 1][plr + 1];
+            if (WITH_DX && xin && oy < a.Ho) {
+                f32x4 d = {0.f, 0.f, 0.f, 0.f};
+#pragma unroll
+                for (int t = 0; t < 9; ++t) {
+                    const float v = xs[r + t / 3][plr + t % 3];
+#pragma unroll
+                    for (int e = 0; e < 4; ++e) d[e] = fmaf(wf[t][e], v, d[e]);
+                }
+#pragma unroll
+                for (int e = 0; e < 4; ++e) d[e] = fmaxf(d[e], d[e] * nslope);
+                if (a.mask_act != ACT_NONE) {
+#pragma unroll
+                    for (int e = 0; e < 4; ++e) d[e] *= act_grad_from_output(g[r][e], a.mask_act, a.slope);
+                }
+                *(f32x4*)(a.out + (((size_t)n * a.Ho + oy) * a.Wo + ox) * a.C + c4 * 4) = d;
+            }
         }
     }
     for (int m = C4; m < 64; m <<= 1) {
@@ -171,6 +194,15 @@
     for (int o = tid; o < nout; o += 256)
         a.partial[(size_t)blockIdx.x * nout + o] =
             (red[o] + red[(size_t)nout + o]) + (red[2 * (size_t)nout + o] + red[3 * (size_t)nout + o]);
+}
+
+template <bool WITH_BE>
+__global__ __launch_bounds__(256) void thin_reduce_kernel(ThinArgs a) {
+    thin_reduce_body<WITH_BE, false>(a);
+}
+
+__global__ __launch_bounds__(256) void thin_expand_kernel_cout1_bwd(ThinArgs a) {
+    thin_reduce_body<false, true>(a);
 }
 
 __global__ __launch_bounds__(256) void thin_collapse_kernel(const float* __restrict__ x, const float* __restrict__ w,
@@ -345,6 +377,21 @@
     return AESR_OK;
 }
 
+int aesr_launch_thin_cout1_bwd(ThinArgs a, int nwg, hipStream_t st) {
+    if (!thin_shape_ok(a)) {
+        aesr_set_error("thin conv: C=%d must be 4 times a power of two (4..256)", a.C);
+        return AESR_ERR_ARG;
+    }
+    const int TW = thin_tw(a.C / 4);
+    a.tiles_y = ceil_div(a.Ho, THIN_TH);
+    a.tiles_x = ceil_div(a.Wo, TW);
+    a.ntiles = a.N * a.tiles_y * a.tiles_x;
+    const size_t shmem = (size_t)4 * 10 * a.C * sizeof(float);
+    hipLaunchKernelGGL(thin_expand_kernel_cout1_bwd, dim3(nwg), dim3(256), shmem, st, a);
+    AESR_LAUNCH_CHECK("thin_cout1_bwd");
+    return AESR_OK;
+}
+
 int aesr_launch_thin_collapse(const float* x, const float* w, const float* bias, float* out, int N, int H, int W, int C, int act,
                               float slope, hipStream_t st) {
     const int C4 = C / 4;
diff --git a/superresolution_aniso_mri_amd/csrc/conv_wgrad.hip b/superresolution_aniso_mri_amd/csrc/conv_wgrad.hip
--- a/superresolution_aniso_mri_amd/csrc/conv_wgrad.hip
+++ b/superresolution_aniso_mri_amd/csrc/conv_wgrad.hip
@@ -243,12 +243,110 @@
     }
 }
 
+constexpr int TAIL_COLS = 16;
+__device__ __forceinline__ float tail_sum_column(const float* __restrict__ partial, int np, int n, int o, double (*red)[TAIL_COLS]) {
+    const int col = threadIdx.x & (TAIL_COLS - 1), rl = threadIdx.x / TAIL_COLS;
+    double s = 0.0;
+    if (o < n) {
+        double s0 = 0.0, s1 = 0.0, s2 = 0.0, s3 = 0.0;
+        int p = rl;
+        for (; p + 48 < np; p += 64) {
+            const float v0 = partial[(size_t)p * n + o], v1 = partial[(size_t)(p + 16) * n + o];
+            const float v2 = partial[(size_t)(p + 32) * n + o], v3 = partial[(size_t)(p + 48) * n + o];
+            s0 += (double)v0;
+            s1 += (double)v1;
+            s2 += (double)v2;
+            s3 += (double)v3;
+        }
+        for (; p < np; p += 16) s0 += (double)partial[(size_t)p * n + o];
+        s = (s0 + s1) + (s2 + s3);
+    }
+    red[rl][col] = s;
+    __syncthreads();
+    s = 0.0;
+    if (rl == 0 && o < n) {
+#pragma unroll
+        for (int k = 0; k < 16; ++k) s += red[k][col];
+    }
+    return (float)s;
+}
+
+__device__ __forceinline__ void tail_stem_finish(const float* __restrict__ R, const ReduceJob& jb) {
+    const int Cs = jb.Cin, C1 = jb.Cout;
+    const int lane = threadIdx.x & 63, wave = threadIdx.x >> 6;
+    for (int c = wave; c < Cs; c += 4) {
+        double sw[4], sb[4];
+#pragma unroll
+        for (int k = 0; k < 4; ++k) {
+            sw[k] = 0.0;
+            sb[k] = 0.0;
+            for (int o = lane + 64 * k; o < C1 * 9; o += 256) {
+                const int co = o / 9, tp = o - co * 9;
+                const double wv = (double)jb.w1[((size_t)co * Cs + c) * 9 + tp];
+                sw[k] += wv * (double)R[tp * C1 + co];
+                sb[k] += wv * (double)R[(9 + tp) * C1 + co];
+            }
+        }
+        double aw = (sw[0] + sw[2]) + (sw[1] + sw[3]), ab = (sb[0] + sb[2]) + (sb[1] + sb[3]);
+#pragma unroll
+        for (int h = 32; h > 0; h >>= 1) {
+            aw += __shfl_down(aw, h, 64);
+            ab += __shfl_down(ab, h, 64);
+        }
+        if (lane == 0) {
+            jb.dws[c] = (float)aw;
+            if (jb.dbs) jb.dbs[c] = (float)ab;
+        }
+    }
+    for (int o = threadIdx.x; o < C1 * Cs * 9; o += 256) {
+        const int tp = o % 9, c = (o / 9) % Cs, co = o / (9 * Cs);
+        float v = R[tp * C1 + co] * jb.w_stem[c];
+        if (jb.b_stem) v = fmaf(R[(9 + tp) * C1 + co], jb.b_stem[c], v);
+        jb.dw[o] = v;
+    }
+    if (jb.db)
+        for (int co = threadIdx.x; co < C1; co += 256) jb.db[co] = R[(9 + 4) * C1 + co];
+}
+
+__device__ __forceinline__ void tail_job(const ReduceJob& jb, int blk) {
+    __shared__ double red[16][TAIL_COLS];
+    __shared__ int last;
+    const int col = threadIdx.x & (TAIL_COLS - 1), rl = threadIdx.x / TAIL_COLS;
+    const int o = blk * TAIL_COLS + col;
+    if (jb.kind == REDUCE_COUT1) {
+        const int n = 10 * jb.Cin;
+        const float r = tail_sum_column(jb.slab, jb.nslab, n, o, red);
+        if (rl == 0 && o < n) {
+            const int row = o / jb.Cin, ci = o - row * jb.Cin;
+            if (row < 9) jb.dw[ci * 9 + (8 - row)] = r;
+            else if (ci == 0 && jb.db) jb.db[0] = r;
+        }
+        return;
+    }
+    const int n = 19 * jb.Cout, nuse = 18 * jb.Cout;
+    float* R = const_cast<float*>(jb.slab) + (size_t)jb.nslab * n;
+    const float r = tail_sum_column(jb.slab, jb.nslab, n, o < nuse ? o : n, red);
+    if (rl == 0 && o < nuse) R[o] = r;
+    __threadfence();
+    __syncthreads();
+    if (threadIdx.x == 0) last = atomicAdd(jb.done, 1u) == (unsigned)(jb.nblk - 1) ? 1 : 0;
+    __syncthreads();
+    if (!last) return;
+    __threadfence();
+    if (threadIdx.x == 0) *jb.done = 0u;
+    tail_stem_finish(R, jb);
+}
+
 __global__ __launch_bounds__(256) void wgrad_reduce_many_kernel(ReduceTable t) {
     __shared__ float red[4][64];
     int j = 0;
     for (int k = 1; k < t.njobs; ++k)
         if ((int)blockIdx.x >= t.job[k].block0) j = k;
     const ReduceJob& jb = t.job[j];
+    if (jb.kind != REDUCE_SLABS) {
+        tail_job(jb, (int)blockIdx.x - jb.block0);
+        return;
+    }
     const int o = ((int)blockIdx.x - jb.block0) * 64 + (threadIdx.x & 63);
     const int sl = threadIdx.x >> 6;
     const int nw = jb.KS2 * jb.Cin * jb.Cout;
diff --git a/superresolution_aniso_mri_amd/csrc/conv_wgrad_wino.hip b/superresolution_aniso_mri_amd/csrc/conv_wgrad_wino.hip
--- a/superresolution_aniso_mri_amd/csrc/conv_wgrad_wino.hip
+++ b/superresolution_aniso_mri_amd/csrc/conv_wgrad_wino.hip
@@ -206,11 +206,47 @@
             asm volatile("v_mfma_f32_16x16x4_f32 %0, %1, %2, %0" : "+a"(acc_) : "v"(va_), "v"(vb_));
         });
     };
+    auto mfma_row_if = [&](auto Rc, int cb, int run) {
+        constexpr int r = decltype(Rc)::value;
+        f32x4 &c0 = acc[4 * r][0][0], &c1 = acc[4 * r][0][1], &c2 = acc[4 * r][1][0], &c3 = acc[4 * r][1][1];
+        f32x4 &c4 = acc[4 * r + 1][0][0], &c5 = acc[4 * r + 1][0][1], &c6 = acc[4 * r + 1][1][0], &c7 = acc[4 * r + 1][1][1];
+        f32x4 &c8 = acc[4 * r + 2][0][0], &c9 = acc[4 * r + 2][0][1], &c10 = acc[4 * r + 2][1][0], &c11 = acc[4 * r + 2][1][1];
+        f32x4 &c12 = acc[4 * r + 3][0][0], &c13 = acc[4 * r + 3][0][1], &c14 = acc[4 * r + 3][1][0], &c15 = acc[4 * r + 3][1][1];
+        constexpr int s_ = r >> 1, h_ = r & 1;
+        const float a00 = Vp[cb][0][s_][0][h_], a01 = Vp[cb][0][s_][1][h_], a02 = Vp[cb][0][s_][2][h_], a03 = Vp[cb][0][s_][3][h_];
+        const float a10 = Vp[cb][1][s_][0][h_], a11 = Vp[cb][1][s_][1][h_], a12 = Vp[cb][1][s_][2][h_], a13 = Vp[cb][1][s_][3][h_];
+        constexpr int m0 = r == 0 || r == 3 ? 0 : 2, m3 = r == 0 || r == 3 ? 1 : 3, mh = r >= 2 ? 1 : 0;
+        const float b00 = Mp[cb][0][m0][mh], b01 = Mp[cb][0][4 + r][0], b02 = Mp[cb][0][4 + r][1], b03 = Mp[cb][0][m3][mh];
+        const float b10 = Mp[cb][1][m0][mh], b11 = Mp[cb][1][4 + r][0], b12 = Mp[cb][1][4 + r][1], b13 = Mp[cb][1][m3][mh];
+        asm volatile("s_cmp_eq_u32 %32, 0\n\t"
+                     "s_cbranch_scc1 1f\n\t"
+                     "v_mfma_f32_16x16x4_f32 %0, %16, %24, %0\n\t"
+                     "v_mfma_f32_16x16x4_f32 %1, %16, %28, %1\n\t"
+                     "v_mfma_f32_16x16x4_f32 %2, %20, %24, %2\n\t"
+                     "v_mfma_f32_16x16x4_f32 %3, %20, %28, %3\n\t"
+                     "v_mfma_f32_16x16x4_f32 %4, %17, %25, %4\n\t"
+                     "v_mfma_f32_16x16x4_f32 %5, %17, %29, %5\n\t"
+                     "v_mfma_f32_16x16x4_f32 %6, %21, %25, %6\n\t"
+                     "v_mfma_f32_16x16x4_f32 %7, %21, %29, %7\n\t"
+                     "v_mfma_f32_16x16x4_f32 %8, %18, %26, %8\n\t"
+                     "v_mfma_f32_16x16x4_f32 %9, %18, %30, %9\n\t"
+                     "v_mfma_f32_16x16x4_f32 %10, %22, %26, %10\n\t"
+                     "v_mfma_f32_16x16x4_f32 %11, %22, %30, %11\n\t"
+                     "v_mfma_f32_16x16x4_f32 %12, %19, %27, %12\n\t"
+                     "v_mfma_f32_16x16x4_f32 %13, %19, %31, %13\n\t"
+                     "v_mfma_f32_16x16x4_f32 %14, %23, %27, %14\n\t"
+                     "v_mfma_f32_16x16x4_f32 %15, %23, %31, %15\n\t"
+                     "\n1:"
+                     : "+a"(c0), "+a"(c1), "+a"(c2), "+a"(c3), "+a"(c4), "+a"(c5), "+a"(c6), "+a"(c7), "+a"(c8), "+a"(c9), "+a"(c10),
+                       "+a"(c11), "+a"(c12), "+a"(c13), "+a"(c14), "+a"(c15)
+                     : "v"(a00), "v"(a01), "v"(a02), "v"(a03), "v"(a10), "v"(a11), "v"(a12), "v"(a13), "v"(b00), "v"(b01), "v"(b02),
+                       "v"(b03), "v"(b10), "v"(b11), "v"(b12), "v"(b13), "s"(__builtin_amdgcn_readfirstlane(run))
+                     : "scc");
+    };
     auto step_xu = [&](int j, int buf) { const int ks = wave + 4 * j, tyl = ks / KPR, kx = ks - tyl * KPR; return buf * XFL + ((2 * tyl) * PWL + 8 * kx) * 32; };
     auto step_du = [&](int j, int buf) { const int ks = wave + 4 * j, tyl = ks / KPR, kx = ks - tyl * KPR; return buf * DFL + ((2 * tyl) * TWL + 8 * kx) * 32; };
     using C0 = std::integral_constant<int, 0>;
     using C16 = std::integral_constant<int, 16>;
-    using C32 = std::integral_constant<int, 32>;
 
     long long tph[3] = {0, 0, 0}, tq = 0;
 #define WW_STAMP(k)                                                   \
@@ -240,13 +276,14 @@
     op_transform(0);
     WW_STAMP(2)
     if (t0.n < a.N) do {
+        const int full = t0.ty * TH + TH / 2 < a.H ? 1 : 0;
         __builtin_amdgcn_sched_barrier(0);
 #if WW_ABL != 3 && WW_ABL != 4
-        op_read(step_xu(1, buf), step_du(1, buf), 1);
+        if (full) op_read(step_xu(1, buf), step_du(1, buf), 1);
 #endif
         mfmas(C0{}, C16{}, 0);
 #if WW_ABL != 2 && WW_ABL != 4
-        op_transform(1);
+        if (full) op_transform(1);
 #endif
         mfmas(C16{}, std::integral_constant<int, 48>{}, 0);
         __builtin_amdgcn_sched_barrier(0);
@@ -258,17 +295,18 @@
 #if WW_ABL != 3 && WW_ABL != 4
         op_read(step_xu(0, buf ^ 1), step_du(0, buf ^ 1), 0);
 #endif
-        mfmas(C0{}, C16{}, 1);
+        mfma_row_if(C0{}, 1, full);
         __builtin_amdgcn_sched_barrier(0);
 #if WW_ABL != 1 && WW_ABL != 4
         fetch(t2, buf);
 #endif
         __builtin_amdgcn_sched_barrier(0);
-        mfmas(C16{}, C16{}, 1);
+        mfma_row_if(std::integral_constant<int, 1>{}, 1, full);
 #if WW_ABL != 2 && WW_ABL != 4
         op_transform(0);
 #endif
-        mfmas(C32{}, C32{}, 1);
+        mfma_row_if(std::integral_constant<int, 2>{}, 1, full);
+        mfma_row_if(std::integral_constant<int, 3>{}, 1, full);
         __builtin_amdgcn_sched_barrier(0);
         t0 = t1;
         t1 = t2;
diff --git a/superresolution_aniso_mri_amd/engine.py b/superresolution_aniso_mri_amd/engine.py
--- a/superresolution_aniso_mri_amd/engine.py
+++ b/superresolution_aniso_mri_amd/engine.py
@@ -592,6 +592,20 @@
             flush_wgrad_reductions(reduce_jobs)
         return g, grads
 
+    def _cout1_fused_bwd(self, steps, saved, k, need_input_grad):
+        s = steps[k]
+        if (k == 0 and not need_input_grad) or s.in_up2 or s.s2d or not _thin_channels(s.cin):
+            return None
+        w = s.mod.weight
+        if s.flipped is None or s.packed_epoch != (self.weights_epoch, w._version, w.data_ptr()):
+            return None
+        if k > 0 and steps[k - 1].kind in ("conv", "stemconv") and steps[k - 1].act != _hip.ACT_NONE:
+            xin, mask = saved[k][0], saved[k - 1][1]
+            if mask.data_ptr() != xin.data_ptr() or mask.shape != xin.shape or not xin.is_contiguous():
+                return None
+            return steps[k - 1].act, steps[k - 1].slope
+        return _hip.ACT_NONE, 0.0
+
     def _backward_steps(self, steps, saved, g, ngrad, need_input_grad, grads, G, ns, reduce_jobs):
         for k in range(len(steps) - 1, -1, -1):
             s = steps[k]
@@ -605,9 +619,19 @@
                 db1 = self._grad_dst(s.mod.bias, grads) if s.mod.bias is not None else None
                 ws = _empty((lib.aesr_stemconv_workspace_floats(s.cout),), g)
                 _pb("thin_reduce", 0.0, 4.0 * (ngrad * H * W + g.numel()))
-                check(lib.aesr_stemconv_wgrad(ptr(xin), ptr(g), ptr(s.stem.weight), ptr(s.stem.bias), ptr(s.mod.weight),
-                                              ptr(dws), ptr(dbs), ptr(dw1), ptr(db1), ptr(ws), ngrad, H, W, s.cs, s.cout,
-                                              s.stem_pad, stream()), "aesr_stemconv_wgrad")
+                if reduce_jobs or _DEFERRED is not None:
+                    check(lib.aesr_stemconv_wgrad_partial(ptr(xin), ptr(g), ptr(ws), ngrad, H, W, s.cout, s.stem_pad, stream()),
+                          "aesr_stemconv_wgrad_partial")
+                    outs = [(s.stem.weight, dws), (s.stem.bias, dbs), (s.mod.weight, dw1)] + ([(s.mod.bias, db1)] if db1 is not None else [])
+                    direct = all(grads[p_] is None for p_, _ in outs)
+                    job = _hip.WgradReduceJob(ws.data_ptr(), dw1.data_ptr(), db1.data_ptr() if db1 is not None else None, 0, 0, 0, s.cs, s.cout,
+                                              0, 0, _hip.REDUCE_STEM, s.stem.weight.data_ptr(), s.stem.bias.data_ptr(), s.mod.weight.data_ptr(),
+                                              dws.data_ptr(), dbs.data_ptr())
+                    reduce_jobs.append((job, ws, dw1, dws, direct, (dbs, db1)))
+                else:
+                    check(lib.aesr_stemconv_wgrad(ptr(xin), ptr(g), ptr(s.stem.weight), ptr(s.stem.bias), ptr(s.mod.weight),
+                                                  ptr(dws), ptr(dbs), ptr(dw1), ptr(db1), ptr(ws), ngrad, H, W, s.cs, s.cout,
+                                                  s.stem_pad, stream()), "aesr_stemconv_wgrad")
                 _pe()
                 g = None
                 break
@@ -647,10 +671,33 @@
                                                          s.pad, stream()), "aesr_conv2d_smallcin_wgrad")
                 elif s.cout == 1 and s.ks == 3 and s.pad == 1 and db is not None:
                     ws = _empty((lib.aesr_conv2d_cout1_workspace_floats(s.cin),), g)
-                    _pb("thin_reduce", 0.0, 4.0 * (N * H * W * s.cin + g.numel()))
-                    check(lib.aesr_conv2d_cout1_wgrad(ptr(xin), ptr(g), ptr(dw), ptr(db), ptr(ws), N, H, W, s.cin, stream()),
-                          "aesr_conv2d_cout1_wgrad")
-                    _pe()
+                    fused_dx = self._cout1_fused_bwd(steps, saved, k, need_input_grad)
+                    tail = _thin_channels(s.cin) and (_DEFERRED is not None or any(
+                        t_.kind == "conv" and not t_.s2d and t_.cin % 4 == 0 and t_.cout % 4 == 0 for t_ in steps[:k]))
+                    if fused_dx is not None:
+                        mask_act, mslope = fused_dx
+                        dx = _empty((N, H, W, s.cin), g)
+                        _pb("thin_expand", 0.0, 4.0 * (N * H * W * s.cin + g.numel()) + 4.0 * (g.numel() + dx.numel() * 2))
+                        if tail:
+                            check(lib.aesr_conv2d_cout1_bwd_partial(ptr(xin), ptr(g), ptr(s.flipped), ptr(dx), ptr(ws), N, H, W, s.cin, mask_act,
+                                                                    mslope, stream()), "aesr_conv2d_cout1_bwd_partial")
+                        else:
+                            check(lib.aesr_conv2d_cout1_bwd(ptr(xin), ptr(g), ptr(s.flipped), ptr(dx), ptr(dw), ptr(db), ptr(ws), N, H, W, s.cin,
+                                                            mask_act, mslope, stream()), "aesr_conv2d_cout1_bwd")
+                        _pe()
+                    else:
+                        _pb("thin_reduce", 0.0, 4.0 * (N * H * W * s.cin + g.numel()))
+                        check(lib.aesr_conv2d_cout1_wgrad(ptr(xin), ptr(g), ptr(dw), ptr(db), ptr(ws), N, H, W, s.cin, stream()),
+                              "aesr_conv2d_cout1_wgrad")
+                        _pe()
+                        tail = False
+                    if tail:
+                        direct = grads[s.mod.weight] is None and grads[s.mod.bias] is None
+                        job = _hip.WgradReduceJob(ws.data_ptr(), dw.data_ptr(), db.data_ptr(), 0, 0, 0, s.cin, 1, 0, 0, _hip.REDUCE_COUT1)
+                        reduce_jobs.append((job, ws, dw, db, direct))
+                    if fused_dx is not None:
+                        g = dx
+                        continue
                 else:
                     raise NotImplementedError("no wgrad kernel for conv %d->%d k%d" % (s.cin, s.cout, s.ks))
                 if s.s2d:
```

Result: no change. 15860 slices/s (-0.1%).
